# alazarteka/Self-Forcing

Hardware: AMD Instinct MI355X
Metric: decoded frames/sec/node, Wan-1.3B 832x480 4-step AR rollout (higher is better)
Workload: dtype bf16

## Files before the change

include/sf_hip.h:

```cpp
#ifndef SF_HIP_H
#define SF_HIP_H

#include <stddef.h>
#include <stdint.h>

#ifdef __cplusplus
extern "C" {
#endif

#define SF_HIP_ABI_VERSION 10

int sf_abi_version(void);
const char* sf_last_error(void);

enum sf_epilogue {
  SF_EPI_BIAS = 0,
  SF_EPI_BIAS_GELU = 1,
  SF_EPI_BIAS_RESID = 2,
  SF_EPI_BIAS_GATE_RESID = 3,
  SF_EPI_F32 = 4
};

typedef struct sf_gemm_args {
  const void* a;
  const void* w;
  const void* bias;
  void* out;
  const void* resid;
  const void* gate_mod;
  const void* gate_e0;
  int64_t gate_group_stride;
  int32_t rows_per_group;
  int32_t M, N, K;
  int32_t lda, ldw, ldo, ldr;
  int32_t epilogue;
  int32_t batch;
  int64_t a_bstride, w_bstride, o_bstride, r_bstride;
  int32_t structure;
} sf_gemm_args;

enum sf_gemm_structure { SF_GEMM_AUTO = 0, SF_GEMM_T128 = 1 ,
                         SF_GEMM_PP256 = 2 ,
                         SF_GEMM_PP128 = 3 ,
                         SF_GEMM_PP224 = 4, SF_GEMM_PP192 = 5  };

int sf_gemm_bf16(const sf_gemm_args* args, void* stream);

#define SF_FP8_AMAX_PARTS 1024
int sf_quantize_fp8(const void* x, int ldx, int M, int K, int rows_per_segment, void* q_out, float* scale_out, void* stream);

int sf_gemm_fp8(const sf_gemm_args* args, const float* a_scale, int rows_per_segment, const float* w_scale, void* stream);

int sf_small_linear_fp8(const void* x, const void* w_q, const float* w_scale, const void* bias, void* out, int M, int N, int K,
                        int rows_per_segment, int act_in, int act_out, void* stream);

int sf_small_linear(const void* x, const void* w, const void* bias, void* out, int M, int N, int K,
                    int act_in, int act_out, void* stream);

int sf_sinusoid_embedding(const void* t, int t_is_int64, void* out, int n, int dim, void* stream);

int sf_layernorm_modulate(const void* x, void* out, int M, int C, float eps, const void* mod_shift,
                          const void* mod_scale, const void* e0_shift, const void* e0_scale,
                          int64_t e0_group_stride, int rows_per_group, void* stream);

int sf_layernorm_affine(const void* x, const void* weight, const void* bias, void* out, int M, int C,
                        float eps, void* stream);

int sf_rmsnorm(const void* x, int ldx, const void* weight, void* out, int ldo, int M, int C, float eps,
               void* stream);

int sf_qkv_norm_rope_cache(const void* qkv, const void* norm_q_w, const void* norm_k_w, void* q_out,
                           void* k_cache, void* v_cache, const float* rope_cos, const float* rope_sin,
                           int B, int f, int h, int w, int C, int num_heads, int64_t cache_tokens,
                           int write_start, int start_frame, float eps, void* stream);

int sf_kv_evict(void* cache, int B, int64_t cache_tokens, int row_elems, int sink, int evict, int keep,
                void* scratch, size_t scratch_bytes, void* stream);

int sf_attention(const void* q, const void* k, const void* v, void* out, int B, int H, int Lq, int Lk,
                 int64_t q_stride, int64_t q_bstride, int64_t kv_stride, int64_t kv_bstride,
                 int64_t o_stride, int64_t o_bstride, void* stream);

enum sf_attn_structure { SF_ATTN_AUTO = 0, SF_ATTN_R64 = 1, SF_ATTN_W8 = 2, SF_ATTN_W4 = 3 };
int sf_attention_ex(const void* q, const void* k, const void* v, void* out, int B, int H, int Lq, int Lk,
                    int64_t q_stride, int64_t q_bstride, int64_t kv_stride, int64_t kv_bstride,
                    int64_t o_stride, int64_t o_bstride, int structure, void* stream);

int sf_patchify(const void* x, void* cols, int B, int F, int Cin, int H, int W, void* stream);

int sf_unpatchify_x0(const void* head_out, const void* xt, const void* timestep, int t_is_int64,
                     const float* sigmas, const float* timesteps, int n_table, void* flow, void* x0,
                     int B, int F, int groups, int Cout, int H, int W, void* stream);

int sf_add_noise(const void* x0, const void* eps, const void* timestep, int t_is_int64,
                 const float* sigmas, const float* timesteps, int n_table, void* out, int n_outer,
                 int64_t inner, void* stream);

#define SF_LINCOMB_MAX 6
int sf_lincomb_bf16(void* out, const void* const* xs, const float* coefs, int n_terms, int64_t n, void* stream);

typedef struct sf_layer_weights {
  const void* modulation;
  const void *norm3_w, *norm3_b;
  const void *qkv_w, *qkv_b;
  const void *norm_q_w, *norm_k_w;
  const void *o_w, *o_b;
  const void *cq_w, *cq_b;
  const void *ckv_w, *ckv_b;
  const void *cnorm_q_w, *cnorm_k_w;
  const void *co_w, *co_b;
  const void *ffn0_w, *ffn0_b;
  const void *ffn2_w, *ffn2_b;
} sf_layer_weights;

typedef struct sf_model {
  int32_t dim, ffn_dim, num_heads, num_layers, in_dim, out_dim, freq_dim, text_dim, text_len;
  float eps;
  const void *patch_w, *patch_b;
  const void *text0_w, *text0_b, *text2_w, *text2_b;
  const void *time0_w, *time0_b, *time2_w, *time2_b;
  const void *tproj_w, *tproj_b;
  const void *head_w, *head_b;
  const void* head_mod;
  const void *pose_w, *pose_b;
  int32_t pose_dim;
  const sf_layer_weights* layers_host;
  const float *rope_cos, *rope_sin;
  const float *sched_sigmas, *sched_timesteps;
  int32_t n_table;
  int32_t fp8;
  const void *text0_q, *text2_q, *time0_q, *time2_q, *tproj_q, *head_q, *pose_q;
  const float *text0_s, *text2_s, *time0_s, *time2_s, *tproj_s, *head_s, *pose_s;
  const struct sf_layer_fp8* layers_fp8_host;
} sf_model;

typedef struct sf_layer_fp8 {
  const void *qkv_q, *o_q, *cq_q, *ckv_q, *co_q, *ffn0_q, *ffn2_q;
  const float *qkv_s, *o_s, *cq_s, *ckv_s, *co_s, *ffn0_s, *ffn2_s;
} sf_layer_fp8;

typedef struct sf_forward_args {
  int32_t batch, frames, lat_h, lat_w;
  int32_t groups;
  const void* noisy;
  const void* timestep;
  int32_t t_is_int64;
  const void* prompt_embeds;
  int32_t init_cross;
  const void* add_condition;
  void* const* k_cache_host;
  void* const* v_cache_host;
  void* const* ck_cache_host;
  void* const* cv_cache_host;
  int64_t cache_tokens;
  int32_t sink_tokens, evict, keep;
  int32_t write_start;
  int32_t attn_start, attn_end;
  int32_t start_frame;
  void* evict_scratch;
  size_t evict_scratch_bytes;
  int32_t cache_only;
  void* flow_out;
  void* x0_out;
  void* workspace;
  size_t workspace_bytes;
  void* kv_index_out;
  int64_t global_end;
} sf_forward_args;

size_t sf_dit_workspace_bytes(const sf_model* model, int batch, int frames, int lat_h, int lat_w,
                              int groups);
int sf_dit_forward(const sf_model* model, const sf_forward_args* args, void* stream);
int sf_dit_forward_pair(const sf_model* model, const sf_forward_args* context_pass, const sf_forward_args* next_pass,
                        void* stream);


enum sf_conv_epilogue {
  SF_CONV_BIAS = 0,
  SF_CONV_BIAS_RESID = 1,
  SF_CONV_BIAS_CLAMP_F32 = 2
};

typedef struct sf_conv_args {
  const void* x;
  const void* w;
  const void* bias;
  void* out;
  const void* resid;
  float* out_f32;
  int32_t Tout, H, W;
  int32_t Hin, Win;
  int32_t Cin, Cout;
  int32_t kt, kh, kw;
  int32_t upsample;
  int32_t t_in_offset;
  int32_t ldw, ldo, ldr;
  int32_t out_frame_offset;
  int32_t interleave_c;
  int32_t epilogue;
  int32_t structure;
  void* norm_out;
  const void* norm_gamma;
  int32_t norm_ld, norm_frame_offset;
  int32_t stride_hw, stride_t;
} sf_conv_args;

enum sf_conv_structure { SF_CONV_AUTO = 0, SF_CONV_IGEMM = 1 ,
                         SF_CONV_HALO = 2  };

int sf_conv_igemm(const sf_conv_args* args, void* stream);
int sf_conv_pick_nt(int cout);

int sf_rmsnorm_silu_cl(const void* x, const void* gamma, void* out, int64_t rows, int C, int silu,
                       void* stream);

int sf_softmax_rows(const float* s, int64_t lds, void* p, int64_t ldp, int rows, int cols,
                    int cols_padded, float scale, void* stream);

int sf_vae_prepare_latent(const void* latent, const float* mean, const float* std, const void* conv2_w,
                          const void* conv2_b, void* out, int z, int h, int w, int c_pad, void* stream);

typedef struct sf_vae_conv {
  const void* w;
  const void* bias;
  int32_t cin, cout, kt, kh, kw, ldw;
} sf_vae_conv;

typedef struct sf_vae_resblock {
  const void* gamma1;
  const void* gamma2;
  sf_vae_conv conv1;
  sf_vae_conv conv2;
  sf_vae_conv shortcut;
} sf_vae_resblock;

#define SF_VAE_MAX_STAGES 4

typedef struct sf_vae_model {
  int32_t z_dim;
  int32_t n_stages;
  int32_t res_per_stage;
  int32_t temporal_up[SF_VAE_MAX_STAGES];
  const float* latent_mean;
  const float* latent_std;
  const void *conv2_w, *conv2_b;
  sf_vae_conv conv1;
  sf_vae_resblock mid0, mid2;
  const void* attn_gamma;
  const void *attn_qk_w, *attn_qk_b;
  const void *attn_v_w, *attn_v_b;
  const void *attn_proj_w, *attn_proj_b;
  const sf_vae_resblock* res_host;
  sf_vae_conv time_conv[SF_VAE_MAX_STAGES];
  sf_vae_conv up_conv[SF_VAE_MAX_STAGES];
  const void* head_gamma;
  sf_vae_conv head_conv;
} sf_vae_model;

size_t sf_vae_state_bytes(const sf_vae_model* model, int lat_h, int lat_w, int window_frames);
size_t sf_vae_scratch_bytes(const sf_vae_model* model, int lat_h, int lat_w, int window_frames);
int sf_vae_reset(const sf_vae_model* model, void* state, size_t state_bytes, int lat_h, int lat_w,
                 int window_frames, void* stream);
int sf_vae_decode_frames(const sf_vae_model* model, void* state, size_t state_bytes, void* scratch,
                         size_t scratch_bytes, const void* latent_frames, int lat_h, int lat_w, int window_frames,
                         int frame_index, int n_frames, int window, int history_at, float* pixels_out, void* stream);


int sf_vae_prepare_pixels(const void* pixels, int is_f32, int64_t c_stride, void* out, int T, int H, int W, int c_pad,
                          void* stream);

int sf_vae_finish_latent(const void* head_out, int ld_in, int cin, const void* conv1_w, int ld_w, const void* conv1_b,
                         const float* mean, const float* std, float* out, int T, int z, int h, int w, void* stream);

typedef struct sf_vae_encoder {
  int32_t z_dim;
  int32_t n_stages;
  int32_t res_per_stage;
  int32_t temporal_down[SF_VAE_MAX_STAGES];
  const float* latent_mean;
  const float* latent_std;
  const void *conv1_w, *conv1_b;
  sf_vae_conv in_conv;
  const sf_vae_resblock* res_host;
  sf_vae_conv down_conv[SF_VAE_MAX_STAGES];
  sf_vae_conv time_conv[SF_VAE_MAX_STAGES];
  sf_vae_resblock mid0, mid2;
  const void* attn_gamma;
  const void *attn_qk_w, *attn_qk_b;
  const void *attn_v_w, *attn_v_b;
  const void *attn_proj_w, *attn_proj_b;
  const void* head_gamma;
  sf_vae_conv head_conv;
} sf_vae_encoder;

size_t sf_vae_encode_state_bytes(const sf_vae_encoder* enc, int H, int W, int window_frames);
size_t sf_vae_encode_scratch_bytes(const sf_vae_encoder* enc, int H, int W, int window_frames);
int sf_vae_encode_reset(const sf_vae_encoder* enc, void* state, size_t state_bytes, int H, int W, int window_frames,
                        void* stream);
int sf_vae_encode_frames(const sf_vae_encoder* enc, void* state, size_t state_bytes, void* scratch, size_t scratch_bytes,
                         const void* pixels, int is_f32, int64_t c_stride, int H, int W, int window_frames,
                         int chunk_index, int n_chunks, int window, int history_at, float* latents_out, void* stream);


enum sf_taehv_epilogue {
  SF_TAEHV_BIAS_RELU = 0,
  SF_TAEHV_BIAS_RESID_RELU = 1,
  SF_TAEHV_PLAIN = 2,
  SF_TAEHV_RELU = 3,
  SF_TAEHV_HEAD_F32 = 4
};

typedef struct sf_taehv_conv_args {
  const void* x;
  const void* w;
  const void* bias;
  void* out;
  const void* resid;
  float* out_f32;
  int32_t Tout, H, W;
  int32_t Cin, Cout;
  int32_t kt;
  int32_t upsample;
  int32_t ldw, ldo, ldr;
  int32_t tgrow;
  int32_t epilogue;
  int32_t clamp;
} sf_taehv_conv_args;

// ... 145 lines not shown
```

self-forcing_amd/_lib.py:

```python
from __future__ import annotations

import ctypes as C
import os
import subprocess
from typing import Optional

os.environ.setdefault("ROC_SIGNAL_POOL_SIZE", "1024")

_HERE = os.path.dirname(os.path.abspath(__file__))
CSRC = os.path.join(_HERE, "csrc")
LIB_PATH = os.environ.get("SF_HIP_LIB") or os.path.join(CSRC, "libsf_hip.so")

ABI_VERSION = 10
FP8_AMAX_PARTS = 1024

EPI_BIAS, EPI_BIAS_GELU, EPI_BIAS_RESID, EPI_BIAS_GATE_RESID, EPI_F32 = 0, 1, 2, 3, 4
CONV_BIAS, CONV_BIAS_RESID, CONV_BIAS_CLAMP_F32 = 0, 1, 2
VAE_MAX_STAGES = 4
TAEHV_EPILOGUES = {"bias_relu": 0, "bias_resid_relu": 1, "plain": 2, "relu": 3, "head_f32": 4}
TAEHV_STAGES, TAEHV_BLOCKS = 3, 3
POSE_DTYPES = {"uint8": 0, "float32": 1, "bfloat16": 2}
POSE_CONVS = 6
JPEG_SUBSAMPLINGS = {"420": 0, "444": 1}
JPEG_DTYPES = {"uint8": 0, "float32": 1, "bfloat16": 2}
JPEG_RANGES = {(-1, 1): 0, (0, 1): 1}
JPEG_STATUS = {1: "an interval outgrew its worst-case slot", 2: "a coefficient is outside the baseline range",
               4: "the files do not fit the output buffer"}
ACT_NONE, ACT_SILU, ACT_GELU = 0, 1, 2
ATTN_STRUCTURES = {"auto": 0, "r64": 1, "w8": 2, "w4": 3}
CONV_STRUCTURES = {"auto": 0, "igemm": 1, "halo": 2}
GEMM_STRUCTURES = {"auto": 0, "t128": 1, "pp256": 2, "pp128": 3, "pp224": 4, "pp192": 5}


class GemmArgs(C.Structure):
    _fields_ = [
        ("a", C.c_void_p), ("w", C.c_void_p), ("bias", C.c_void_p), ("out", C.c_void_p),
        ("resid", C.c_void_p), ("gate_mod", C.c_void_p), ("gate_e0", C.c_void_p),
        ("gate_group_stride", C.c_int64), ("rows_per_group", C.c_int32),
        ("M", C.c_int32), ("N", C.c_int32), ("K", C.c_int32),
        ("lda", C.c_int32), ("ldw", C.c_int32), ("ldo", C.c_int32), ("ldr", C.c_int32),
        ("epilogue", C.c_int32), ("batch", C.c_int32),
        ("a_bstride", C.c_int64), ("w_bstride", C.c_int64), ("o_bstride", C.c_int64), ("r_bstride", C.c_int64),
        ("structure", C.c_int32),
    ]


class LayerWeights(C.Structure):
    _fields_ = [(n, C.c_void_p) for n in (
        "modulation", "norm3_w", "norm3_b", "qkv_w", "qkv_b", "norm_q_w", "norm_k_w", "o_w", "o_b",
        "cq_w", "cq_b", "ckv_w", "ckv_b", "cnorm_q_w", "cnorm_k_w", "co_w", "co_b",
        "ffn0_w", "ffn0_b", "ffn2_w", "ffn2_b")]


class LayerFp8(C.Structure):
    _fields_ = [(n, C.c_void_p) for n in (
        "qkv_q", "o_q", "cq_q", "ckv_q", "co_q", "ffn0_q", "ffn2_q",
        "qkv_s", "o_s", "cq_s", "ckv_s", "co_s", "ffn0_s", "ffn2_s")]


FP8_MODEL_LINEARS = (("text0", ("text_embedding.0",)), ("text2", ("text_embedding.2",)), ("time0", ("time_embedding.0",)),
                     ("time2", ("time_embedding.2",)), ("tproj", ("time_projection.1",)), ("head", ("head.head",)),
                     ("pose", ("pose_proj",)))
FP8_LAYER_LINEARS = (("qkv", ("self_attn.q", "self_attn.k", "self_attn.v")), ("o", ("self_attn.o",)), ("cq", ("cross_attn.q",)),
                     ("ckv", ("cross_attn.k", "cross_attn.v")), ("co", ("cross_attn.o",)), ("ffn0", ("ffn.0",)), ("ffn2", ("ffn.2",)))


class Model(C.Structure):
    _fields_ = (
        [(n, C.c_int32) for n in ("dim", "ffn_dim", "num_heads", "num_layers", "in_dim", "out_dim",
                                  "freq_dim", "text_dim", "text_len")]
        + [("eps", C.c_float)]
        + [(n, C.c_void_p) for n in ("patch_w", "patch_b", "text0_w", "text0_b", "text2_w", "text2_b",
                                     "time0_w", "time0_b", "time2_w", "time2_b", "tproj_w", "tproj_b",
                                     "head_w", "head_b", "head_mod", "pose_w", "pose_b")]
        + [("pose_dim", C.c_int32)]
        + [("layers_host", C.POINTER(LayerWeights)),
           ("rope_cos", C.c_void_p), ("rope_sin", C.c_void_p),
           ("sched_sigmas", C.c_void_p), ("sched_timesteps", C.c_void_p),
           ("n_table", C.c_int32)]
        + [("fp8", C.c_int32)]
        + [(n + "_q", C.c_void_p) for n, _ in FP8_MODEL_LINEARS]
        + [(n + "_s", C.c_void_p) for n, _ in FP8_MODEL_LINEARS]
        + [("layers_fp8_host", C.POINTER(LayerFp8))]
    )


class ForwardArgs(C.Structure):
    _fields_ = [
        ("batch", C.c_int32), ("frames", C.c_int32), ("lat_h", C.c_int32), ("lat_w", C.c_int32),
        ("groups", C.c_int32),
        ("noisy", C.c_void_p), ("timestep", C.c_void_p), ("t_is_int64", C.c_int32),
        ("prompt_embeds", C.c_void_p), ("init_cross", C.c_int32), ("add_condition", C.c_void_p),
        ("k_cache_host", C.POINTER(C.c_void_p)), ("v_cache_host", C.POINTER(C.c_void_p)),
        ("ck_cache_host", C.POINTER(C.c_void_p)), ("cv_cache_host", C.POINTER(C.c_void_p)),
        ("cache_tokens", C.c_int64),
        ("sink_tokens", C.c_int32), ("evict", C.c_int32), ("keep", C.c_int32),
        ("write_start", C.c_int32), ("attn_start", C.c_int32), ("attn_end", C.c_int32),
        ("start_frame", C.c_int32),
        ("evict_scratch", C.c_void_p), ("evict_scratch_bytes", C.c_size_t),
        ("cache_only", C.c_int32),
        ("flow_out", C.c_void_p), ("x0_out", C.c_void_p),
        ("workspace", C.c_void_p), ("workspace_bytes", C.c_size_t),
        ("kv_index_out", C.c_void_p), ("global_end", C.c_int64),
    ]


class ConvArgs(C.Structure):
    _fields_ = (
        [(n, C.c_void_p) for n in ("x", "w", "bias", "out", "resid", "out_f32")]
        + [(n, C.c_int32) for n in ("Tout", "H", "W", "Hin", "Win", "Cin", "Cout", "kt", "kh", "kw", "upsample",
                                    "t_in_offset", "ldw", "ldo", "ldr", "out_frame_offset", "interleave_c", "epilogue", "structure")]
        + [("norm_out", C.c_void_p), ("norm_gamma", C.c_void_p), ("norm_ld", C.c_int32), ("norm_frame_offset", C.c_int32)]
        + [("stride_hw", C.c_int32), ("stride_t", C.c_int32)]
    )


class VaeConv(C.Structure):
    _fields_ = [("w", C.c_void_p), ("bias", C.c_void_p)] + [(n, C.c_int32) for n in ("cin", "cout", "kt", "kh", "kw", "ldw")]


class VaeResBlock(C.Structure):
    _fields_ = [("gamma1", C.c_void_p), ("gamma2", C.c_void_p), ("conv1", VaeConv), ("conv2", VaeConv), ("shortcut", VaeConv)]


class VaeModel(C.Structure):
    _fields_ = [
        ("z_dim", C.c_int32), ("n_stages", C.c_int32), ("res_per_stage", C.c_int32),
        ("temporal_up", C.c_int32 * VAE_MAX_STAGES),
        ("latent_mean", C.c_void_p), ("latent_std", C.c_void_p), ("conv2_w", C.c_void_p), ("conv2_b", C.c_void_p),
        ("conv1", VaeConv), ("mid0", VaeResBlock), ("mid2", VaeResBlock),
        ("attn_gamma", C.c_void_p), ("attn_qk_w", C.c_void_p), ("attn_qk_b", C.c_void_p),
        ("attn_v_w", C.c_void_p), ("attn_v_b", C.c_void_p), ("attn_proj_w", C.c_void_p), ("attn_proj_b", C.c_void_p),
        ("res_host", C.POINTER(VaeResBlock)),
        ("time_conv", VaeConv * VAE_MAX_STAGES), ("up_conv", VaeConv * VAE_MAX_STAGES),
        ("head_gamma", C.c_void_p), ("head_conv", VaeConv),
    ]


class VaeEncoder(C.Structure):
    _fields_ = [
        ("z_dim", C.c_int32), ("n_stages", C.c_int32), ("res_per_stage", C.c_int32),
        ("temporal_down", C.c_int32 * VAE_MAX_STAGES),
        ("latent_mean", C.c_void_p), ("latent_std", C.c_void_p), ("conv1_w", C.c_void_p), ("conv1_b", C.c_void_p),
        ("in_conv", VaeConv), ("res_host", C.POINTER(VaeResBlock)),
        ("down_conv", VaeConv * VAE_MAX_STAGES), ("time_conv", VaeConv * VAE_MAX_STAGES),
        ("mid0", VaeResBlock), ("mid2", VaeResBlock),
        ("attn_gamma", C.c_void_p), ("attn_qk_w", C.c_void_p), ("attn_qk_b", C.c_void_p),
        ("attn_v_w", C.c_void_p), ("attn_v_b", C.c_void_p), ("attn_proj_w", C.c_void_p), ("attn_proj_b", C.c_void_p),
        ("head_gamma", C.c_void_p), ("head_conv", VaeConv),
    ]


class TaehvConvArgs(C.Structure):
    _fields_ = ([(n, C.c_void_p) for n in ("x", "w", "bias", "out", "resid", "out_f32")]
                + [(n, C.c_int32) for n in ("Tout", "H", "W", "Cin", "Cout", "kt", "upsample", "ldw", "ldo", "ldr", "tgrow", "epilogue", "clamp")])


class TaehvLayer(C.Structure):
    _fields_ = [("w", C.c_void_p), ("bias", C.c_void_p)] + [(n, C.c_int32) for n in ("cin", "cout", "kt", "ldw")]


class TaehvModel(C.Structure):
    _fields_ = [("z_dim", C.c_int32), ("in_conv", TaehvLayer), ("block", ((TaehvLayer * 3) * TAEHV_BLOCKS) * TAEHV_STAGES),
                ("exit_conv", TaehvLayer * TAEHV_STAGES), ("tgrow", C.c_int32 * TAEHV_STAGES), ("head", TaehvLayer)]


class PoseConvArgs(C.Structure):
    _fields_ = ([(n, C.c_void_p) for n in ("x", "w", "bias", "out")]
                + [(n, C.c_int32) for n in ("T", "H", "W", "Cin", "Cout", "kt", "stride_t", "stride_s", "ldw", "ldo", "silu")])


class PoseLayer(C.Structure):
    _fields_ = [("w", C.c_void_p), ("bias", C.c_void_p)] + [(n, C.c_int32) for n in ("cin", "cout", "kt", "stride_t", "stride_s", "ldw", "silu")]


class PoseModel(C.Structure):
    _fields_ = [("conv", PoseLayer * POSE_CONVS), ("embed_w", C.c_void_p), ("embed_b", C.c_void_p), ("pose_dim", C.c_int32),
                ("ref_conv", PoseLayer * POSE_CONVS)]


class T5Layer(C.Structure):
    _fields_ = [(n, C.c_void_p) for n in ("norm1_w", "qk_w", "v_w", "o_w", "norm2_w", "gate_w", "fc1_w", "fc2_w", "pos_emb")]


class T5Model(C.Structure):
    _fields_ = ([(n, C.c_int32) for n in ("vocab", "dim", "dim_attn", "dim_ffn", "num_heads", "num_layers", "num_buckets")]
                + [("eps", C.c_float), ("token_embedding", C.c_void_p), ("layers_host", C.POINTER(T5Layer)),
                   ("final_norm_w", C.c_void_p)])


_vp, _i, _i64, _f, _sz = C.c_void_p, C.c_int, C.c_int64, C.c_float, C.c_size_t
SIGNATURES = {
    "sf_abi_version": (C.c_int, []),
    "sf_last_error": (C.c_char_p, []),
    "sf_gemm_bf16": (C.c_int, [C.POINTER(GemmArgs), _vp]),
    "sf_small_linear": (C.c_int, [_vp, _vp, _vp, _vp, _i, _i, _i, _i, _i, _vp]),
    "sf_quantize_fp8": (C.c_int, [_vp, _i, _i, _i, _i, _vp, _vp, _vp]),
    "sf_gemm_fp8": (C.c_int, [C.POINTER(GemmArgs), _vp, _i, _vp, _vp]),
    "sf_small_linear_fp8": (C.c_int, [_vp, _vp, _vp, _vp, _vp, _i, _i, _i, _i, _i, _i, _vp]),
    "sf_sinusoid_embedding": (C.c_int, [_vp, _i, _vp, _i, _i, _vp]),
    "sf_layernorm_modulate": (C.c_int, [_vp, _vp, _i, _i, _f, _vp, _vp, _vp, _vp, _i64, _i, _vp]),
    "sf_layernorm_affine": (C.c_int, [_vp, _vp, _vp, _vp, _i, _i, _f, _vp]),
    "sf_rmsnorm": (C.c_int, [_vp, _i, _vp, _vp, _i, _i, _i, _f, _vp]),
    "sf_qkv_norm_rope_cache": (C.c_int, [_vp, _vp, _vp, _vp, _vp, _vp, _vp, _vp, _i, _i, _i, _i, _i, _i, _i64,
                                         _i, _i, _f, _vp]),
    "sf_kv_evict": (C.c_int, [_vp, _i, _i64, _i, _i, _i, _i, _vp, _sz, _vp]),
    "sf_attention": (C.c_int, [_vp, _vp, _vp, _vp, _i, _i, _i, _i, _i64, _i64, _i64, _i64, _i64, _i64, _vp]),
    "sf_attention_ex": (C.c_int, [_vp, _vp, _vp, _vp, _i, _i, _i, _i, _i64, _i64, _i64, _i64, _i64, _i64, _i, _vp]),
    "sf_patchify": (C.c_int, [_vp, _vp, _i, _i, _i, _i, _i, _vp]),
    "sf_unpatchify_x0": (C.c_int, [_vp, _vp, _vp, _i, _vp, _vp, _i, _vp, _vp, _i, _i, _i, _i, _i, _i, _vp]),
    "sf_add_noise": (C.c_int, [_vp, _vp, _vp, _i, _vp, _vp, _i, _vp, _i, _i64, _vp]),
    "sf_lincomb_bf16": (C.c_int, [_vp, C.POINTER(C.c_void_p), C.POINTER(C.c_float), _i, _i64, _vp]),
    "sf_dit_workspace_bytes": (C.c_size_t, [C.POINTER(Model), _i, _i, _i, _i, _i]),
    "sf_dit_forward": (C.c_int, [C.POINTER(Model), C.POINTER(ForwardArgs), _vp]),
    "sf_dit_forward_pair": (C.c_int, [C.POINTER(Model), C.POINTER(ForwardArgs), C.POINTER(ForwardArgs), _vp]),
    "sf_conv_igemm": (C.c_int, [C.POINTER(ConvArgs), _vp]),
    "sf_conv_pick_nt": (C.c_int, [_i]),
    "sf_rmsnorm_silu_cl": (C.c_int, [_vp, _vp, _vp, _i64, _i, _i, _vp]),
    "sf_softmax_rows": (C.c_int, [_vp, _i64, _vp, _i64, _i, _i, _i, _f, _vp]),
    "sf_vae_prepare_latent": (C.c_int, [_vp, _vp, _vp, _vp, _vp, _vp, _i, _i, _i, _i, _vp]),
    "sf_vae_state_bytes": (C.c_size_t, [C.POINTER(VaeModel), _i, _i, _i]),
    "sf_vae_scratch_bytes": (C.c_size_t, [C.POINTER(VaeModel), _i, _i, _i]),
    "sf_vae_reset": (C.c_int, [C.POINTER(VaeModel), _vp, _sz, _i, _i, _i, _vp]),
    "sf_vae_decode_frames": (C.c_int, [C.POINTER(VaeModel), _vp, _sz, _vp, _sz, _vp, _i, _i, _i, _i, _i, _i, _i, _vp, _vp]),
    "sf_vae_prepare_pixels": (C.c_int, [_vp, _i, _i64, _vp, _i, _i, _i, _i, _vp]),
    "sf_vae_finish_latent": (C.c_int, [_vp, _i, _i, _vp, _i, _vp, _vp, _vp, _vp, _i, _i, _i, _i, _vp]),
    "sf_vae_encode_state_bytes": (C.c_size_t, [C.POINTER(VaeEncoder), _i, _i, _i]),
    "sf_vae_encode_scratch_bytes": (C.c_size_t, [C.POINTER(VaeEncoder), _i, _i, _i]),
    "sf_vae_encode_reset": (C.c_int, [C.POINTER(VaeEncoder), _vp, _sz, _i, _i, _i, _vp]),
    "sf_vae_encode_frames": (C.c_int, [C.POINTER(VaeEncoder), _vp, _sz, _vp, _sz, _vp, _i, _i64, _i, _i, _i, _i, _i, _i, _i, _vp,
                                       _vp]),
    "sf_taehv_conv": (C.c_int, [C.POINTER(TaehvConvArgs), _vp]),
    "sf_taehv_pick_nt": (C.c_int, [_i]),
    "sf_taehv_prepare_latent": (C.c_int, [_vp, _vp, _i, _i, _i, _i, _i, _vp]),
    "sf_taehv_state_bytes": (C.c_size_t, [C.POINTER(TaehvModel), _i, _i]),
    "sf_taehv_scratch_bytes": (C.c_size_t, [C.POINTER(TaehvModel), _i, _i, _i]),
    "sf_taehv_reset": (C.c_int, [C.POINTER(TaehvModel), _vp, _sz, _i, _i, _vp]),
    "sf_taehv_decode_frames": (C.c_int, [C.POINTER(TaehvModel), _vp, _sz, _vp, _sz, _vp, _i, _i, _i, _i, _vp, _vp]),
    "sf_pose_out_size": (C.c_int, [_i, _i, _i]),
    "sf_pose_conv": (C.c_int, [C.POINTER(PoseConvArgs), _vp]),
    "sf_pose_prepare": (C.c_int, [_vp, _i, _i, _i, _i, _i, _i, _vp, _vp]),
    "sf_pose_patch_embed": (C.c_int, [_vp, _i, _i, _i, _vp, _vp, _i, _vp, _vp, _vp]),
    "sf_pose_scratch_bytes": (C.c_size_t, [C.POINTER(PoseModel), _i, _i, _i]),
    "sf_pose_embed": (C.c_int, [C.POINTER(PoseModel), _vp, _i, _i, _i, _i, _vp, _sz, _vp, _i64, _vp]),
    "sf_pose_embed_ref": (C.c_int, [C.POINTER(PoseModel), _vp, _i, _i, _i, _vp, _sz, _vp, _vp]),
    "sf_jpeg_workspace_bytes": (C.c_size_t, [_i, _i, _i, _i, _i]),
    "sf_jpeg_transform": (C.c_int, [_vp, _i, _i, _i, _i, _i, _i, _i, _vp, _vp]),
    "sf_jpeg_entropy": (C.c_int, [_vp, _i, _i, _i, _i, _i, _i, _vp, _sz, _vp, _sz, _vp, _vp, _vp]),
    "sf_jpeg_encode_frames": (C.c_int, [_vp, _i, _i, _i, _i, _i, _i, _i, _i, _vp, _sz, _vp, _sz, _vp, _vp, _vp]),
    "sf_embedding_gather": (C.c_int, [_vp, _vp, _vp, _i, _i, _i, _vp]),
    "sf_t5_softmax_bias": (C.c_int, [_vp, _vp, _vp, _vp, _vp, _i, _i, _i, _vp]),
    "sf_mul_bf16": (C.c_int, [_vp, _vp, _vp, _i64, _vp]),
    "sf_zero_masked_rows": (C.c_int, [_vp, _vp, _i, _i, _vp]),
    "sf_t5_workspace_bytes": (C.c_size_t, [C.POINTER(T5Model), _i, _i]),
    "sf_t5_encode": (C.c_int, [C.POINTER(T5Model), _vp, _vp, _vp, _i, _i, _vp, _vp, _sz, _vp]),
    "sf_probe_mfma": (C.c_int, [_i, _i, _i, _vp, _vp, C.POINTER(C.c_double), _vp]),
    "sf_probe_copy": (C.c_int, [_vp, _vp, _sz, _vp]),
}

_lib: Optional[C.CDLL] = None


class SfHipError(RuntimeError):
    pass


def build(verbose: bool = False) -> str:
    cmd = ["make", "-C", CSRC, "-j8"]
    res = subprocess.run(cmd, capture_output=True, text=True)
    if verbose or res.returncode != 0:
        print(res.stdout)
        print(res.stderr)
    if res.returncode != 0:
        raise SfHipError(f"building {LIB_PATH} failed (exit {res.returncode})")
    return LIB_PATH


def lib() -> C.CDLL:
    global _lib
    if _lib is not None:
        return _lib
    if not os.path.exists(LIB_PATH):
        raise SfHipError(
            f"{LIB_PATH} not found: the HIP extension is not built. Run "
            f"`python -c 'import __graft_entry__ as g; g.build()'` (or `make -C {CSRC}`). "
            "There is no CPU/eager fallback for this path.")
    handle = C.CDLL(LIB_PATH)
    for name, (res, args) in SIGNATURES.items():
        fn = getattr(handle, name)
        fn.restype = res
        fn.argtypes = args
    ver = handle.sf_abi_version()
    if ver != ABI_VERSION:
        raise SfHipError(f"{LIB_PATH}: ABI version {ver}, expected {ABI_VERSION}; rebuild")
    _lib = handle
    return handle


def check(rc: int, what: str = "") -> None:
    if rc != 0:
        msg = lib().sf_last_error()
        raise SfHipError(f"{what or 'sf_hip'} failed (rc={rc}): {msg.decode() if msg else '?'}")
```

self-forcing_amd/csrc/dit_forward.hip:

```cpp
#include <algorithm>
#include "sf_host.h"

int sf_internal_write_kv_indices(void* buf, int layers, int64_t global_end, int64_t local_end, void* stream);

namespace {

struct Work {
  void *x, *xn, *qkv, *q, *att, *hbuf, *cols, *headout, *sin, *etmp, *e, *e0, *ctx1, *ctx;
  void* xq;
  float* xs;
  size_t total;
};

constexpr int FP8_MAX_SEGMENTS = 8;

Work carve(const sf_model* m, void* ws, int B, int F, int lat_h, int lat_w, int groups) {
  const size_t M = (size_t)B * F * (lat_h / 2) * (lat_w / 2);
  const size_t C = m->dim, BG = (size_t)B * groups, T = (size_t)B * m->text_len;
  Carve c(ws);
  Work w;
  w.x = c.take(M * C * 2);
  w.xn = c.take(M * C * 2);
  w.qkv = c.take(M * 3 * C * 2);
  w.q = c.take(M * C * 2);
  w.att = c.take(M * C * 2);
  w.hbuf = c.take(M * (size_t)m->ffn_dim * 2);
  w.cols = c.take(M * (size_t)m->in_dim * 4 * 2);
  w.headout = c.take(M * (size_t)m->out_dim * 4 * 2);
  w.sin = c.take(BG * m->freq_dim * 2);
  w.etmp = c.take(BG * C * 2);
  w.e = c.take(BG * C * 2);
  w.e0 = c.take(BG * 6 * C * 2);
  w.ctx1 = c.take(T * C * 2);
  w.ctx = c.take(T * C * 2);
  w.xq = nullptr;
  w.xs = nullptr;
  if (m->fp8) {
    const size_t pose = m->pose_dim > 0 ? (size_t)m->pose_dim : C;
    const size_t widest_tok = std::max({(size_t)m->ffn_dim, C, pose}), widest_txt = std::max((size_t)m->text_dim, C);
    w.xq = c.take(std::max(M * widest_tok, T * widest_txt));
    w.xs = (float*)c.take(FP8_MAX_SEGMENTS * (1 + SF_FP8_AMAX_PARTS) * sizeof(float));
  }
  w.total = c.off;
  return w;
}

inline const char* bptr(const void* p, size_t elems) { return (const char*)p + elems * 2; }

}

extern "C" size_t sf_dit_workspace_bytes(const sf_model* model, int batch, int frames, int lat_h, int lat_w, int groups) {
  if (!model || batch <= 0 || frames <= 0 || lat_h <= 0 || lat_w <= 0 || groups <= 0) return 0;
  return carve(model, nullptr, batch, frames, lat_h, lat_w, groups).total;
}

static int forward_passes(const sf_model* m, const sf_forward_args* const* ps, int np, void* stream) {
  const sf_forward_args* a = ps[0];
  SF_CHECK(m && a, "sf_dit_forward: null argument");
  SF_CHECK(m->layers_host && m->num_layers > 0, "sf_dit_forward: model has no layers");
  SF_CHECK(m->dim == m->num_heads * 128, "sf_dit_forward: head_dim must be 128 (dim=%d heads=%d)", m->dim, m->num_heads);
  SF_CHECK(a->batch > 0 && a->frames > 0 && a->groups > 0, "sf_dit_forward: empty input");
  SF_CHECK(a->lat_h % 2 == 0 && a->lat_w % 2 == 0, "sf_dit_forward: latent size must be even");
  const int B = a->batch, F = a->frames, h = a->lat_h / 2, w = a->lat_w / 2;
  const int L = F * h * w, M = B * L, C = m->dim, G = a->groups, BG = B * G;
  const int Mt = np * M, BGt = np * BG;
  SF_CHECK(F % G == 0, "sf_dit_forward: frames=%d not divisible by timestep groups=%d", F, G);
  const int rpg = L / G;
  SF_CHECK(BGt <= 32, "sf_dit_forward: passes*batch*groups=%d exceeds the small-linear limit of 32", BGt);
  int first_full = np;
  for (int p = 0; p < np; ++p) {
    const sf_forward_args* q = ps[p];
    SF_CHECK(q, "sf_dit_forward: null pass");
    SF_CHECK(q->batch == B && q->frames == F && q->lat_h == a->lat_h && q->lat_w == a->lat_w && q->groups == G,
             "sf_dit_forward: the passes of one call must share batch, frames, latent size and timestep groups");
    SF_CHECK(q->k_cache_host == a->k_cache_host && q->v_cache_host == a->v_cache_host && q->ck_cache_host == a->ck_cache_host &&
             q->cv_cache_host == a->cv_cache_host && q->cache_tokens == a->cache_tokens, "sf_dit_forward: the passes of one call must share their caches");
    SF_CHECK(q->noisy && q->timestep, "sf_dit_forward: null tensor");
    SF_CHECK(q->cache_only || (q->flow_out && q->x0_out), "sf_dit_forward: null output tensor");
    SF_CHECK(q->attn_start >= 0 && q->attn_end > q->attn_start && q->attn_end <= q->cache_tokens, "sf_dit_forward: bad attention window [%d, %d) of %lld",
             q->attn_start, q->attn_end, (long long)q->cache_tokens);
    SF_CHECK(q->write_start >= 0 && (int64_t)q->write_start + L <= q->cache_tokens,
             "sf_dit_forward: KV cache overflow: write_start=%d + %d new tokens > capacity %lld", q->write_start, L, (long long)q->cache_tokens);
    SF_CHECK(q->write_start + L == q->attn_end, "sf_dit_forward: the new tokens must end the attention window");
    if (q->evict > 0) SF_CHECK(q->evict_scratch && q->keep >= 0, "sf_dit_forward: eviction needs evict_scratch");
    SF_CHECK(np == 1 || !q->init_cross, "sf_dit_forward_pair: the cross-attention cache must be initialised by an earlier single pass");
    if (!q->cache_only && first_full == np) first_full = p;
    SF_CHECK(!(q->cache_only && first_full != np), "sf_dit_forward_pair: cache_only passes must come first");
  }
  SF_CHECK(a->k_cache_host && a->v_cache_host && a->ck_cache_host && a->cv_cache_host, "sf_dit_forward: null cache table");
  const Work ws = carve(m, a->workspace, np * B, F, a->lat_h, a->lat_w, G);
  SF_CHECK(a->workspace && a->workspace_bytes >= ws.total, "sf_dit_forward: workspace too small (%zu < %zu)", a->workspace_bytes, ws.total);
  SF_CHECK(!a->init_cross || a->prompt_embeds, "sf_dit_forward: init_cross needs prompt_embeds");

  const bool f8 = m->fp8 != 0;
  static const sf_layer_fp8 no_fp8 = {};
  SF_CHECK(!f8 || m->layers_fp8_host, "sf_dit_forward: fp8 model without per-layer fp8 weights");
  auto run = [&](const Gemm& g) -> int { return f8 ? g.fp8(ws.xq, ws.xs, stream) : g.bf16(stream); };
  auto lin = [&](const Gemm& g) -> int {
    if (f8) SF_TRY(sf_quantize_fp8(g.g.a, g.g.lda, g.g.M, g.g.K, g.rows_per_segment, ws.xq, ws.xs, stream));
    return run(g);
  };
  auto small = [&](const void* x, const void* w16, const void* w8, const float* s8, const void* bias, void* out, int N, int K, int act_in,
                   int act_out) -> int {
    if (!f8) return sf_small_linear(x, w16, bias, out, BGt, N, K, act_in, act_out, stream);
    return sf_small_linear_fp8(x, w8, s8, bias, out, BGt, N, K, BG, act_in, act_out, stream);
  };

  const int Kp = m->in_dim * 4, Nh = m->out_dim * 4;
  const long cache_b = (long)a->cache_tokens * C;
  const long ctx_b = (long)m->text_len * C;
  const sf_forward_args* last = ps[np - 1];
  auto finish_indices = [&]() -> int {
    if (last->kv_index_out) return sf_internal_write_kv_indices(last->kv_index_out, m->num_layers, last->global_end, last->attn_end, stream);
    return 0;
  };

  for (int p = 0; p < np; ++p)
    SF_TRY(sf_patchify(ps[p]->noisy, (void*)bptr(ws.cols, (size_t)p * M * Kp), B, F, m->in_dim, a->lat_h, a->lat_w, stream));
  SF_TRY(Gemm(ws.cols, Kp, m->patch_w, Kp, ws.x, C, Mt, C, Kp).bias(m->patch_b).bf16(stream));

  for (int p = 0; p < np; ++p) {
    if (!ps[p]->add_condition) continue;
    void* xp = (void*)bptr(ws.x, (size_t)p * M * C);
    if (m->pose_w || (f8 && m->pose_q)) {
      SF_CHECK(m->pose_dim > 0, "sf_dit_forward: pose_proj weights without pose_dim");
      SF_TRY(lin(Gemm(ps[p]->add_condition, m->pose_dim, m->pose_w, m->pose_dim, xp, C, M, C, m->pose_dim).bias(m->pose_b)
                     .epi(SF_EPI_BIAS_RESID).resid(xp, C).fp8w(m->pose_q, m->pose_s, M)));
    } else {
      SF_CHECK(m->pose_dim == C, "sf_dit_forward: add_condition without pose_proj weights needs pose_dim == dim (%d != %d)", m->pose_dim, C);
      const void* terms[2] = {xp, ps[p]->add_condition};
      const float ones[2] = {1.0f, 1.0f};
      SF_TRY(sf_lincomb_bf16(xp, terms, ones, 2, (int64_t)M * C, stream));
    }
  }

  for (int p = 0; p < np; ++p)
    SF_TRY(sf_sinusoid_embedding(ps[p]->timestep, ps[p]->t_is_int64, (void*)bptr(ws.sin, (size_t)p * BG * m->freq_dim), BG, m->freq_dim, stream));
  SF_TRY(small(ws.sin, m->time0_w, m->time0_q, m->time0_s, m->time0_b, ws.etmp, C, m->freq_dim, 0, 1));
  SF_TRY(small(ws.etmp, m->time2_w, m->time2_q, m->time2_s, m->time2_b, ws.e, C, C, 0, 0));
  SF_TRY(small(ws.e, m->tproj_w, m->tproj_q, m->tproj_s, m->tproj_b, ws.e0, 6 * C, C, 1, 0));

  if (a->init_cross) {
    const int T = B * m->text_len;
    SF_TRY(lin(Gemm(a->prompt_embeds, m->text_dim, m->text0_w, m->text_dim, ws.ctx1, C, T, C, m->text_dim).bias(m->text0_b).epi(SF_EPI_BIAS_GELU)
                   .fp8w(m->text0_q, m->text0_s, T)));
    SF_TRY(lin(Gemm(ws.ctx1, C, m->text2_w, C, ws.ctx, C, T, C, C).bias(m->text2_b).fp8w(m->text2_q, m->text2_s, T)));
    if (f8) SF_TRY(sf_quantize_fp8(ws.ctx, C, T, C, T, ws.xq, ws.xs, stream));
    for (int l = 0; l < m->num_layers; ++l) {
      const sf_layer_weights& lw = m->layers_host[l];
      const sf_layer_fp8& lq = f8 ? m->layers_fp8_host[l] : no_fp8;
      SF_TRY(run(Gemm(ws.ctx, C, lw.ckv_w, C, a->ck_cache_host[l], C, T, C, C).bias(lw.ckv_b).fp8w(lq.ckv_q, lq.ckv_s, T)));
      SF_TRY(sf_rmsnorm(a->ck_cache_host[l], C, lw.cnorm_k_w, a->ck_cache_host[l], C, T, C, m->eps, stream));
      SF_TRY(run(Gemm(ws.ctx, C, bptr(lw.ckv_w, (size_t)C * C), C, a->cv_cache_host[l], C, T, C, C).bias(bptr(lw.ckv_b, C))
                     .fp8w(f8 ? (const char*)lq.ckv_q + (size_t)C * C : nullptr, f8 ? lq.ckv_s + C : nullptr, T)));
    }
  }

  for (int l = 0; l < m->num_layers; ++l) {
    const sf_layer_weights& lw = m->layers_host[l];
    const sf_layer_fp8& lq = f8 ? m->layers_fp8_host[l] : no_fp8;
    const void* mod = lw.modulation;
    const bool last_layer = l == m->num_layers - 1;
    SF_TRY(sf_layernorm_modulate(ws.x, ws.xn, Mt, C, m->eps, bptr(mod, 0), bptr(mod, C), bptr(ws.e0, 0), bptr(ws.e0, C), 6L * C, rpg, stream));
    SF_TRY(lin(Gemm(ws.xn, C, lw.qkv_w, C, ws.qkv, 3 * C, Mt, 3 * C, C).bias(lw.qkv_b).fp8w(lq.qkv_q, lq.qkv_s, M)));
    for (int p = 0; p < np; ++p) {
      const sf_forward_args* q = ps[p];
      const size_t roff = (size_t)p * M;
      if (q->evict > 0) {
        SF_TRY(sf_kv_evict(q->k_cache_host[l], B, q->cache_tokens, C, q->sink_tokens, q->evict, q->keep, q->evict_scratch, q->evict_scratch_bytes, stream));
        SF_TRY(sf_kv_evict(q->v_cache_host[l], B, q->cache_tokens, C, q->sink_tokens, q->evict, q->keep, q->evict_scratch, q->evict_scratch_bytes, stream));
      }
      SF_TRY(sf_qkv_norm_rope_cache(bptr(ws.qkv, roff * 3 * C), lw.norm_q_w, lw.norm_k_w, (void*)bptr(ws.q, roff * C), q->k_cache_host[l], q->v_cache_host[l],
                                    m->rope_cos, m->rope_sin, B, F, h, w, C, m->num_heads, q->cache_tokens, q->write_start, q->start_frame, m->eps, stream));
      if (q->cache_only && last_layer) continue;
      SF_TRY(sf_attention(bptr(ws.q, roff * C), bptr(q->k_cache_host[l], (size_t)q->attn_start * C), bptr(q->v_cache_host[l], (size_t)q->attn_start * C),
                          (void*)bptr(ws.att, roff * C), B, m->num_heads, L, q->attn_end - q->attn_start, C, (long)L * C, C, cache_b, C, (long)L * C, stream));
    }
    const int p0 = last_layer ? first_full : 0;
    if (p0 == np) return finish_indices();
    const size_t r0 = (size_t)p0 * M;
    const int Mr = (np - p0) * M;
    void* x = (void*)bptr(ws.x, r0 * C);
    void* xn = (void*)bptr(ws.xn, r0 * C);
    void* qb = (void*)bptr(ws.q, r0 * C);
    void* att = (void*)bptr(ws.att, r0 * C);
    void* hb = (void*)bptr(ws.hbuf, r0 * m->ffn_dim);
    const void* e0r = bptr(ws.e0, (size_t)p0 * BG * 6 * C);
    SF_TRY(lin(Gemm(att, C, lw.o_w, C, x, C, Mr, C, C).bias(lw.o_b).epi(SF_EPI_BIAS_GATE_RESID).resid(x, C)
                   .gate(bptr(mod, 2 * (size_t)C), bptr(e0r, 2 * (size_t)C), 6L * C, rpg).fp8w(lq.o_q, lq.o_s, M)));
    SF_TRY(sf_layernorm_affine(x, lw.norm3_w, lw.norm3_b, xn, Mr, C, m->eps, stream));
    SF_TRY(lin(Gemm(xn, C, lw.cq_w, C, qb, C, Mr, C, C).bias(lw.cq_b).fp8w(lq.cq_q, lq.cq_s, M)));
    SF_TRY(sf_rmsnorm(qb, C, lw.cnorm_q_w, qb, C, Mr, C, m->eps, stream));
    for (int p = p0; p < np; ++p)
      SF_TRY(sf_attention(bptr(ws.q, (size_t)p * M * C), a->ck_cache_host[l], a->cv_cache_host[l], (void*)bptr(ws.att, (size_t)p * M * C), B, m->num_heads, L,
                          m->text_len, C, (long)L * C, C, ctx_b, C, (long)L * C, stream));
    SF_TRY(lin(Gemm(att, C, lw.co_w, C, x, C, Mr, C, C).bias(lw.co_b).epi(SF_EPI_BIAS_RESID).resid(x, C).fp8w(lq.co_q, lq.co_s, M)));
    SF_TRY(sf_layernorm_modulate(x, xn, Mr, C, m->eps, bptr(mod, 3 * (size_t)C), bptr(mod, 4 * (size_t)C), bptr(e0r, 3 * (size_t)C),
                                 bptr(e0r, 4 * (size_t)C), 6L * C, rpg, stream));
    SF_TRY(lin(Gemm(xn, C, lw.ffn0_w, C, hb, m->ffn_dim, Mr, m->ffn_dim, C).bias(lw.ffn0_b).epi(SF_EPI_BIAS_GELU).fp8w(lq.ffn0_q, lq.ffn0_s, M)));
    SF_TRY(lin(Gemm(hb, m->ffn_dim, lw.ffn2_w, m->ffn_dim, x, C, Mr, C, m->ffn_dim).bias(lw.ffn2_b).epi(SF_EPI_BIAS_GATE_RESID).resid(x, C)
                   .gate(bptr(mod, 5 * (size_t)C), bptr(e0r, 5 * (size_t)C), 6L * C, rpg).fp8w(lq.ffn2_q, lq.ffn2_s, M)));
  }

  {
    const size_t r0 = (size_t)first_full * M;
    const int Mr = (np - first_full) * M;
    const void* er = bptr(ws.e, (size_t)first_full * BG * C);
    SF_TRY(sf_layernorm_modulate(bptr(ws.x, r0 * C), (void*)bptr(ws.xn, r0 * C), Mr, C, m->eps, bptr(m->head_mod, 0), bptr(m->head_mod, C), er, er, (long)C, rpg, stream));
    SF_TRY(lin(Gemm(bptr(ws.xn, r0 * C), C, m->head_w, C, (void*)bptr(ws.headout, r0 * Nh), Nh, Mr, Nh, C).bias(m->head_b)
                   .fp8w(m->head_q, m->head_s, M)));
    for (int p = first_full; p < np; ++p)
      SF_TRY(sf_unpatchify_x0(bptr(ws.headout, (size_t)p * M * Nh), ps[p]->noisy, ps[p]->timestep, ps[p]->t_is_int64, m->sched_sigmas, m->sched_timesteps, m->n_table,
                              ps[p]->flow_out, ps[p]->x0_out, B, F, G, m->out_dim, a->lat_h, a->lat_w, stream));
  }
  return finish_indices();
}

extern "C" int sf_dit_forward(const sf_model* m, const sf_forward_args* a, void* stream) {
  SF_CHECK(m && a, "sf_dit_forward: null argument");
  const sf_forward_args* one[1] = {a};
  return forward_passes(m, one, 1, stream);
}

extern "C" int sf_dit_forward_pair(const sf_model* m, const sf_forward_args* context_pass, const sf_forward_args* next_pass, void* stream) {
  SF_CHECK(m && context_pass && next_pass, "sf_dit_forward_pair: null argument");
  SF_CHECK(context_pass->workspace == next_pass->workspace && context_pass->workspace_bytes == next_pass->workspace_bytes,
           "sf_dit_forward_pair: both passes name the same workspace (sized for 2 x batch)");
  const sf_forward_args* two[2] = {context_pass, next_pass};
  return forward_passes(m, two, 2, stream);
}
```

self-forcing_amd/csrc/elementwise.hip:

```cpp
#include "sf_common.h"
#include "../../include/sf_hip.h"

namespace {

constexpr int ROWS_PER_BLOCK = 4;

template <int NCH>
__device__ __forceinline__ void load_row(const bf16_t* row, int lane, float (&v)[NCH][8]) {
#pragma unroll
  for (int i = 0; i < NCH; ++i) {
    const bf16x8 t = *reinterpret_cast<const bf16x8*>(row + (i * 64 + lane) * 8);
#pragma unroll
    for (int j = 0; j < 8; ++j) v[i][j] = (float)t[j];
  }
}

template <int NCH>
__device__ __forceinline__ void ln_stats(const float (&v)[NCH][8], int C, float eps, float& mean, float& rstd) {
  float s = 0.f;
#pragma unroll
  for (int i = 0; i < NCH; ++i)
#pragma unroll
    for (int j = 0; j < 8; ++j) s += v[i][j];
  mean = wave_sum(s) / (float)C;
  float q = 0.f;
#pragma unroll
  for (int i = 0; i < NCH; ++i)
#pragma unroll
    for (int j = 0; j < 8; ++j) {
      const float d = v[i][j] - mean;
      q += d * d;
    }
  rstd = rsqrtf(wave_sum(q) / (float)C + eps);
}

#ifndef SF_LN_RPW
#define SF_LN_RPW 2
#endif
template <int NCH> struct LnRows { static constexpr int value = NCH <= 4 ? SF_LN_RPW : (NCH <= 6 ? 2 : 1); };
template <int NCH, int MODE>
__global__ __launch_bounds__(64) void layernorm_kernel(const bf16_t* __restrict__ x, bf16_t* __restrict__ out,
                                                       int M, int C, float eps, const bf16_t* __restrict__ p0,
                                                       const bf16_t* __restrict__ p1, const bf16_t* __restrict__ e0_shift,
                                                       const bf16_t* __restrict__ e0_scale, long e0_group_stride,
                                                       int rows_per_group) {
  constexpr int LN_RPW = LnRows<NCH>::value;
  const int lane = threadIdx.x;
  const int row0 = blockIdx.x * LN_RPW;
  bf16x8 raw[LN_RPW][NCH];
#pragma unroll
  for (int r = 0; r < LN_RPW; ++r) {
    const long row = min(row0 + r, M - 1);
#pragma unroll
    for (int i = 0; i < NCH; ++i) raw[r][i] = *reinterpret_cast<const bf16x8*>(x + row * C + (i * 64 + lane) * 8);
  }
  bf16x8 scl[NCH], add[NCH];
  int cur_group = -1;
#pragma unroll
  for (int r = 0; r < LN_RPW; ++r) {
    const int row = row0 + r;
    if (row >= M) break;
    const int grp = MODE == 0 ? row / rows_per_group : 0;
    if (grp != cur_group) {
      cur_group = grp;
      const long goff = (long)grp * e0_group_stride;
#pragma unroll
      for (int i = 0; i < NCH; ++i) {
        const int e = (i * 64 + lane) * 8;
        if (MODE == 0) {
          const bf16x8 ms = *reinterpret_cast<const bf16x8*>(p0 + e);
          const bf16x8 mc = *reinterpret_cast<const bf16x8*>(p1 + e);
          const bf16x8 es = *reinterpret_cast<const bf16x8*>(e0_shift + goff + e);
          const bf16x8 ec = *reinterpret_cast<const bf16x8*>(e0_scale + goff + e);
#pragma unroll
          for (int j = 0; j < 8; ++j) {
            add[i][j] = (bf16_t)((float)ms[j] + (float)es[j]);
            scl[i][j] = (bf16_t)((float)mc[j] + (float)ec[j]);
          }
        } else {
          scl[i] = *reinterpret_cast<const bf16x8*>(p0 + e);
          add[i] = *reinterpret_cast<const bf16x8*>(p1 + e);
        }
      }
    }
    float v[NCH][8];
#pragma unroll
    for (int i = 0; i < NCH; ++i)
#pragma unroll
      for (int j = 0; j < 8; ++j) v[i][j] = (float)raw[r][i][j];
    float mean, rstd;
    ln_stats<NCH>(v, C, eps, mean, rstd);
#pragma unroll
    for (int i = 0; i < NCH; ++i) {
      bf16x8 o;
#pragma unroll
      for (int j = 0; j < 8; ++j)
        o[j] = (bf16_t)((v[i][j] - mean) * rstd * (MODE == 0 ? 1.0f + (float)scl[i][j] : (float)scl[i][j]) + (float)add[i][j]);
      *reinterpret_cast<bf16x8*>(out + (long)row * C + (i * 64 + lane) * 8) = o;
    }
  }
}

template <int NCH>
__global__ __launch_bounds__(256) void rmsnorm_kernel(const bf16_t* __restrict__ x, int ldx, const bf16_t* __restrict__ w,
                                                      bf16_t* __restrict__ out, int ldo, int M, int C, float eps) {
  const int lane = threadIdx.x & 63;
  const int row = blockIdx.x * ROWS_PER_BLOCK + (threadIdx.x >> 6);
  if (row >= M) return;
  float v[NCH][8];
  load_row<NCH>(x + (long)row * ldx, lane, v);
  float q = 0.f;
#pragma unroll
  for (int i = 0; i < NCH; ++i)
#pragma unroll
    for (int j = 0; j < 8; ++j) q += v[i][j] * v[i][j];
  const float r = rsqrtf(wave_sum(q) / (float)C + eps);
#pragma unroll
  for (int i = 0; i < NCH; ++i) {
    const int e = (i * 64 + lane) * 8;
    const bf16x8 wt = *reinterpret_cast<const bf16x8*>(w + e);
    bf16x8 o;
#pragma unroll
    for (int j = 0; j < 8; ++j) o[j] = (bf16_t)((float)(bf16_t)(v[i][j] * r) * (float)wt[j]);
    *reinterpret_cast<bf16x8*>(out + (long)row * ldo + e) = o;
  }
}

template <int NCH>
__global__ __launch_bounds__(256) void qkv_norm_rope_cache_kernel(
    const bf16_t* __restrict__ qkv, const bf16_t* __restrict__ wq, const bf16_t* __restrict__ wk,
    bf16_t* __restrict__ q_out, bf16_t* __restrict__ k_cache, bf16_t* __restrict__ v_cache,
    const float* __restrict__ rope_cos, const float* __restrict__ rope_sin, int rows, int L, int hgt, int wid, int C,
    long cache_tokens, int write_start, int start_frame, float eps, int c0, int c1) {
  const int lane = threadIdx.x & 63;
  const int row = blockIdx.x * ROWS_PER_BLOCK + (threadIdx.x >> 6);
  if (row >= rows) return;
  const int b = row / L, t = row - b * L;
  const int fi = t / (hgt * wid), rem = t - fi * (hgt * wid);
  const int hi = rem / wid, wi = rem - hi * wid;
  const int pos_t = start_frame + fi;
  const bf16_t* src = qkv + (long)row * 3 * C;
  const long crow = ((long)b * cache_tokens + write_start + t) * C;

#pragma unroll
  for (int i = 0; i < NCH; ++i) {
    const int e = (i * 64 + lane) * 8;
    *reinterpret_cast<u32x4*>(v_cache + crow + e) = *reinterpret_cast<const u32x4*>(src + 2 * C + e);
  }

#pragma unroll
  for (int which = 0; which < 2; ++which) {
    float v[NCH][8];
    load_row<NCH>(src + which * C, lane, v);
    float q = 0.f;
#pragma unroll
    for (int i = 0; i < NCH; ++i)
#pragma unroll
      for (int j = 0; j < 8; ++j) q += v[i][j] * v[i][j];
    const float r = rsqrtf(wave_sum(q) / (float)C + eps);
    const bf16_t* wn = which ? wk : wq;
    bf16_t* dst = which ? (k_cache + crow) : (q_out + (long)row * C);
#pragma unroll
    for (int i = 0; i < NCH; ++i) {
      const int e = (i * 64 + lane) * 8;
      const bf16x8 wt = *reinterpret_cast<const bf16x8*>(wn + e);
      const int pair0 = (e & 127) >> 1;
      bf16x8 o;
#pragma unroll
      for (int pp = 0; pp < 4; ++pp) {
        const int pj = pair0 + pp;
        const int pos = pj < c0 ? pos_t : (pj < c0 + c1 ? hi : wi);
        const float cs = rope_cos[pos * 64 + pj];
        const float sn = rope_sin[pos * 64 + pj];
        const float re = (float)(bf16_t)((float)(bf16_t)(v[i][2 * pp] * r) * (float)wt[2 * pp]);
        const float im = (float)(bf16_t)((float)(bf16_t)(v[i][2 * pp + 1] * r) * (float)wt[2 * pp + 1]);
        o[2 * pp] = (bf16_t)(re * cs - im * sn);
        o[2 * pp + 1] = (bf16_t)(re * sn + im * cs);
      }
      *reinterpret_cast<bf16x8*>(dst + e) = o;
    }
  }
}

__global__ __launch_bounds__(256) void copy_rows_kernel(const char* __restrict__ src, long src_bstride,
                                                        char* __restrict__ dst, long dst_bstride, long bytes_per_batch) {
  const long n16 = bytes_per_batch >> 4;
  const char* s = src + (long)blockIdx.y * src_bstride;
  char* d = dst + (long)blockIdx.y * dst_bstride;
  for (long i = (long)blockIdx.x * blockDim.x + threadIdx.x; i < n16; i += (long)gridDim.x * blockDim.x)
    reinterpret_cast<u32x4*>(d)[i] = reinterpret_cast<const u32x4*>(s)[i];
}

__global__ __launch_bounds__(256) void patchify_kernel(const bf16_t* __restrict__ x, bf16_t* __restrict__ cols, long total,
                                                       int Cin, int H, int W) {
  const int h2 = H >> 1, w2 = W >> 1;
  for (long i = (long)blockIdx.x * blockDim.x + threadIdx.x; i < total; i += (long)gridDim.x * blockDim.x) {
    const int cch = (int)(i % Cin);
    long r = i / Cin;
    const int ww = (int)(r % w2); r /= w2;
    const int hh = (int)(r % h2);
    const long bf = r / h2;
    const bf16_t* s = x + ((bf * Cin + cch) * H + 2 * hh) * (long)W + 2 * ww;
    bf16x4 o;
    o[0] = s[0]; o[1] = s[1]; o[2] = s[W]; o[3] = s[W + 1];
    *reinterpret_cast<bf16x4*>(cols + ((bf * h2 + hh) * w2 + ww) * (long)(Cin * 4) + cch * 4) = o;
  }
}

__device__ __forceinline__ double block_sigma_lookup(double t, const float* __restrict__ sigmas,
                                                     const float* __restrict__ timesteps, int n_table) {
  __shared__ double s_val[4];
  __shared__ int s_idx[4];
  double best = 1e300;
  int bi = 0x7fffffff;
  for (int j = threadIdx.x; j < n_table; j += blockDim.x) {
    const double d = fabs((double)timesteps[j] - t);
    if (d < best) { best = d; bi = j; }
  }
#pragma unroll
  for (int o = 32; o > 0; o >>= 1) {
    const double ob = __shfl_xor(best, o, 64);
    const int oi = __shfl_xor(bi, o, 64);
    if (ob < best || (ob == best && oi < bi)) { best = ob; bi = oi; }
  }
  const int wv = threadIdx.x >> 6;
  if ((threadIdx.x & 63) == 0) { s_val[wv] = best; s_idx[wv] = bi; }
  __syncthreads();
  best = s_val[0]; bi = s_idx[0];
  for (int k = 1; k < (int)(blockDim.x >> 6); ++k)
    if (s_val[k] < best || (s_val[k] == best && s_idx[k] < bi)) { best = s_val[k]; bi = s_idx[k]; }
  return (double)sigmas[bi];
}

__device__ __forceinline__ bf16_t double_to_bf16(double d) {
  const float f = (float)d;
  const unsigned u = __float_as_uint(f);
  if ((u & 0xFFFFu) == 0x8000u) {
    const double r = d - (double)f;
    if (r != 0.0) {
      const bool up = (f > 0.f) ? (r > 0.0) : (r < 0.0);
      const unsigned hi = (u >> 16) + (up ? 1u : 0u);
      return __builtin_bit_cast(bf16_t, (unsigned short)hi);
    }
  }
  return (bf16_t)f;
}

__device__ __forceinline__ double read_timestep(const void* t, int is_i64, long idx) {
  return is_i64 ? (double)reinterpret_cast<const long long*>(t)[idx] : (double)reinterpret_cast<const float*>(t)[idx];
}

__global__ __launch_bounds__(256) void unpatchify_x0_kernel(const bf16_t* __restrict__ head_out, const bf16_t* __restrict__ xt,
                                                            const void* __restrict__ timestep, int t_is_i64,
                                                            const float* __restrict__ sigmas, const float* __restrict__ timesteps,
                                                            int n_table, bf16_t* __restrict__ flow, bf16_t* __restrict__ x0,
                                                            int F, int groups, int Cout, int H, int W) {
#pragma clang fp contract(off)
  const int bf = blockIdx.y;
  const int b = bf / F, f = bf - b * F;
  const int grp = f / (F / groups);
  const double sigma = block_sigma_lookup(read_timestep(timestep, t_is_i64, (long)b * groups + grp), sigmas, timesteps, n_table);
  const int h2 = H >> 1, w2 = W >> 1;
  const int total = Cout * H * w2;
  for (int i = blockIdx.x * blockDim.x + threadIdx.x; i < total; i += gridDim.x * blockDim.x) {
    const int ww = i % w2;
    int r = i / w2;
    const int y = r % H;
    const int cch = r / H;
    const int hh = y >> 1, pq = y & 1;
    const long tok = ((long)bf * h2 + hh) * w2 + ww;
    const bf16_t* hs = head_out + tok * (4 * Cout) + (pq * 2) * Cout + cch;
    const long o = (((long)bf * Cout + cch) * H + y) * W + 2 * ww;
    const bf16_t f0 = hs[0], f1 = hs[Cout];
    bf16x2 fo; fo[0] = f0; fo[1] = f1;
    *reinterpret_cast<bf16x2*>(flow + o) = fo;
    const bf16x2 xv = *reinterpret_cast<const bf16x2*>(xt + o);
    bf16x2 xo;
    xo[0] = double_to_bf16((double)(float)xv[0] - sigma * (double)(float)f0);
    xo[1] = double_to_bf16((double)(float)xv[1] - sigma * (double)(float)f1);
    *reinterpret_cast<bf16x2*>(x0 + o) = xo;
  }
}

__global__ __launch_bounds__(256) void add_noise_kernel(const bf16_t* __restrict__ x0, const bf16_t* __restrict__ eps,
                                                        const void* __restrict__ timestep, int t_is_i64,
                                                        const float* __restrict__ sigmas, const float* __restrict__ timesteps,
                                                        int n_table, bf16_t* __restrict__ out, long inner) {
#pragma clang fp contract(off)
  const long base = (long)blockIdx.y * inner;
  const float sigma = (float)block_sigma_lookup(read_timestep(timestep, t_is_i64, blockIdx.y), sigmas, timesteps, n_table);
  const float om = 1.0f - sigma;
  const long n8 = inner >> 3;
  for (long i = (long)blockIdx.x * blockDim.x + threadIdx.x; i < n8; i += (long)gridDim.x * blockDim.x) {
    const bf16x8 a = *reinterpret_cast<const bf16x8*>(x0 + base + i * 8);
    const bf16x8 e = *reinterpret_cast<const bf16x8*>(eps + base + i * 8);
    bf16x8 o;
#pragma unroll
    for (int j = 0; j < 8; ++j) o[j] = (bf16_t)(om * (float)a[j] + sigma * (float)e[j]);
    *reinterpret_cast<bf16x8*>(out + base + i * 8) = o;
  }
}

struct LinCombP {
  const bf16_t* x[SF_LINCOMB_MAX];
  float c[SF_LINCOMB_MAX];
  bf16_t* out;
  long n8;
  int n_terms;
};
template <int NT>
__global__ __launch_bounds__(256) void lincomb_kernel(const LinCombP p) {
#pragma clang fp contract(off)
  for (long i = (long)blockIdx.x * blockDim.x + threadIdx.x; i < p.n8; i += (long)gridDim.x * blockDim.x) {
    float acc[8];
#pragma unroll
    for (int k = 0; k < NT; ++k) {
      const bf16x8 v = *reinterpret_cast<const bf16x8*>(p.x[k] + i * 8);
#pragma unroll
      for (int j = 0; j < 8; ++j) acc[j] = k == 0 ? p.c[0] * (float)v[j] : acc[j] + p.c[k] * (float)v[j];
    }
    bf16x8 o;
#pragma unroll
    for (int j = 0; j < 8; ++j) o[j] = (bf16_t)acc[j];
    *reinterpret_cast<bf16x8*>(p.out + i * 8) = o;
  }
}

__global__ __launch_bounds__(256) void sinusoid_kernel(const void* __restrict__ t, int t_is_i64, bf16_t* __restrict__ out,
                                                       int n, int dim) {
  const int half = dim >> 1;
  const int i = blockIdx.x * blockDim.x + threadIdx.x;
  if (i >= n * half) return;
  const int r = i / half, k = i - r * half;
  const double pos = read_timestep(t, t_is_i64, r);
  const double ang = pos * pow(10000.0, -(double)k / (double)half);
  out[(long)r * dim + k] = double_to_bf16(cos(ang));
  out[(long)r * dim + half + k] = double_to_bf16(sin(ang));
}

template <int MODE>
int launch_layernorm(const bf16_t* x, bf16_t* out, int M, int C, float eps, const bf16_t* p0, const bf16_t* p1,
                     const bf16_t* e0s, const bf16_t* e0c, long gs, int rpg, hipStream_t s) {
  const dim3 block(64);
  switch (C / 512) {
#define SF_LN_CASE(N) \
  case N: hipLaunchKernelGGL((layernorm_kernel<N, MODE>), dim3((M + LnRows<N>::value - 1) / LnRows<N>::value), block, 0, s, x, out, M, C, eps, p0, p1, e0s, e0c, gs, rpg); break;
    SF_LN_CASE(1) SF_LN_CASE(2) SF_LN_CASE(3) SF_LN_CASE(4) SF_LN_CASE(5) SF_LN_CASE(6) SF_LN_CASE(8) SF_LN_CASE(10)
#undef SF_LN_CASE
    default: sf_set_error("layernorm: unsupported channel count %d", C); return -1;
  }
  return 0;
}

bool channels_ok(int C) {
  if (C % 512 != 0) return false;
  const int n = C / 512;
  return n == 1 || n == 2 || n == 3 || n == 4 || n == 5 || n == 6 || n == 8 || n == 10;
}

}

extern "C" int sf_layernorm_modulate(const void* x, void* out, int M, int C, float eps, const void* mod_shift,
                                     const void* mod_scale, const void* e0_shift, const void* e0_scale,
                                     int64_t e0_group_stride, int rows_per_group, void* stream) {
  SF_CHECK(x && out && mod_shift && mod_scale && e0_shift && e0_scale, "sf_layernorm_modulate: null tensor");
  SF_CHECK(M > 0 && channels_ok(C), "sf_layernorm_modulate: unsupported shape M=%d C=%d (C must be 512*{1,2,3,4,5,6,8,10})", M, C);
  SF_CHECK(rows_per_group > 0 && e0_group_stride % 8 == 0, "sf_layernorm_modulate: bad group layout");
  if (launch_layernorm<0>((const bf16_t*)x, (bf16_t*)out, M, C, eps, (const bf16_t*)mod_shift, (const bf16_t*)mod_scale,
                          (const bf16_t*)e0_shift, (const bf16_t*)e0_scale, e0_group_stride, rows_per_group,
                          (hipStream_t)stream) != 0)
    return -1;
  SF_HIP_LAUNCH_CHECK("sf_layernorm_modulate");
  return 0;
}

extern "C" int sf_layernorm_affine(const void* x, const void* weight, const void* bias, void* out, int M, int C,
                                   float eps, void* stream) {
  SF_CHECK(x && out && weight && bias, "sf_layernorm_affine: null tensor");
  SF_CHECK(M > 0 && channels_ok(C), "sf_layernorm_affine: unsupported shape M=%d C=%d", M, C);
  if (launch_layernorm<1>((const bf16_t*)x, (bf16_t*)out, M, C, eps, (const bf16_t*)weight, (const bf16_t*)bias, nullptr,
                          nullptr, 0, 1, (hipStream_t)stream) != 0)
    return -1;
  SF_HIP_LAUNCH_CHECK("sf_layernorm_affine");
  return 0;
}

extern "C" int sf_rmsnorm(const void* x, int ldx, const void* weight, void* out, int ldo, int M, int C, float eps,
                          void* stream) {
  SF_CHECK(x && out && weight, "sf_rmsnorm: null tensor");
  SF_CHECK(M > 0 && channels_ok(C) && ldx >= C && ldo >= C && ldx % 8 == 0 && ldo % 8 == 0, "sf_rmsnorm: unsupported shape M=%d C=%d", M, C);
  const dim3 grid((M + ROWS_PER_BLOCK - 1) / ROWS_PER_BLOCK), block(256);
  hipStream_t s = (hipStream_t)stream;
  switch (C / 512) {
#define SF_RMS_CASE(N) \
  case N: hipLaunchKernelGGL((rmsnorm_kernel<N>), grid, block, 0, s, (const bf16_t*)x, ldx, (const bf16_t*)weight, (bf16_t*)out, ldo, M, C, eps); break;
    SF_RMS_CASE(1) SF_RMS_CASE(2) SF_RMS_CASE(3) SF_RMS_CASE(4) SF_RMS_CASE(5) SF_RMS_CASE(6) SF_RMS_CASE(8) SF_RMS_CASE(10)
#undef SF_RMS_CASE
  }
  SF_HIP_LAUNCH_CHECK("sf_rmsnorm");
  return 0;
}

extern "C" int sf_qkv_norm_rope_cache(const void* qkv, const void* norm_q_w, const void* norm_k_w, void* q_out,
                                      void* k_cache, void* v_cache, const float* rope_cos, const float* rope_sin,
                                      int B, int f, int h, int w, int C, int num_heads, int64_t cache_tokens,
                                      int write_start, int start_frame, float eps, void* stream) {
  SF_CHECK(qkv && norm_q_w && norm_k_w && q_out && k_cache && v_cache && rope_cos && rope_sin, "sf_qkv_norm_rope_cache: null tensor");
  SF_CHECK(B > 0 && f > 0 && h > 0 && w > 0 && channels_ok(C), "sf_qkv_norm_rope_cache: unsupported shape");
  SF_CHECK(num_heads > 0 && C == num_heads * 128, "sf_qkv_norm_rope_cache: head_dim must be 128 (C=%d heads=%d)", C, num_heads);
  const int L = f * h * w;
  SF_CHECK(write_start >= 0 && (int64_t)write_start + L <= cache_tokens, "sf_qkv_norm_rope_cache: cache overflow: write_start=%d + L=%d > capacity=%lld",
           write_start, L, (long long)cache_tokens);
  SF_CHECK(start_frame >= 0 && start_frame + f <= 1024 && h <= 1024 && w <= 1024, "sf_qkv_norm_rope_cache: RoPE position out of the 1024-entry table");
  const int rows = B * L;
  const dim3 grid((rows + ROWS_PER_BLOCK - 1) / ROWS_PER_BLOCK), block(256);
  hipStream_t s = (hipStream_t)stream;
  const int c = 64, c1 = c / 3, c0 = c - 2 * c1;
  switch (C / 512) {
#define SF_QKV_CASE(N)                                                                                                   \
  case N: hipLaunchKernelGGL((qkv_norm_rope_cache_kernel<N>), grid, block, 0, s, (const bf16_t*)qkv, (const bf16_t*)norm_q_w, \
                             (const bf16_t*)norm_k_w, (bf16_t*)q_out, (bf16_t*)k_cache, (bf16_t*)v_cache, rope_cos, rope_sin,  \
                             rows, L, h, w, C, (long)cache_tokens, write_start, start_frame, eps, c0, c1); break;
    SF_QKV_CASE(1) SF_QKV_CASE(2) SF_QKV_CASE(3) SF_QKV_CASE(4) SF_QKV_CASE(5) SF_QKV_CASE(6) SF_QKV_CASE(8) SF_QKV_CASE(10)
#undef SF_QKV_CASE
  }
  SF_HIP_LAUNCH_CHECK("sf_qkv_norm_rope_cache");
  return 0;
}

extern "C" int sf_kv_evict(void* cache, int B, int64_t cache_tokens, int row_elems, int sink, int evict, int keep,
                           void* scratch, size_t scratch_bytes, void* stream) {
  SF_CHECK(cache && B > 0 && row_elems > 0 && (row_elems % 8) == 0, "sf_kv_evict: bad arguments");
  SF_CHECK(sink >= 0 && evict >= 0 && keep >= 0 && (int64_t)sink + evict + keep <= cache_tokens, "sf_kv_evict: window out of range");
  if (evict == 0 || keep == 0) return 0;
  const long row_b = (long)row_elems * 2;
  const long bytes = (long)keep * row_b;
  SF_CHECK(scratch && scratch_bytes >= (size_t)(bytes * B), "sf_kv_evict: scratch too small (%zu < %ld)", scratch_bytes, bytes * B);
  char* base = (char*)cache;
  const long bstride = (long)cache_tokens * row_b;
  const int gx = (int)min((long)2048, (bytes / 16 + 255) / 256);
  const dim3 grid(gx, B), block(256);
  hipStream_t s = (hipStream_t)stream;
  hipLaunchKernelGGL(copy_rows_kernel, grid, block, 0, s, base + (long)(sink + evict) * row_b, bstride, (char*)scratch, bytes, bytes);
  hipLaunchKernelGGL(copy_rows_kernel, grid, block, 0, s, (const char*)scratch, bytes, base + (long)sink * row_b, bstride, bytes);
  SF_HIP_LAUNCH_CHECK("sf_kv_evict");
  return 0;
}

extern "C" int sf_patchify(const void* x, void* cols, int B, int F, int Cin, int H, int W, void* stream) {
  SF_CHECK(x && cols && B > 0 && F > 0 && Cin > 0, "sf_patchify: bad arguments");
  SF_CHECK(H % 2 == 0 && W % 2 == 0, "sf_patchify: latent H=%d W=%d must be even (patch 2x2)", H, W);
  const long total = (long)B * F * (H / 2) * (W / 2) * Cin;
  const int gx = (int)min((long)4096, (total + 255) / 256);
  hipLaunchKernelGGL(patchify_kernel, dim3(gx), dim3(256), 0, (hipStream_t)stream, (const bf16_t*)x, (bf16_t*)cols, total, Cin, H, W);
  SF_HIP_LAUNCH_CHECK("sf_patchify");
  return 0;
}

extern "C" int sf_unpatchify_x0(const void* head_out, const void* xt, const void* timestep, int t_is_int64,
                                const float* sigmas, const float* timesteps, int n_table, void* flow, void* x0,
                                int B, int F, int groups, int Cout, int H, int W, void* stream) {
  SF_CHECK(head_out && xt && timestep && sigmas && timesteps && flow && x0, "sf_unpatchify_x0: null tensor");
  SF_CHECK(B > 0 && F > 0 && groups > 0 && F % groups == 0, "sf_unpatchify_x0: frames=%d not divisible by groups=%d", F, groups);
  SF_CHECK(H % 2 == 0 && W % 2 == 0 && n_table > 0, "sf_unpatchify_x0: bad shape");
  const int total = Cout * H * (W / 2);
  const dim3 grid(min(64, (total + 255) / 256), B * F), block(256);
  hipLaunchKernelGGL(unpatchify_x0_kernel, grid, block, 0, (hipStream_t)stream, (const bf16_t*)head_out, (const bf16_t*)xt, timestep,
                     t_is_int64, sigmas, timesteps, n_table, (bf16_t*)flow, (bf16_t*)x0, F, groups, Cout, H, W);
  SF_HIP_LAUNCH_CHECK("sf_unpatchify_x0");
  return 0;
}

extern "C" int sf_add_noise(const void* x0, const void* eps, const void* timestep, int t_is_int64, const float* sigmas,
                            const float* timesteps, int n_table, void* out, int n_outer, int64_t inner, void* stream) {
  SF_CHECK(x0 && eps && timestep && sigmas && timesteps && out, "sf_add_noise: null tensor");
  SF_CHECK(n_outer > 0 && inner > 0 && inner % 8 == 0 && n_table > 0, "sf_add_noise: bad shape (inner must be a multiple of 8)");
  const dim3 grid((unsigned)min((long)64, (long)((inner / 8 + 255) / 256)), n_outer), block(256);
  hipLaunchKernelGGL(add_noise_kernel, grid, block, 0, (hipStream_t)stream, (const bf16_t*)x0, (const bf16_t*)eps, timestep, t_is_int64,
                     sigmas, timesteps, n_table, (bf16_t*)out, (long)inner);
  SF_HIP_LAUNCH_CHECK("sf_add_noise");
  return 0;
}

extern "C" int sf_lincomb_bf16(void* out, const void* const* xs, const float* coefs, int n_terms, int64_t n, void* stream) {
  SF_CHECK(out && xs && coefs, "sf_lincomb_bf16: null argument");
  SF_CHECK(n_terms >= 1 && n_terms <= SF_LINCOMB_MAX, "sf_lincomb_bf16: n_terms must be 1..%d, got %d", SF_LINCOMB_MAX, n_terms);
  SF_CHECK(n > 0 && n % 8 == 0, "sf_lincomb_bf16: element count must be a positive multiple of 8");
  LinCombP p;
  for (int k = 0; k < SF_LINCOMB_MAX; ++k) {
    p.x[k] = k < n_terms ? (const bf16_t*)xs[k] : nullptr;
    p.c[k] = k < n_terms ? coefs[k] : 0.0f;
    SF_CHECK(k >= n_terms || xs[k], "sf_lincomb_bf16: null input %d", k);
  }
  p.out = (bf16_t*)out;
  p.n8 = n / 8;
  p.n_terms = n_terms;
  const dim3 grid((unsigned)min((long)2048, (p.n8 + 255) / 256)), block(256);
  switch (n_terms) {
    case 1: hipLaunchKernelGGL(lincomb_kernel<1>, grid, block, 0, (hipStream_t)stream, p); break;
    case 2: hipLaunchKernelGGL(lincomb_kernel<2>, grid, block, 0, (hipStream_t)stream, p); break;
    case 3: hipLaunchKernelGGL(lincomb_kernel<3>, grid, block, 0, (hipStream_t)stream, p); break;
    case 4: hipLaunchKernelGGL(lincomb_kernel<4>, grid, block, 0, (hipStream_t)stream, p); break;
    case 5: hipLaunchKernelGGL(lincomb_kernel<5>, grid, block, 0, (hipStream_t)stream, p); break;
    default: hipLaunchKernelGGL(lincomb_kernel<6>, grid, block, 0, (hipStream_t)stream, p); break;
  }
  SF_HIP_LAUNCH_CHECK("sf_lincomb_bf16");
  return 0;
}

__global__ void kv_index_kernel(long long* __restrict__ buf, int layers, long long global_end, long long local_end) {
  const int i = blockIdx.x * blockDim.x + threadIdx.x;
  if (i < 2 * layers) buf[i] = (i & 1) ? local_end : global_end;
}
__attribute__((visibility("hidden"))) int sf_internal_write_kv_indices(void* buf, int layers, int64_t global_end, int64_t local_end, void* stream) {
  hipLaunchKernelGGL(kv_index_kernel, dim3((2 * layers + 63) / 64), dim3(64), 0, (hipStream_t)stream, (long long*)buf, layers,
                     (long long)global_end, (long long)local_end);
  SF_HIP_LAUNCH_CHECK("kv_index_kernel");
  return 0;
}

extern "C" int sf_sinusoid_embedding(const void* t, int t_is_int64, void* out, int n, int dim, void* stream) {
  SF_CHECK(t && out && n > 0 && dim > 0 && dim % 2 == 0, "sf_sinusoid_embedding: bad arguments");
  const int total = n * (dim / 2);
  hipLaunchKernelGGL(sinusoid_kernel, dim3((total + 255) / 256), dim3(256), 0, (hipStream_t)stream, t, t_is_int64, (bf16_t*)out, n, dim);
  SF_HIP_LAUNCH_CHECK("sf_sinusoid_embedding");
  return 0;
}
```

self-forcing_amd/csrc/gemm_bf16.hip:

```cpp
#include <type_traits>
#include "sf_common.h"
#include "../../include/sf_hip.h"

namespace {

constexpr int BM = 128, BN = 128, BK = 64;
constexpr int GEMM_THREADS = 256;
constexpr int TILE_BYTES = BM * BK * 2;
constexpr int STAGE_BYTES = 2 * TILE_BYTES;
constexpr int GEMM_LDS = 2 * STAGE_BYTES;

struct GemmP {
  const bf16_t* a;
  const bf16_t* w;
  const bf16_t* bias;
  bf16_t* out;
  const bf16_t* resid;
  const bf16_t* gate_mod;
  const bf16_t* gate_e0;
  long gate_group_stride;
  int rows_per_group;
  int M, N, K, lda, ldw, ldo, ldr;
  int tiles_m, tiles_n;
  long a_bs, w_bs, o_bs, r_bs;
  const float* a_scale;
  const float* w_scale;
  int rows_per_seg;
};

typedef const __attribute__((address_space(1))) void* gptr_t;
typedef __attribute__((address_space(3))) void* lptr_t;

__device__ __forceinline__ void glds16(const bf16_t* src, char* lds_wave_base) {
  __builtin_amdgcn_global_load_lds((gptr_t)src, (lptr_t)lds_wave_base, 16, 0, 0);
}

typedef int i32x4 __attribute__((ext_vector_type(4)));
typedef int i32x8 __attribute__((ext_vector_type(8)));

__device__ __forceinline__ f32x4 mfma_f8(const bf16x8& w0, const bf16x8& w1, const bf16x8& x0, const bf16x8& x1, const f32x4& acc) {
  const i32x8 wv = __builtin_shufflevector(__builtin_bit_cast(i32x4, w0), __builtin_bit_cast(i32x4, w1), 0, 1, 2, 3, 4, 5, 6, 7);
  const i32x8 xv = __builtin_shufflevector(__builtin_bit_cast(i32x4, x0), __builtin_bit_cast(i32x4, x1), 0, 1, 2, 3, 4, 5, 6, 7);
  return __builtin_amdgcn_mfma_scale_f32_16x16x128_f8f6f4(wv, xv, acc, 0, 0, 0, 127, 0, 127);
}

template <int MT>
__device__ __forceinline__ void fp8_scale_acc(const GemmP& p, f32x4 (&acc)[MT][4], int m_base, int n_base, int lane) {
  f32x4 ws[4];
#pragma unroll
  for (int nt = 0; nt < 4; ++nt) ws[nt] = *reinterpret_cast<const f32x4*>(p.w_scale + min(n_base + nt * 16 + (lane >> 4) * 4, p.N - 4));
#pragma unroll
  for (int mt = 0; mt < MT; ++mt) {
    const float sa = p.a_scale[min(m_base + mt * 16 + (lane & 15), p.M - 1) / p.rows_per_seg];
#pragma unroll
    for (int nt = 0; nt < 4; ++nt)
#pragma unroll
      for (int j = 0; j < 4; ++j) acc[mt][nt][j] = acc[mt][nt][j] * (sa * ws[nt][j]);
  }
}

template <int EPI>
__device__ __forceinline__ bf16x4 epi_apply(const GemmP& p, const f32x4& a4, int m, int n, const bf16_t* e0row) {
  float y[4];
#pragma unroll
  for (int j = 0; j < 4; ++j) y[j] = a4[j];
  if (p.bias) {
    const bf16x4 b = *reinterpret_cast<const bf16x4*>(p.bias + n);
#pragma unroll
    for (int j = 0; j < 4; ++j) y[j] += (float)b[j];
  }
  if (EPI == SF_EPI_BIAS_GELU) {
#pragma unroll
    for (int j = 0; j < 4; ++j) y[j] = gelu_tanh_f(y[j]);
  }
  if (EPI == SF_EPI_BIAS_GATE_RESID) {
    const bf16x4 gm = *reinterpret_cast<const bf16x4*>(p.gate_mod + n);
    const bf16x4 ge = *reinterpret_cast<const bf16x4*>(e0row + n);
#pragma unroll
    for (int j = 0; j < 4; ++j) y[j] *= (float)(bf16_t)((float)gm[j] + (float)ge[j]);
  }
  if (EPI == SF_EPI_BIAS_RESID || EPI == SF_EPI_BIAS_GATE_RESID) {
    const bf16x4 rv = *reinterpret_cast<const bf16x4*>(p.resid + (long)m * p.ldr + n);
#pragma unroll
    for (int j = 0; j < 4; ++j) y[j] += (float)rv[j];
  }
  bf16x4 o;
#pragma unroll
  for (int j = 0; j < 4; ++j) o[j] = (bf16_t)y[j];
  return o;
}

template <int EPI, int MT>
__device__ __forceinline__ void gemm_epilogue(const GemmP& p, f32x4 (&acc)[MT][4], int mrow, int ncol) {
#pragma unroll
  for (int mt = 0; mt < MT; ++mt) {
    const int m = mrow + mt * 16;
    if (m >= p.M) continue;
    const bf16_t* e0row = nullptr;
    if (EPI == SF_EPI_BIAS_GATE_RESID) e0row = p.gate_e0 + (long)(m / p.rows_per_group) * p.gate_group_stride;
#pragma unroll
    for (int nt = 0; nt < 4; ++nt) {
      const int n = ncol + nt * 16;
      if (n >= p.N) continue;
      if (EPI == SF_EPI_F32) {
        *reinterpret_cast<f32x4*>(reinterpret_cast<float*>(p.out) + (long)m * p.ldo + n) = acc[mt][nt];
        continue;
      }
      *reinterpret_cast<bf16x4*>(p.out + (long)m * p.ldo + n) = epi_apply<EPI>(p, acc[mt][nt], m, n, e0row);
    }
  }
}

template <int EPI>
__device__ __forceinline__ bf16x4 epi_math(const f32x4& a4, const bf16x4& b, const bf16x4& gm, const bf16x4& ge, const bf16x4& rv) {
  float y[4];
#pragma unroll
  for (int j = 0; j < 4; ++j) y[j] = a4[j] + (float)b[j];
  if (EPI == SF_EPI_BIAS_GELU) {
#pragma unroll
    for (int j = 0; j < 4; ++j) y[j] = gelu_tanh_f(y[j]);
  }
  if (EPI == SF_EPI_BIAS_GATE_RESID) {
#pragma unroll
    for (int j = 0; j < 4; ++j) y[j] *= (float)(bf16_t)((float)gm[j] + (float)ge[j]);
  }
  if (EPI == SF_EPI_BIAS_RESID || EPI == SF_EPI_BIAS_GATE_RESID) {
#pragma unroll
    for (int j = 0; j < 4; ++j) y[j] += (float)rv[j];
  }
  bf16x4 o;
#pragma unroll
  for (int j = 0; j < 4; ++j) o[j] = (bf16_t)y[j];
  return o;
}

template <int EPI, int MT>
__device__ __forceinline__ void gemm_epilogue_lds(const GemmP& p, f32x4 (&acc)[MT][4], int m_base, int n_base, char* wbuf, int lane) {
  const int r16 = lane & 15, cg = lane >> 4;
  constexpr bool GATE = EPI == SF_EPI_BIAS_GATE_RESID;
  constexpr bool RESID = EPI == SF_EPI_BIAS_RESID || EPI == SF_EPI_BIAS_GATE_RESID;
  const bf16x4 zero4 = {(bf16_t)0.f, (bf16_t)0.f, (bf16_t)0.f, (bf16_t)0.f};
  int ncol[4];
  bf16x4 bias_v[4], gm_v[4];
#pragma unroll
  for (int nt = 0; nt < 4; ++nt) {
    ncol[nt] = min(n_base + nt * 16 + cg * 4, p.N - 4);
    bias_v[nt] = zero4;
    gm_v[nt] = zero4;
  }
  if (p.bias) {
#pragma unroll
    for (int nt = 0; nt < 4; ++nt) bias_v[nt] = *reinterpret_cast<const bf16x4*>(p.bias + ncol[nt]);
  }
  if (GATE) {
#pragma unroll
    for (int nt = 0; nt < 4; ++nt) gm_v[nt] = *reinterpret_cast<const bf16x4*>(p.gate_mod + ncol[nt]);
  }
  constexpr int MB = 4;
#pragma unroll
  for (int m0 = 0; m0 < MT; m0 += MB) {
    bf16x4 rv[MB][4], ge[MB][4];
#pragma unroll
    for (int i = 0; i < MB; ++i) {
      if (m0 + i >= MT) break;
      const int m = min(m_base + (m0 + i) * 16 + r16, p.M - 1);
      const bf16_t* e0row = GATE ? p.gate_e0 + (long)(m / p.rows_per_group) * p.gate_group_stride : nullptr;
#pragma unroll
      for (int nt = 0; nt < 4; ++nt) {
        rv[i][nt] = RESID ? *reinterpret_cast<const bf16x4*>(p.resid + (long)m * p.ldr + ncol[nt]) : zero4;
        ge[i][nt] = GATE ? *reinterpret_cast<const bf16x4*>(e0row + ncol[nt]) : zero4;
      }
    }
#pragma unroll
    for (int i = 0; i < MB; ++i) {
      if (m0 + i >= MT) break;
      const int row = (m0 + i) * 16 + r16;
#pragma unroll
      for (int nt = 0; nt < 4; ++nt) {
        const int col = nt * 16 + cg * 4;
        const bf16x4 o = epi_math<EPI>(acc[m0 + i][nt], bias_v[nt], gm_v[nt], ge[i][nt], rv[i][nt]);
        const int chunk = (col >> 3) ^ (row & 7);
        *reinterpret_cast<bf16x4*>(wbuf + row * 128 + (chunk << 4) + (col & 4) * 2) = o;
      }
    }
  }
  __builtin_amdgcn_s_waitcnt(0xc07f);
  const int rr = lane >> 3, ch = lane & 7;
#pragma unroll
  for (int i = 0; i < 2 * MT; ++i) {
    const int row = i * 8 + rr;
    const int m = m_base + row, n = n_base + ch * 8;
    const bf16x8 v = *reinterpret_cast<const bf16x8*>(wbuf + row * 128 + ((ch ^ (row & 7)) << 4));
    if (m < p.M && n < p.N) *reinterpret_cast<bf16x8*>(p.out + (long)m * p.ldo + n) = v;
  }
}

template <int EPI, bool F8>
__global__ __launch_bounds__(GEMM_THREADS, 2) void gemm_bf16_kernel(GemmP p) {
  extern __shared__ __attribute__((aligned(16))) char smem[];
  const int tid = threadIdx.x;
  const int lane = tid & 63;
  const int wave = __builtin_amdgcn_readfirstlane(tid >> 6);

  if (blockIdx.y) {
    const long bz = blockIdx.y;
    p.a += bz * p.a_bs; p.w += bz * p.w_bs;
    if (EPI == SF_EPI_F32) p.out = reinterpret_cast<bf16_t*>(reinterpret_cast<float*>(p.out) + bz * p.o_bs); else p.out += bz * p.o_bs;
    if (p.resid) p.resid += bz * p.r_bs;
  }
  const int nwg = gridDim.x, bid = blockIdx.x;
  const int wg = sf_xcd_remap(bid, nwg);
  constexpr int GROUP_M = 8;
  const int width = GROUP_M * p.tiles_n;
  const int group = wg / width, first_m = group * GROUP_M;
  const int gsz = min(p.tiles_m - first_m, GROUP_M);
  const int in_group = wg - group * width;
  const int tm = first_m + in_group % gsz, tn = in_group / gsz;
  const int m0 = tm * BM, n0 = tn * BN;

  const bf16_t* a_src[4];
  const bf16_t* w_src[4];
#pragma unroll
  for (int i = 0; i < 4; ++i) {
    const int r = (wave * 4 + i) * 8 + (lane >> 3);
    const int c = (lane & 7) ^ ((r >> 1) & 7);
    const int am = min(m0 + r, p.M - 1);
    const int wn = min(n0 + r, p.N - 1);
    a_src[i] = p.a + (long)am * p.lda + c * 8;
    w_src[i] = p.w + (long)wn * p.ldw + c * 8;
  }
  auto stage = [&](int buf, int kt) {
    char* base = smem + buf * STAGE_BYTES + wave * 4096;
    const int k0 = kt * BK;
#pragma unroll
    for (int i = 0; i < 4; ++i) glds16(a_src[i] + k0, base + i * 1024);
#pragma unroll
    for (int i = 0; i < 4; ++i) glds16(w_src[i] + k0, base + TILE_BYTES + i * 1024);
  };

  const int wr = wave >> 1, wc = wave & 1;
  const int i16 = lane & 15, kq = lane >> 4;
  const int swz = (i16 >> 1) & 7;
  const int x_row_off = (wr * 64 + i16) * 128;
  const int w_row_off = TILE_BYTES + (wc * 64 + i16) * 128;
  const int coff0 = ((0 + kq) ^ swz) << 4;
  const int coff1 = ((4 + kq) ^ swz) << 4;

  f32x4 acc[4][4];
#pragma unroll
  for (int i = 0; i < 4; ++i)
#pragma unroll
    for (int j = 0; j < 4; ++j) acc[i][j] = f32x4{0.f, 0.f, 0.f, 0.f};

  const int nk = p.K / BK;
  stage(0, 0);
  __builtin_amdgcn_s_waitcnt(0);
  __syncthreads();

  for (int kt = 0; kt < nk; ++kt) {
    const int cur = kt & 1;
    const char* buf = smem + cur * STAGE_BYTES;
    const int kn = min(kt + 1, nk - 1) * BK;
    char* sbase = smem + (cur ^ 1) * STAGE_BYTES + wave * 4096;
    bf16x8 xf0[4], wf0[4], xf1[4], wf1[4];
    if constexpr (F8) {
#pragma unroll
      for (int t = 0; t < 4; ++t) {
        xf0[t] = *reinterpret_cast<const bf16x8*>(buf + x_row_off + t * 2048 + coff0);
        wf0[t] = *reinterpret_cast<const bf16x8*>(buf + w_row_off + t * 2048 + coff0);
        xf1[t] = *reinterpret_cast<const bf16x8*>(buf + x_row_off + t * 2048 + coff1);
        wf1[t] = *reinterpret_cast<const bf16x8*>(buf + w_row_off + t * 2048 + coff1);
      }
      __builtin_amdgcn_sched_barrier(0);
#pragma unroll
      for (int i = 0; i < 8; ++i) {
        const int mt = i >> 1, nt0 = (i & 1) * 2;
        acc[mt][nt0] = mfma_f8(wf0[nt0], wf1[nt0], xf0[mt], xf1[mt], acc[mt][nt0]);
        acc[mt][nt0 + 1] = mfma_f8(wf0[nt0 + 1], wf1[nt0 + 1], xf0[mt], xf1[mt], acc[mt][nt0 + 1]);
        if (i < 4) glds16(a_src[i] + kn, sbase + i * 1024);
        else glds16(w_src[i - 4] + kn, sbase + TILE_BYTES + (i - 4) * 1024);
        __builtin_amdgcn_sched_barrier(0);
      }
      __syncthreads();
      continue;
    }
#pragma unroll
    for (int t = 0; t < 4; ++t) {
      xf0[t] = *reinterpret_cast<const bf16x8*>(buf + x_row_off + t * 2048 + coff0);
      wf0[t] = *reinterpret_cast<const bf16x8*>(buf + w_row_off + t * 2048 + coff0);
    }
    __builtin_amdgcn_sched_barrier(0);
#pragma unroll
    for (int i = 0; i < 8; ++i) {
      const int mt = i >> 1, nt0 = (i & 1) * 2;
      acc[mt][nt0] = __builtin_amdgcn_mfma_f32_16x16x32_bf16(wf0[nt0], xf0[mt], acc[mt][nt0], 0, 0, 0);
      acc[mt][nt0 + 1] = __builtin_amdgcn_mfma_f32_16x16x32_bf16(wf0[nt0 + 1], xf0[mt], acc[mt][nt0 + 1], 0, 0, 0);
      if (i < 4) {
        xf1[i] = *reinterpret_cast<const bf16x8*>(buf + x_row_off + i * 2048 + coff1);
        glds16(a_src[i] + kn, sbase + i * 1024);
      } else {
        wf1[i - 4] = *reinterpret_cast<const bf16x8*>(buf + w_row_off + (i - 4) * 2048 + coff1);
        glds16(w_src[i - 4] + kn, sbase + TILE_BYTES + (i - 4) * 1024);
      }
      __builtin_amdgcn_sched_barrier(0);
    }
#pragma unroll
    for (int mt = 0; mt < 4; ++mt)
#pragma unroll
      for (int nt = 0; nt < 4; ++nt)
        acc[mt][nt] = __builtin_amdgcn_mfma_f32_16x16x32_bf16(wf1[nt], xf1[mt], acc[mt][nt], 0, 0, 0);
    __builtin_amdgcn_sched_barrier(0);
    __syncthreads();
  }

  if constexpr (F8) fp8_scale_acc<4>(p, acc, m0 + wr * 64, n0 + wc * 64, lane);
  const int mrow = m0 + wr * 64 + (lane & 15);
  const int ncol = n0 + wc * 64 + (lane >> 4) * 4;
  if (EPI != SF_EPI_F32 && (p.N & 7) == 0 && (p.ldo & 7) == 0)
    gemm_epilogue_lds<EPI, 4>(p, acc, m0 + wr * 64, n0 + wc * 64, smem + wave * 8192, lane);
  else
    gemm_epilogue<EPI, 4>(p, acc, mrow, ncol);
}


constexpr int PP_THREADS = 512;

template <int MT>
struct PPCfg {
  static constexpr int BM = 32 * MT;
  static constexpr int A_BYTES = BM * 128;
  static constexpr int B_BYTES = 256 * 128;
  static constexpr int STAGE = A_BYTES + B_BYTES;
  static constexpr int LDS = 2 * STAGE;
  static constexpr int PA = (2 * MT + 7) / 8;
};

template <int EPI, int MT, bool F8>
__global__ __launch_bounds__(PP_THREADS) void gemm_pp_kernel(GemmP p) {
  using Cfg = PPCfg<MT>;
  constexpr int BMp = Cfg::BM, PA = Cfg::PA;
  constexpr int HQA = (MT + 1) / 2, HQB = MT / 2;
  extern __shared__ __attribute__((aligned(16))) char smem[];
  const int tid = threadIdx.x;
  const int lane = tid & 63;
  const int wave = __builtin_amdgcn_readfirstlane(tid >> 6);
  const int grp = wave >> 2, wc = wave & 3;

  const int nwg = gridDim.x, bid = blockIdx.x;
  const int wg = sf_xcd_remap(bid, nwg);
  constexpr int GROUP_M = MT >= 6 ? 4 : 8;
  const int width = GROUP_M * p.tiles_n;
  const int group = wg / width, first_m = group * GROUP_M;
  const int gsz = min(p.tiles_m - first_m, GROUP_M);
  const int in_group = wg - group * width;
  const int tm = first_m + in_group % gsz, tn = in_group / gsz;
  const int m0 = tm * BMp, n0 = tn * 256;

  const bf16_t* a_src[2][PA];
  const bf16_t* w_src[2][2];
#pragma unroll
  for (int h = 0; h < 2; ++h) {
#pragma unroll
    for (int i = 0; i < PA; ++i) {
      const int r = h * (BMp / 2) + (wave + 8 * i) * 8 + (lane >> 3);
      const int c = (lane & 7) ^ ((r >> 1) & 7);
      a_src[h][i] = p.a + (long)min(m0 + r, p.M - 1) * p.lda + c * 8;
    }
#pragma unroll
    for (int i = 0; i < 2; ++i) {
      const int r = h * 128 + (wave + 8 * i) * 8 + (lane >> 3);
      const int c = (lane & 7) ^ ((r >> 1) & 7);
      w_src[h][i] = p.w + (long)min(n0 + r, p.N - 1) * p.ldw + c * 8;
    }
  }
  auto dma_a = [&](int h, int kt) {
    char* base = smem + (kt & 1) * Cfg::STAGE + h * (Cfg::A_BYTES / 2) + wave * 1024;
#pragma unroll
    for (int i = 0; i < PA; ++i)
      if (wave + 8 * i < 2 * MT) glds16(a_src[h][i] + kt * BK, base + i * 8192);
  };
  auto dma_b = [&](int h, int kt) {
    char* base = smem + (kt & 1) * Cfg::STAGE + Cfg::A_BYTES + h * (Cfg::B_BYTES / 2) + wave * 1024;
#pragma unroll
    for (int i = 0; i < 2; ++i) glds16(w_src[h][i] + kt * BK, base + i * 8192);
  };

  const int i16 = lane & 15, kq = lane >> 4;
  const int swz = (i16 >> 1) & 7;
  const int x_row_off = (grp * (BMp / 2) + i16) * 128;
  const int w_row_off = Cfg::A_BYTES + (wc * 64 + i16) * 128;
  const int coff[2] = {((0 + kq) ^ swz) << 4, ((4 + kq) ^ swz) << 4};

  f32x4 acc[MT][4];
#pragma unroll
  for (int i = 0; i < MT; ++i)
#pragma unroll
    for (int j = 0; j < 4; ++j) acc[i][j] = f32x4{0.f, 0.f, 0.f, 0.f};
  bf16x8 af[HQA][2], bfr[4][2];

#ifdef SF_STAMP
  unsigned long long* stamp = (EPI == SF_EPI_BIAS && p.gate_e0) ? reinterpret_cast<unsigned long long*>(const_cast<bf16_t*>(p.gate_e0)) + ((long)bid * 2 + grp) * 8 : nullptr;
  if (stamp && (tid & 255) == 0) { stamp[0] = __builtin_amdgcn_s_memtime(); stamp[4] = __builtin_amdgcn_s_memrealtime(); }
#endif
  const int nk = p.K / BK;
  dma_a(0, 0); dma_a(1, 0); dma_b(0, 0); dma_b(1, 0);
  if (nk > 1) { dma_b(0, 1); dma_b(1, 1); asm volatile("s_waitcnt vmcnt(4)" ::: "memory"); }
  else asm volatile("s_waitcnt vmcnt(0)" ::: "memory");
  __builtin_amdgcn_s_barrier();
#ifdef SF_STAMP
  if (stamp && (tid & 255) == 0) stamp[1] = __builtin_amdgcn_s_memtime();
#endif
  if (grp == 1) __builtin_amdgcn_s_barrier();

  auto end_load_segment = [&]() {
    __builtin_amdgcn_s_waitcnt(0xc07f);
    __builtin_amdgcn_sched_barrier(0);
    __builtin_amdgcn_s_barrier();
    __builtin_amdgcn_sched_barrier(0);
  };
  auto cluster = [&](auto qc, int c0) {
    constexpr int q = decltype(qc)::value, NQ = q == 0 ? HQA : HQB;
    __builtin_amdgcn_s_setprio(1);
    if constexpr (F8) {
#pragma unroll
      for (int mt = 0; mt < NQ; ++mt)
#pragma unroll
        for (int nt = 0; nt < 2; ++nt)
          acc[q * HQA + mt][c0 + nt] = mfma_f8(bfr[c0 + nt][0], bfr[c0 + nt][1], af[mt][0], af[mt][1], acc[q * HQA + mt][c0 + nt]);
    } else {
#pragma unroll
      for (int ks = 0; ks < 2; ++ks)
#pragma unroll
        for (int mt = 0; mt < NQ; ++mt)
#pragma unroll
          for (int nt = 0; nt < 2; ++nt)
            acc[q * HQA + mt][c0 + nt] = __builtin_amdgcn_mfma_f32_16x16x32_bf16(bfr[c0 + nt][ks], af[mt][ks], acc[q * HQA + mt][c0 + nt], 0, 0, 0);
    }
    __builtin_amdgcn_s_setprio(0);
    __builtin_amdgcn_sched_barrier(0);
    __builtin_amdgcn_s_barrier();
    __builtin_amdgcn_sched_barrier(0);
  };
  auto read_a = [&](const char* buf, auto qc) {
    constexpr int q = decltype(qc)::value, NQ = q == 0 ? HQA : HQB;
#pragma unroll
    for (int mt = 0; mt < NQ; ++mt)
#pragma unroll
      for (int ks = 0; ks < 2; ++ks)
        af[mt][ks] = *reinterpret_cast<const bf16x8*>(buf + x_row_off + (q * HQA + mt) * 2048 + coff[ks]);
  };
  auto read_b = [&](const char* buf, int c0) {
#pragma unroll
    for (int nt = 0; nt < 2; ++nt)
#pragma unroll
      for (int ks = 0; ks < 2; ++ks)
        bfr[c0 + nt][ks] = *reinterpret_cast<const bf16x8*>(buf + w_row_off + (c0 + nt) * 2048 + coff[ks]);
  };

  constexpr std::integral_constant<int, 0> Q0{};
  constexpr std::integral_constant<int, 1> Q1{};
  for (int kt = 0; kt < nk; ++kt) {
    const char* buf = smem + (kt & 1) * Cfg::STAGE;
    const bool more1 = kt + 1 < nk, more2 = kt + 2 < nk;
    read_a(buf, Q0);
    read_b(buf, 0);
    if (more1) dma_a(0, kt + 1);
    end_load_segment();
    cluster(Q0, 0);
    read_b(buf, 2);
    if (more1) dma_a(1, kt + 1);
    end_load_segment();
    cluster(Q0, 2);
    read_a(buf, Q1);
    if (more2) dma_b(0, kt + 2);
    end_load_segment();
    cluster(Q1, 2);
    if (more2) {
      dma_b(1, kt + 2);
      asm volatile("s_waitcnt vmcnt(4)" ::: "memory");
    } else {
      asm volatile("s_waitcnt vmcnt(0)" ::: "memory");
    }
    end_load_segment();
    cluster(Q1, 0);
  }
  if (grp == 0) __builtin_amdgcn_s_barrier();
#ifdef SF_STAMP
  if (stamp && (tid & 255) == 0) stamp[2] = __builtin_amdgcn_s_memtime();
#endif

  const int m_base = m0 + grp * (BMp / 2), n_base = n0 + wc * 64;
  if constexpr (F8) fp8_scale_acc<MT>(p, acc, m_base, n_base, lane);
  if ((p.N & 7) == 0 && (p.ldo & 7) == 0)
    gemm_epilogue_lds<EPI, MT>(p, acc, m_base, n_base, smem + wave * (MT * 2048), lane);
  else
    gemm_epilogue<EPI, MT>(p, acc, m_base + (lane & 15), n_base + (lane >> 4) * 4);
#ifdef SF_STAMP
  asm volatile("s_waitcnt vmcnt(0)" ::: "memory");
  if (stamp && (tid & 255) == 0) { stamp[3] = __builtin_amdgcn_s_memtime(); stamp[5] = __builtin_amdgcn_s_memrealtime(); }
#endif
}

constexpr int PP2_A = 128 * 128, PP2_B = 256 * 128;
constexpr int PP2_LDS = 3 * (PP2_A + PP2_B);

template <int EPI, bool F8>
__global__ __launch_bounds__(PP_THREADS) void gemm_pp2_kernel(GemmP p) {
  extern __shared__ __attribute__((aligned(16))) char smem[];
  const int tid = threadIdx.x;
  const int lane = tid & 63;
  const int wave = __builtin_amdgcn_readfirstlane(tid >> 6);
  const int grp = wave >> 2, wc = wave & 3;

  const int nwg = gridDim.x, bid = blockIdx.x;
  const int wg = sf_xcd_remap(bid, nwg);
  constexpr int GROUP_M = 8;
  const int width = GROUP_M * p.tiles_n;
  const int group = wg / width, first_m = group * GROUP_M;
  const int gsz = min(p.tiles_m - first_m, GROUP_M);
  const int in_group = wg - group * width;
  const int tm = first_m + in_group % gsz, tn = in_group / gsz;
  const int m0 = tm * 128, n0 = tn * 256;

  const bf16_t* a_src[2];
  const bf16_t* w_src[4];
#pragma unroll
  for (int i = 0; i < 2; ++i) {
    const int r = (wave + 8 * i) * 8 + (lane >> 3);
    a_src[i] = p.a + (long)min(m0 + r, p.M - 1) * p.lda + ((lane & 7) ^ ((r >> 1) & 7)) * 8;
  }
#pragma unroll
  for (int i = 0; i < 4; ++i) {
    const int r = (wave + 8 * i) * 8 + (lane >> 3);
    w_src[i] = p.w + (long)min(n0 + r, p.N - 1) * p.ldw + ((lane & 7) ^ ((r >> 1) & 7)) * 8;
  }
  auto dma_a = [&](int slot, int kt) {
    char* base = smem + slot * PP2_A + wave * 1024;
#pragma unroll
    for (int i = 0; i < 2; ++i) glds16(a_src[i] + kt * BK, base + i * 8192);
  };
  auto dma_b = [&](int slot, int kt) {
    char* base = smem + 3 * PP2_A + slot * PP2_B + wave * 1024;
#pragma unroll
    for (int i = 0; i < 4; ++i) glds16(w_src[i] + kt * BK, base + i * 8192);
  };

  const int i16 = lane & 15, kq = lane >> 4;
  const int swz = (i16 >> 1) & 7;
  const int x_row_off = (grp * 64 + i16) * 128;
  const int w_row_off = 3 * PP2_A + (wc * 64 + i16) * 128;
  const int coff[2] = {((0 + kq) ^ swz) << 4, ((4 + kq) ^ swz) << 4};

  f32x4 acc[4][4];
#pragma unroll
  for (int i = 0; i < 4; ++i)
#pragma unroll
    for (int j = 0; j < 4; ++j) acc[i][j] = f32x4{0.f, 0.f, 0.f, 0.f};
  bf16x8 af[4][2], bfr[4][2];

  const int nk = p.K / BK;
  dma_a(0, 0); dma_b(0, 0);
  if (nk > 1) { dma_a(1, 1); dma_b(1, 1); asm volatile("s_waitcnt vmcnt(6)" ::: "memory"); }
  else asm volatile("s_waitcnt vmcnt(0)" ::: "memory");
  __builtin_amdgcn_s_barrier();
  if (grp == 1) __builtin_amdgcn_s_barrier();

  auto end_load_segment = [&]() {
    __builtin_amdgcn_s_waitcnt(0xc07f);
    __builtin_amdgcn_sched_barrier(0);
    __builtin_amdgcn_s_barrier();
    __builtin_amdgcn_sched_barrier(0);
  };
  auto cluster = [&](int c0) {
    __builtin_amdgcn_s_setprio(1);
    if constexpr (F8) {
#pragma unroll
      for (int mt = 0; mt < 4; ++mt)
#pragma unroll
        for (int nt = 0; nt < 2; ++nt)
          acc[mt][c0 + nt] = mfma_f8(bfr[c0 + nt][0], bfr[c0 + nt][1], af[mt][0], af[mt][1], acc[mt][c0 + nt]);
    } else {
#pragma unroll
      for (int ks = 0; ks < 2; ++ks)
#pragma unroll
        for (int mt = 0; mt < 4; ++mt)
#pragma unroll
          for (int nt = 0; nt < 2; ++nt)
            acc[mt][c0 + nt] = __builtin_amdgcn_mfma_f32_16x16x32_bf16(bfr[c0 + nt][ks], af[mt][ks], acc[mt][c0 + nt], 0, 0, 0);
    }
    __builtin_amdgcn_s_setprio(0);
    __builtin_amdgcn_sched_barrier(0);
    __builtin_amdgcn_s_barrier();
    __builtin_amdgcn_sched_barrier(0);
  };

  int slot = 0;
  for (int kt = 0; kt < nk; ++kt) {
    const char* abuf = smem + slot * PP2_A;
    const char* bbuf = smem + slot * PP2_B;
    const int nslot = slot == 0 ? 2 : slot - 1;
    const bool more2 = kt + 2 < nk;
#pragma unroll
    for (int mt = 0; mt < 4; ++mt)
#pragma unroll
      for (int ks = 0; ks < 2; ++ks) af[mt][ks] = *reinterpret_cast<const bf16x8*>(abuf + x_row_off + mt * 2048 + coff[ks]);
#pragma unroll
    for (int nt = 0; nt < 2; ++nt)
#pragma unroll
      for (int ks = 0; ks < 2; ++ks) bfr[nt][ks] = *reinterpret_cast<const bf16x8*>(bbuf + w_row_off + nt * 2048 + coff[ks]);
    if (more2) dma_a(nslot, kt + 2);
    end_load_segment();
    cluster(0);
#pragma unroll
    for (int nt = 2; nt < 4; ++nt)
#pragma unroll
      for (int ks = 0; ks < 2; ++ks) bfr[nt][ks] = *reinterpret_cast<const bf16x8*>(bbuf + w_row_off + nt * 2048 + coff[ks]);
    if (more2) {
      dma_b(nslot, kt + 2);
      asm volatile("s_waitcnt vmcnt(6)" ::: "memory");
    } else {
      asm volatile("s_waitcnt vmcnt(0)" ::: "memory");
    }
    end_load_segment();
    cluster(2);
    slot = slot == 2 ? 0 : slot + 1;
  }
  if (grp == 0) __builtin_amdgcn_s_barrier();

  const int m_base = m0 + grp * 64, n_base = n0 + wc * 64;
  if constexpr (F8) fp8_scale_acc<4>(p, acc, m_base, n_base, lane);
  if ((p.N & 7) == 0 && (p.ldo & 7) == 0)
    gemm_epilogue_lds<EPI, 4>(p, acc, m_base, n_base, smem + wave * 8192, lane);
  else
    gemm_epilogue<EPI, 4>(p, acc, m_base + (lane & 15), n_base + (lane >> 4) * 4);
}

template <int EPI, bool F8>
int launch_pp2(GemmP& p, hipStream_t s) {
  static bool attr = false;
  if (!attr) {
    (void)hipFuncSetAttribute(reinterpret_cast<const void*>(&gemm_pp2_kernel<EPI, F8>), hipFuncAttributeMaxDynamicSharedMemorySize, PP2_LDS);
    attr = true;
  }
  p.tiles_m = (p.M + 127) / 128;
  p.tiles_n = (p.N + 255) / 256;
  hipLaunchKernelGGL((gemm_pp2_kernel<EPI, F8>), dim3(p.tiles_m * p.tiles_n), dim3(PP_THREADS), PP2_LDS, s, p);
  return 0;
}

template <bool F8>
int launch_pp2_epi(GemmP& p, int epilogue, hipStream_t s) {
  switch (epilogue) {
    case SF_EPI_BIAS: return launch_pp2<SF_EPI_BIAS, F8>(p, s);
    case SF_EPI_BIAS_GELU: return launch_pp2<SF_EPI_BIAS_GELU, F8>(p, s);
    case SF_EPI_BIAS_RESID: return launch_pp2<SF_EPI_BIAS_RESID, F8>(p, s);
    case SF_EPI_BIAS_GATE_RESID: return launch_pp2<SF_EPI_BIAS_GATE_RESID, F8>(p, s);
    default: return -1;
  }
}

template <int EPI, int MT, bool F8>
int launch_pp(GemmP& p, hipStream_t s) {
  using Cfg = PPCfg<MT>;
  static bool attr = false;
  if (!attr) {
    (void)hipFuncSetAttribute(reinterpret_cast<const void*>(&gemm_pp_kernel<EPI, MT, F8>), hipFuncAttributeMaxDynamicSharedMemorySize, Cfg::LDS);
    attr = true;
  }
  p.tiles_m = (p.M + Cfg::BM - 1) / Cfg::BM;
  p.tiles_n = (p.N + 255) / 256;
  hipLaunchKernelGGL((gemm_pp_kernel<EPI, MT, F8>), dim3(p.tiles_m * p.tiles_n), dim3(PP_THREADS), Cfg::LDS, s, p);
  return 0;
}

template <int MT, bool F8>
int launch_pp_epi(GemmP& p, int epilogue, hipStream_t s) {
  switch (epilogue) {
    case SF_EPI_BIAS: return launch_pp<SF_EPI_BIAS, MT, F8>(p, s);
    case SF_EPI_BIAS_GELU: return launch_pp<SF_EPI_BIAS_GELU, MT, F8>(p, s);
    case SF_EPI_BIAS_RESID: return launch_pp<SF_EPI_BIAS_RESID, MT, F8>(p, s);
    case SF_EPI_BIAS_GATE_RESID: return launch_pp<SF_EPI_BIAS_GATE_RESID, MT, F8>(p, s);
    default: return -1;
  }
}

int check_args(const sf_gemm_args* a, const char* name, int bk) {
  SF_CHECK(a != nullptr, "%s: null args", name);
  SF_CHECK(a->M > 0 && a->N > 0 && a->K > 0, "%s: empty problem M=%d N=%d K=%d", name, a->M, a->N, a->K);
  SF_CHECK(a->K % bk == 0, "%s: K=%d must be a multiple of %d", name, a->K, bk);
  SF_CHECK(a->N % 4 == 0, "%s: N=%d must be a multiple of 4", name, a->N);
  SF_CHECK(a->lda % (bk / 8) == 0 && a->ldw % (bk / 8) == 0 && a->ldo % 4 == 0, "%s: lda/ldw must be multiples of %d, ldo of 4", name, bk / 8);
  SF_CHECK(a->lda >= a->K && a->ldw >= a->K && a->ldo >= a->N, "%s: leading dimension too small", name);
  SF_CHECK(a->a && a->w && a->out, "%s: null tensor", name);
  SF_CHECK(((uintptr_t)a->a % 16 == 0) && ((uintptr_t)a->w % 16 == 0) && ((uintptr_t)a->out % 8 == 0), "%s: misaligned tensor", name);
  if (a->epilogue == SF_EPI_BIAS_RESID || a->epilogue == SF_EPI_BIAS_GATE_RESID) {
    SF_CHECK(a->resid != nullptr && a->ldr >= a->N && a->ldr % 4 == 0, "%s: residual epilogue needs resid/ldr", name);
  }
  if (a->epilogue == SF_EPI_BIAS_GATE_RESID) {
    SF_CHECK(a->gate_mod && a->gate_e0 && a->rows_per_group > 0, "%s: gate epilogue needs gate_mod/gate_e0/rows_per_group", name);
  }
  SF_CHECK(a->structure >= SF_GEMM_AUTO && a->structure <= SF_GEMM_PP192, "%s: unknown structure %d", name, a->structure);
  return 0;
}

template <bool F8>
int run_gemm(const sf_gemm_args* a, GemmP& p, const char* name, hipStream_t s) {
  int st = a->structure;
  const int nk = p.K / BK;
  const bool pp_ok = a->batch <= 1 && a->epilogue != SF_EPI_F32 && nk >= 2;
  if (st == SF_GEMM_AUTO) {
    st = SF_GEMM_T128;
    if (pp_ok && a->M >= 1024 && a->N >= 1024 && a->K >= 512) {
      static const struct { int st, rows; double rel; } cand[] = {
          {SF_GEMM_PP256, 256, 1.00}, {SF_GEMM_PP224, 224, 1.02}, {SF_GEMM_PP192, 192, 1.05}, {SF_GEMM_PP128, 128, 1.14}};
      const long tn = (a->N + 255) / 256;
      double best = 1e30;
      for (const auto& c : cand) {
        const long tiles = (long)((a->M + c.rows - 1) / c.rows) * tn;
        const double cost = (double)((tiles + 255) / 256) * (c.rows / 256.0 * c.rel + 0.04);
        if (cost < best - 1e-9) { best = cost; st = c.st; }
      }
    }
  }
  const bool is_pp = st == SF_GEMM_PP256 || st == SF_GEMM_PP224 || st == SF_GEMM_PP192 || st == SF_GEMM_PP128;
  if (is_pp && !pp_ok) st = SF_GEMM_T128;
  else if (is_pp) {
    const int rc = st == SF_GEMM_PP256 ? launch_pp_epi<8, F8>(p, a->epilogue, s)
                 : st == SF_GEMM_PP224 ? launch_pp_epi<7, F8>(p, a->epilogue, s)
                 : st == SF_GEMM_PP192 ? launch_pp_epi<6, F8>(p, a->epilogue, s) : launch_pp2_epi<F8>(p, a->epilogue, s);
    SF_CHECK(rc == 0, "%s: unknown epilogue %d", name, a->epilogue);
    SF_HIP_LAUNCH_CHECK(name);
    return 0;
  }
  const int batch = a->batch > 1 ? a->batch : 1;
  p.a_bs = a->a_bstride; p.w_bs = a->w_bstride; p.o_bs = a->o_bstride; p.r_bs = a->r_bstride;
  SF_CHECK(batch == 1 || (a->a_bstride % 8 == 0 && a->w_bstride % 8 == 0 && a->o_bstride % 4 == 0 && a->r_bstride % 4 == 0),
           "%s: batch strides must keep 16-byte (operands) / 8-byte (output) alignment", name);
  const dim3 grid(p.tiles_m * p.tiles_n, batch), block(GEMM_THREADS);
  switch (a->epilogue) {
    case SF_EPI_BIAS: hipLaunchKernelGGL((gemm_bf16_kernel<SF_EPI_BIAS, F8>), grid, block, GEMM_LDS, s, p); break;
    case SF_EPI_BIAS_GELU: hipLaunchKernelGGL((gemm_bf16_kernel<SF_EPI_BIAS_GELU, F8>), grid, block, GEMM_LDS, s, p); break;
    case SF_EPI_BIAS_RESID: hipLaunchKernelGGL((gemm_bf16_kernel<SF_EPI_BIAS_RESID, F8>), grid, block, GEMM_LDS, s, p); break;
    case SF_EPI_BIAS_GATE_RESID: hipLaunchKernelGGL((gemm_bf16_kernel<SF_EPI_BIAS_GATE_RESID, F8>), grid, block, GEMM_LDS, s, p); break;
    case SF_EPI_F32:
      if constexpr (F8) {
        SF_CHECK(false, "%s: the raw fp32 epilogue is bf16-only", name);
      } else {
        SF_CHECK((uintptr_t)a->out % 16 == 0, "%s: fp32 output must be 16-byte aligned", name);
        hipLaunchKernelGGL((gemm_bf16_kernel<SF_EPI_F32, false>), grid, block, GEMM_LDS, s, p);
      }
      break;
    default: SF_CHECK(false, "%s: unknown epilogue %d", name, a->epilogue);
  }
  SF_HIP_LAUNCH_CHECK(name);
  return 0;
}

void fill_params(const sf_gemm_args* a, GemmP& p, int unit) {
  p.a = (const bf16_t*)a->a; p.w = (const bf16_t*)a->w; p.bias = (const bf16_t*)a->bias;
  p.out = (bf16_t*)a->out; p.resid = (const bf16_t*)a->resid;
  p.gate_mod = (const bf16_t*)a->gate_mod; p.gate_e0 = (const bf16_t*)a->gate_e0;
  p.gate_group_stride = a->gate_group_stride; p.rows_per_group = a->rows_per_group;
  p.M = a->M; p.N = a->N; p.K = a->K / unit; p.lda = a->lda / unit; p.ldw = a->ldw / unit; p.ldo = a->ldo; p.ldr = a->ldr;
  p.tiles_n = (a->N + BN - 1) / BN;
  p.tiles_m = (a->M + BM - 1) / BM;
  p.a_scale = nullptr; p.w_scale = nullptr; p.rows_per_seg = 1;
}

}

extern "C" int sf_gemm_bf16(const sf_gemm_args* a, void* stream) {
  if (const int rc = check_args(a, "sf_gemm_bf16", BK)) return rc;
  GemmP p;
  fill_params(a, p, 1);
  return run_gemm<false>(a, p, "sf_gemm_bf16", (hipStream_t)stream);
}

extern "C" int sf_gemm_fp8(const sf_gemm_args* a, const float* a_scale, int rows_per_segment, const float* w_scale, void* stream) {
  if (const int rc = check_args(a, "sf_gemm_fp8", 2 * BK)) return rc;
  SF_CHECK(a->batch <= 1, "sf_gemm_fp8: batched products are bf16-only");
  SF_CHECK(a_scale && w_scale && rows_per_segment > 0, "sf_gemm_fp8: needs a_scale, w_scale and rows_per_segment > 0");
  SF_CHECK((uintptr_t)w_scale % 16 == 0, "sf_gemm_fp8: w_scale must be 16-byte aligned");
  GemmP p;
  fill_params(a, p, 2);
  p.a_scale = a_scale; p.w_scale = w_scale; p.rows_per_seg = rows_per_segment;
  return run_gemm<true>(a, p, "sf_gemm_fp8", (hipStream_t)stream);
}
```

self-forcing_amd/csrc/sf_host.h:

```cpp
#pragma once
#include <cstring>
#include "sf_common.h"
#include "../../include/sf_hip.h"

#define SF_TRY(expr)            \
  do {                          \
    int rc__ = (expr);          \
    if (rc__ != 0) return rc__; \
  } while (0)

inline int sf_hip_ok(hipError_t e, const char* who, const char* what) {
  SF_CHECK(e == hipSuccess, "%s: %s failed: %s", who, what, hipGetErrorString(e));
  return 0;
}

struct Carve {
  char* base;
  size_t off;
  explicit Carve(void* p) : base((char*)p), off(0) {}
  char* take(size_t bytes) {
    char* r = base ? base + off : nullptr;
    off += (bytes + 255) & ~(size_t)255;
    return r;
  }
};

struct Gemm {
  sf_gemm_args g;
  const void* wq = nullptr;
  const float* w_scale = nullptr;
  int rows_per_segment = 0;
  Gemm(const void* a, int lda, const void* w, int ldw, void* out, int ldo, int M, int N, int K) {
    memset(&g, 0, sizeof(g));
    g.a = a; g.lda = lda; g.w = w; g.ldw = ldw; g.out = out; g.ldo = ldo; g.M = M; g.N = N; g.K = K;
    g.epilogue = SF_EPI_BIAS;
    g.rows_per_group = 1;
  }
  Gemm& bias(const void* b) { g.bias = b; return *this; }
  Gemm& epi(int e) { g.epilogue = e; return *this; }
  Gemm& resid(const void* r, int ldr) { g.resid = r; g.ldr = ldr; return *this; }
  Gemm& gate(const void* gate_mod, const void* gate_e0, long group_stride, int rows_per_group) {
    g.gate_mod = gate_mod; g.gate_e0 = gate_e0; g.gate_group_stride = group_stride; g.rows_per_group = rows_per_group;
    return *this;
  }
  Gemm& batch(int n, long a_bstride, long w_bstride, long o_bstride) {
    g.batch = n; g.a_bstride = a_bstride; g.w_bstride = w_bstride; g.o_bstride = o_bstride;
    return *this;
  }
  Gemm& fp8w(const void* w_e4m3, const float* scale, int rows_per_seg) {
    wq = w_e4m3; w_scale = scale; rows_per_segment = rows_per_seg;
    return *this;
  }
  int bf16(void* stream) const { return sf_gemm_bf16(&g, stream); }
  int fp8(const void* aq, const float* a_scale, void* stream) const {
    sf_gemm_args q = g;
    q.a = aq; q.lda = g.K; q.w = wq;
    return sf_gemm_fp8(&q, a_scale, rows_per_segment, w_scale, stream);
  }
};
```

self-forcing_amd/model.py:

```python
from __future__ import annotations

import ctypes as C
from typing import Dict, List, Optional

import torch

from . import _lib, fp8 as fp8_recipe, torch_ops
from .device_model import DeviceModel
from .kvcache import CachePlan
from .weights import WanShape, param_shapes

Tensor = torch.Tensor


def rope_tables(head_dim: int, max_pos: int = 1024, theta: float = 10000.0):
    d = head_dim
    parts = []
    for dim in (d - 4 * (d // 6), 2 * (d // 6), 2 * (d // 6)):
        inv = 1.0 / torch.pow(torch.tensor(theta, dtype=torch.float64),
                              torch.arange(0, dim, 2, dtype=torch.float64) / dim)
        parts.append(torch.arange(max_pos, dtype=torch.float64)[:, None] * inv[None, :])
    ang = torch.cat(parts, dim=1)
    return ang.cos().float().contiguous(), ang.sin().float().contiguous()


class CausalWanModel(DeviceModel):

    def __init__(self, shape: WanShape, state_dict: Dict[str, Tensor], device, sched_sigmas: Tensor,
                 sched_timesteps: Tensor, fp8: bool = False):
        if shape.head_dim != 128:
            raise ValueError(f"head_dim must be 128 (dim={shape.dim}, heads={shape.num_heads})")
        if tuple(shape.patch_size) != (1, 2, 2):
            raise ValueError("only patch_size (1, 2, 2) is supported")
        super().__init__(device)
        self.shape = shape
        self.dim, self.num_heads, self.num_layers = shape.dim, shape.num_heads, shape.num_layers
        self.local_attn_size = shape.local_attn_size
        self.sink_size = shape.sink_size
        self.num_frame_per_block = 1
        self.independent_first_frame = False
        self.fp8 = bool(fp8)
        self.fp8_weights: Dict[str, tuple] = {}
        self._load(state_dict, sched_sigmas, sched_timesteps)
        self._handle = torch_ops.register_model(self)

    def _dev8(self, name: str, parts: List[Tensor]):
        q, s = fp8_recipe.quantize_weight([p.detach().to(device=self.device, dtype=torch.bfloat16) for p in parts])
        self._keep += [q, s]
        self.fp8_weights[name] = (q, s)
        return C.c_void_p(q.data_ptr()), C.c_void_p(s.data_ptr())

    def _load(self, sd: Dict[str, Tensor], sigmas: Tensor, timesteps: Tensor) -> None:
        self._check_state_dict(sd, param_shapes(self.shape), "state dict")
        s = self.shape
        if self.fp8:
            for name, k in (("text_embedding.0", s.text_dim), ("the dim-wide Linears", s.dim), ("ffn.2", s.ffn_dim)):
                fp8_recipe.check_k(name, k)
            if "pose_proj.weight" in sd:
                fp8_recipe.check_k("pose_proj", sd["pose_proj.weight"].shape[1])
        m = _lib.Model()
        m.fp8 = int(self.fp8)
        m.dim, m.ffn_dim, m.num_heads, m.num_layers = s.dim, s.ffn_dim, s.num_heads, s.num_layers
        m.in_dim, m.out_dim, m.freq_dim, m.text_dim, m.text_len = s.in_dim, s.out_dim, s.freq_dim, s.text_dim, s.text_len
        m.eps = s.eps
        P = lambda t: C.c_void_p(t.data_ptr())
        m.patch_w = P(self._dev(sd["patch_embedding.weight"].flatten(1)))
        m.patch_b = P(self._dev(sd["patch_embedding.bias"]))
        for dst, src in (("text0", "text_embedding.0"), ("text2", "text_embedding.2"), ("time0", "time_embedding.0"),
                         ("time2", "time_embedding.2"), ("tproj", "time_projection.1"), ("head", "head.head")):
            if self.fp8:
                q8, s8 = self._dev8(src, [sd[src + ".weight"]])
                setattr(m, dst + "_q", q8)
                setattr(m, dst + "_s", s8)
            else:
                setattr(m, dst + "_w", P(self._dev(sd[src + ".weight"])))
            setattr(m, dst + "_b", P(self._dev(sd[src + ".bias"])))
        m.head_mod = P(self._dev(sd["head.modulation"].reshape(2, s.dim)))
        from .weights import POSE_DIM
        self.has_pose_proj = "pose_proj.weight" in sd
        if self.has_pose_proj:
            if self.fp8:
                m.pose_q, m.pose_s = self._dev8("pose_proj", [sd["pose_proj.weight"]])
            else:
                m.pose_w = P(self._dev(sd["pose_proj.weight"]))
            m.pose_b = P(self._dev(sd["pose_proj.bias"]))
            m.pose_dim = sd["pose_proj.weight"].shape[1]
        elif s.dim == POSE_DIM:
            m.pose_dim = s.dim
        self.accepts_pose = self.has_pose_proj or s.dim == POSE_DIM
        layers = (_lib.LayerWeights * s.num_layers)()
        layers8 = (_lib.LayerFp8 * s.num_layers)()
        for i in range(s.num_layers):
            p = f"blocks.{i}."
            lw = layers[i]
            if self.fp8:
                for dst, srcs in _lib.FP8_LAYER_LINEARS:
                    q8, s8 = self._dev8(p + dst, [sd[p + src + ".weight"] for src in srcs])
                    setattr(layers8[i], dst + "_q", q8)
                    setattr(layers8[i], dst + "_s", s8)
            lw.modulation = P(self._dev(sd[p + "modulation"].reshape(6, s.dim)))
            lw.norm3_w, lw.norm3_b = P(self._dev(sd[p + "norm3.weight"])), P(self._dev(sd[p + "norm3.bias"]))
            sa, ca = p + "self_attn.", p + "cross_attn."
            W = (lambda t: None) if self.fp8 else (lambda t: P(self._dev(t)))
            lw.qkv_w = W(torch.cat([sd[sa + "q.weight"], sd[sa + "k.weight"], sd[sa + "v.weight"]], 0))
            lw.qkv_b = P(self._dev(torch.cat([sd[sa + "q.bias"], sd[sa + "k.bias"], sd[sa + "v.bias"]], 0)))
            lw.norm_q_w, lw.norm_k_w = P(self._dev(sd[sa + "norm_q.weight"])), P(self._dev(sd[sa + "norm_k.weight"]))
            lw.o_w, lw.o_b = W(sd[sa + "o.weight"]), P(self._dev(sd[sa + "o.bias"]))
            lw.cq_w, lw.cq_b = W(sd[ca + "q.weight"]), P(self._dev(sd[ca + "q.bias"]))
            lw.ckv_w = W(torch.cat([sd[ca + "k.weight"], sd[ca + "v.weight"]], 0))
            lw.ckv_b = P(self._dev(torch.cat([sd[ca + "k.bias"], sd[ca + "v.bias"]], 0)))
            lw.cnorm_q_w, lw.cnorm_k_w = P(self._dev(sd[ca + "norm_q.weight"])), P(self._dev(sd[ca + "norm_k.weight"]))
            lw.co_w, lw.co_b = W(sd[ca + "o.weight"]), P(self._dev(sd[ca + "o.bias"]))
            lw.ffn0_w, lw.ffn0_b = W(sd[p + "ffn.0.weight"]), P(self._dev(sd[p + "ffn.0.bias"]))
            lw.ffn2_w, lw.ffn2_b = W(sd[p + "ffn.2.weight"]), P(self._dev(sd[p + "ffn.2.bias"]))
        self._layers = layers
        m.layers_host = C.cast(layers, C.POINTER(_lib.LayerWeights))
        if self.fp8:
            self._layers8 = layers8
            m.layers_fp8_host = C.cast(layers8, C.POINTER(_lib.LayerFp8))
        cos, sin = rope_tables(s.head_dim)
        self.rope_cos = cos.to(self.device)
        self.rope_sin = sin.to(self.device)
        self.sched_sigmas = sigmas.to(device=self.device, dtype=torch.float32).contiguous()
        self.sched_timesteps = timesteps.to(device=self.device, dtype=torch.float32).contiguous()
        m.rope_cos, m.rope_sin = self.rope_cos.data_ptr(), self.rope_sin.data_ptr()
        m.sched_sigmas, m.sched_timesteps = self.sched_sigmas.data_ptr(), self.sched_timesteps.data_ptr()
        m.n_table = self.sched_sigmas.numel()
        self.cmodel = m

    def workspace(self, B: int, F: int, H: int, W: int, G: int) -> Tensor:
        return self._stream_bytes((B, F, H, W, G), lambda: _lib.lib().sf_dit_workspace_bytes(C.byref(self.cmodel), B, F, H, W, G))

    def forward(self, noisy: Tensor, timestep: Tensor, prompt_embeds: Optional[Tensor], init_cross: bool,
                k_cache: List[Tensor], v_cache: List[Tensor], ck_cache: List[Tensor], cv_cache: List[Tensor], plan: CachePlan,
                start_frame: int, evict_scratch: Optional[Tensor] = None, cache_only: bool = False,
                add_condition: Optional[Tensor] = None, kv_index: Optional[Tensor] = None):
        B, F, Cin, H, W = noisy.shape
        ws = self.workspace(B, F, H, W, timestep.shape[1])
        flow, x0 = torch.ops.sf_hip.dit_forward(
            self._handle, noisy, timestep, prompt_embeds, add_condition, k_cache, v_cache, ck_cache, cv_cache, ws, evict_scratch,
            bool(init_cross), bool(cache_only), plan.sink, plan.evict, plan.keep, plan.write_start, plan.attn_start, plan.local_end,
            start_frame, kv_index, plan.global_end)
        return (None, None) if cache_only else (flow, x0)

    def forward_pair(self, ctx_noisy: Tensor, ctx_timestep: Tensor, noisy: Tensor, timestep: Tensor, k_cache: List[Tensor],
                     v_cache: List[Tensor], ck_cache: List[Tensor], cv_cache: List[Tensor], ctx_plan: CachePlan, plan: CachePlan,
                     ctx_start_frame: int, start_frame: int, evict_scratch: Optional[Tensor] = None, kv_index: Optional[Tensor] = None):
        B, F, Cin, H, W = noisy.shape
        ws = self.workspace(2 * B, F, H, W, timestep.shape[1])
        as_list = lambda pl, sf: [pl.sink, pl.evict, pl.keep, pl.write_start, pl.attn_start, pl.local_end, sf]
        return torch.ops.sf_hip.dit_forward_pair(self._handle, ctx_noisy, ctx_timestep, noisy, timestep, k_cache, v_cache, ck_cache, cv_cache,
                                                 ws, evict_scratch, as_list(ctx_plan, ctx_start_frame), as_list(plan, start_frame), kv_index,
                                                 plan.global_end)
```

self-forcing_amd/ops.py:

```python
from __future__ import annotations

import ctypes as C
from typing import Optional

import torch

from . import _lib
from . import torch_ops
from ._lib import (ACT_GELU, ACT_NONE, ACT_SILU, CONV_BIAS, CONV_BIAS_CLAMP_F32, CONV_BIAS_RESID, EPI_BIAS,
                   EPI_BIAS_GATE_RESID, EPI_BIAS_GELU, EPI_BIAS_RESID, EPI_F32, ConvArgs, GemmArgs, check, lib)

Tensor = torch.Tensor
_EPI = {"bias": EPI_BIAS, "gelu": EPI_BIAS_GELU, "resid": EPI_BIAS_RESID, "gate_resid": EPI_BIAS_GATE_RESID,
        "f32": EPI_F32}
_ACT = {None: ACT_NONE, "none": ACT_NONE, "silu": ACT_SILU, "gelu": ACT_GELU}


def stream_handle() -> int:
    return torch.cuda.current_stream().cuda_stream


def _bf16(t: Tensor, name: str) -> Tensor:
    if not t.is_cuda:
        raise ValueError(f"{name}: expected a CUDA/ROCm tensor (the HIP path has no CPU fallback)")
    if t.dtype != torch.bfloat16:
        raise ValueError(f"{name}: expected bfloat16, got {t.dtype}")
    return t


def _rows(t: Tensor, name: str, dtype=torch.bfloat16) -> Tensor:
    if not t.is_cuda:
        raise ValueError(f"{name}: expected a CUDA/ROCm tensor (the HIP path has no CPU fallback)")
    if t.dtype != dtype:
        raise ValueError(f"{name}: expected {dtype}, got {t.dtype}")
    if t.dim() != 2 or t.stride(1) != 1:
        raise ValueError(f"{name}: expected a 2-D tensor with contiguous rows, got shape {tuple(t.shape)} strides {t.stride()}")
    return t


def _ptr(t: Optional[Tensor]) -> Optional[int]:
    return None if t is None else t.data_ptr()


def _timestep(t: Tensor):
    if t.dtype == torch.int64:
        return t.contiguous(), 1
    return t.to(torch.float32).contiguous(), 0


def gemm(a: Tensor, w: Tensor, bias: Optional[Tensor] = None, epilogue: str = "bias",
         resid: Optional[Tensor] = None, gate_mod: Optional[Tensor] = None, gate_e0: Optional[Tensor] = None,
         rows_per_group: int = 1, out: Optional[Tensor] = None, structure: str = "auto") -> Tensor:
    a, w = _rows(a, "a"), _rows(w, "w")
    epi, st = _EPI[epilogue], _lib.GEMM_STRUCTURES[structure]
    if out is None:
        return torch.ops.sf_hip.gemm(a, w, bias, epi, resid, gate_mod, gate_e0, rows_per_group, st)
    torch.ops.sf_hip.gemm_out(out, a, w, bias, epi, resid, gate_mod, gate_e0, rows_per_group, st)
    return out


def small_linear(x: Tensor, w: Tensor, bias: Optional[Tensor], act_in=None, act_out=None) -> Tensor:
    x, w = _rows(x, "x").contiguous(), _rows(w, "w").contiguous()
    M, K = x.shape
    N = w.shape[0]
    out = torch.empty(M, N, dtype=torch.bfloat16, device=x.device)
    check(lib().sf_small_linear(x.data_ptr(), w.data_ptr(), _ptr(bias), out.data_ptr(), M, N, K,
                                _ACT[act_in], _ACT[act_out], stream_handle()), "sf_small_linear")
    return out


def quantize_fp8(x: Tensor, rows_per_segment: Optional[int] = None):
    x = _rows(x, "x")
    return torch.ops.sf_hip.quantize_fp8(x, rows_per_segment or x.shape[0])


def gemm_fp8(a: Tensor, a_scale: Tensor, w: Tensor, w_scale: Tensor, bias: Optional[Tensor] = None, epilogue: str = "bias",
             resid: Optional[Tensor] = None, gate_mod: Optional[Tensor] = None, gate_e0: Optional[Tensor] = None,
             rows_per_group: int = 1, rows_per_segment: Optional[int] = None, structure: str = "auto") -> Tensor:
    a, w = _rows(a, "a", torch.float8_e4m3fn), _rows(w, "w", torch.float8_e4m3fn)
    if w_scale.numel() == 1:
        w_scale = w_scale.reshape(1).expand(w.shape[0])
    return torch.ops.sf_hip.gemm_fp8(a, a_scale.float().contiguous(), rows_per_segment or a.shape[0], w, w_scale.float().contiguous(), bias,
                                     _EPI[epilogue], resid, gate_mod, gate_e0, rows_per_group, _lib.GEMM_STRUCTURES[structure])


def small_linear_fp8(x: Tensor, w_q: Tensor, w_scale: Tensor, bias: Optional[Tensor], act_in=None, act_out=None,
                     rows_per_segment: Optional[int] = None) -> Tensor:
    x, w_q = _rows(x, "x").contiguous(), _rows(w_q, "w_q", torch.float8_e4m3fn).contiguous()
    M, K = x.shape
    N = w_q.shape[0]
    w_scale = (w_scale.reshape(1).expand(N) if w_scale.numel() == 1 else w_scale).float().contiguous()
    out = torch.empty(M, N, dtype=torch.bfloat16, device=x.device)
    check(lib().sf_small_linear_fp8(x.data_ptr(), w_q.data_ptr(), w_scale.data_ptr(), _ptr(bias), out.data_ptr(), M, N, K,
                                    rows_per_segment or M, _ACT[act_in], _ACT[act_out], stream_handle()), "sf_small_linear_fp8")
    return out


def sinusoid_embedding(t: Tensor, dim: int) -> Tensor:
    tt, is64 = _timestep(t.flatten())
    out = torch.empty(tt.numel(), dim, dtype=torch.bfloat16, device=t.device)
    check(lib().sf_sinusoid_embedding(tt.data_ptr(), is64, out.data_ptr(), tt.numel(), dim, stream_handle()),
          "sf_sinusoid_embedding")
    return out


def layernorm_modulate(x: Tensor, mod_shift: Tensor, mod_scale: Tensor, e0_shift: Tensor, e0_scale: Tensor,
                       rows_per_group: int, eps: float = 1e-6) -> Tensor:
    x = _rows(x, "x").contiguous()
    M, Cc = x.shape
    _rows(e0_shift, "e0_shift"), _rows(e0_scale, "e0_scale")
    if e0_shift.stride(0) != e0_scale.stride(0):
        raise ValueError("layernorm_modulate: e0_shift / e0_scale must share a row stride")
    out = torch.empty_like(x)
    check(lib().sf_layernorm_modulate(x.data_ptr(), out.data_ptr(), M, Cc, eps, mod_shift.data_ptr(), mod_scale.data_ptr(),
                                      e0_shift.data_ptr(), e0_scale.data_ptr(), e0_shift.stride(0), rows_per_group,
                                      stream_handle()), "sf_layernorm_modulate")
    return out


def layernorm_affine(x: Tensor, weight: Tensor, bias: Tensor, eps: float = 1e-6) -> Tensor:
    x = _rows(x, "x").contiguous()
    out = torch.empty_like(x)
    check(lib().sf_layernorm_affine(x.data_ptr(), weight.data_ptr(), bias.data_ptr(), out.data_ptr(), x.shape[0], x.shape[1],
                                    eps, stream_handle()), "sf_layernorm_affine")
    return out


def rmsnorm(x: Tensor, weight: Tensor, eps: float = 1e-6, out: Optional[Tensor] = None) -> Tensor:
    x = _rows(x, "x")
    if out is None:
        out = torch.empty(x.shape, dtype=torch.bfloat16, device=x.device)
    check(lib().sf_rmsnorm(x.data_ptr(), x.stride(0), weight.data_ptr(), out.data_ptr(), out.stride(0), x.shape[0], x.shape[1],
                           eps, stream_handle()), "sf_rmsnorm")
    return out


def qkv_norm_rope_cache(qkv: Tensor, norm_q_w: Tensor, norm_k_w: Tensor, k_cache: Tensor, v_cache: Tensor,
                        rope_cos: Tensor, rope_sin: Tensor, grid, write_start: int, start_frame: int,
                        eps: float = 1e-6) -> Tensor:
    qkv = _rows(qkv, "qkv").contiguous()
    B, S, H, D = k_cache.shape
    f, h, w = grid
    Cc = H * D
    if not (k_cache.is_contiguous() and v_cache.is_contiguous()):
        raise ValueError("qkv_norm_rope_cache: caches must be contiguous [B, S, H, D]")
    q = torch.empty(qkv.shape[0], Cc, dtype=torch.bfloat16, device=qkv.device)
    check(lib().sf_qkv_norm_rope_cache(qkv.data_ptr(), norm_q_w.data_ptr(), norm_k_w.data_ptr(), q.data_ptr(), k_cache.data_ptr(),
                                       v_cache.data_ptr(), rope_cos.data_ptr(), rope_sin.data_ptr(), B, f, h, w, Cc, H, S,
                                       write_start, start_frame, eps, stream_handle()), "sf_qkv_norm_rope_cache")
    return q


def kv_evict(cache: Tensor, sink: int, evict: int, keep: int, scratch: Tensor) -> None:
    B, S, H, D = cache.shape
    check(lib().sf_kv_evict(cache.data_ptr(), B, S, H * D, sink, evict, keep, scratch.data_ptr(),
                            scratch.numel() * scratch.element_size(), stream_handle()), "sf_kv_evict")


def attention(q: Tensor, k: Tensor, v: Tensor, structure: str = "auto") -> Tensor:
    return torch.ops.sf_hip.attention(q, k, v, _lib.ATTN_STRUCTURES[structure])


def patchify(x: Tensor) -> Tensor:
    x = _bf16(x, "x").contiguous()
    B, F, Cin, H, W = x.shape
    out = torch.empty(B * F * (H // 2) * (W // 2), Cin * 4, dtype=torch.bfloat16, device=x.device)
    check(lib().sf_patchify(x.data_ptr(), out.data_ptr(), B, F, Cin, H, W, stream_handle()), "sf_patchify")
    return out


def unpatchify_x0(head_out: Tensor, xt: Tensor, timestep: Tensor, sigmas: Tensor, timesteps: Tensor):
    xt = _bf16(xt, "xt").contiguous()
    B, F, Cout, H, W = xt.shape
    tt, is64 = _timestep(timestep)
    G = tt.shape[1]
    flow = torch.empty_like(xt)
    x0 = torch.empty_like(xt)
    check(lib().sf_unpatchify_x0(_rows(head_out, "head_out").contiguous().data_ptr(), xt.data_ptr(), tt.data_ptr(), is64,
                                 sigmas.data_ptr(), timesteps.data_ptr(), sigmas.numel(), flow.data_ptr(), x0.data_ptr(),
                                 B, F, G, Cout, H, W, stream_handle()), "sf_unpatchify_x0")
    return flow, x0


def add_noise(x0: Tensor, eps: Tensor, timestep: Tensor, sigmas: Tensor, timesteps: Tensor) -> Tensor:
    x0 = _bf16(x0, "x0").contiguous()
    eps = _bf16(eps, "eps").contiguous()
    tt, _ = _timestep(timestep.flatten())
    if tt.numel() != x0.shape[0]:
        raise ValueError(f"add_noise: {x0.shape[0]} samples but {tt.numel()} timesteps")
    return torch.ops.sf_hip.add_noise(x0, eps, tt, sigmas, timesteps)


LINCOMB_MAX = 6


def lincomb(tensors, coefs, out: Optional[Tensor] = None) -> Tensor:
    if not 1 <= len(tensors) <= LINCOMB_MAX or len(tensors) != len(coefs):
        raise ValueError(f"lincomb: 1..{LINCOMB_MAX} tensors with one coefficient each, got {len(tensors)} / {len(coefs)}")
    xs = [_bf16(t, f"tensors[{i}]").contiguous() for i, t in enumerate(tensors)]
    cf = [float(c) for c in coefs]
    if out is None:
        return torch.ops.sf_hip.lincomb(xs, cf)
    torch.ops.sf_hip.lincomb_out(out, xs, cf)
    return out


def conv_igemm(x: Tensor, w_packed: Tensor, bias: Tensor, kernel, t_out: int, upsample: bool = False,
               t_in_offset: int = 0, resid: Optional[Tensor] = None, interleave: bool = False,
               clamp_f32: bool = False, cin: Optional[int] = None, structure: str = "auto", stride=(1, 1)) -> Tensor:
    _bf16(x, "x"), _bf16(w_packed, "w_packed"), _bf16(bias, "bias")
    if x.dim() != 4 or not x.is_contiguous():
        raise ValueError("conv_igemm: x must be a contiguous [T, H, W, C] volume")
    tin, hin, win, c = x.shape
    kt, kh, kw = kernel
    cout = w_packed.shape[0]
    st, sh = stride
    H, W = (2 * hin, 2 * win) if upsample else (hin // 2, win // 2) if sh == 2 else (hin, win)
    if st * (t_out - 1) + kt + t_in_offset > tin:
        raise ValueError(f"conv_igemm: {tin} input frames do not cover {t_out} output frames (kt={kt}, offset={t_in_offset})")
    a = ConvArgs()
    a.x, a.w, a.bias = x.data_ptr(), w_packed.data_ptr(), bias.data_ptr()
    a.Tout, a.H, a.W, a.Hin, a.Win = t_out, H, W, hin, win
    a.Cin, a.Cout, a.kt, a.kh, a.kw = cin or c, cout, kt, kh, kw
    a.upsample, a.t_in_offset, a.ldw = int(upsample), t_in_offset, w_packed.stride(0)
    a.structure = _lib.CONV_STRUCTURES[structure]
    a.stride_t, a.stride_hw = st, sh
    if clamp_f32:
        out = torch.empty(t_out, cout, H, W, dtype=torch.float32, device=x.device)
        a.out_f32, a.epilogue = out.data_ptr(), CONV_BIAS_CLAMP_F32
    else:
        co = cout // 2 if interleave else cout
        out = torch.empty(2 * t_out if interleave else t_out, H, W, co, dtype=torch.bfloat16, device=x.device)
        a.out, a.ldo, a.epilogue = out.data_ptr(), co, CONV_BIAS
        a.interleave_c = co if interleave else 0
        if resid is not None:
            _bf16(resid, "resid")
            if tuple(resid.shape) != tuple(out.shape) or not resid.is_contiguous():
                raise ValueError("conv_igemm: resid must match the output volume")
            a.resid, a.ldr, a.epilogue = resid.data_ptr(), cout, CONV_BIAS_RESID
    check(lib().sf_conv_igemm(a, stream_handle()), "sf_conv_igemm")
    return out


def taehv_conv(x: Tensor, w_packed: Tensor, bias: Optional[Tensor], kt: int, t_out: int, epilogue: str = "bias_relu", upsample: bool = False,
               resid: Optional[Tensor] = None, tgrow: int = 1, clamp: bool = False, cin: Optional[int] = None) -> Tensor:
    _bf16(x, "x"), _bf16(w_packed, "w_packed")
    if bias is not None:
        _bf16(bias, "bias")
    if x.dim() != 4 or not x.is_contiguous():
        raise ValueError("taehv_conv: x must be a contiguous [T, H, W, C] volume")
    if epilogue not in _lib.TAEHV_EPILOGUES:
        raise ValueError(f"taehv_conv: unknown epilogue {epilogue!r}")
    tin, hin, win, c = x.shape
    if t_out - 1 + kt > tin:
        raise ValueError(f"taehv_conv: {tin} input frames do not cover {t_out} output frames (kt={kt})")
    cout = w_packed.shape[0]
    H, W = (2 * hin, 2 * win) if upsample else (hin, win)
    a = _lib.TaehvConvArgs()
    a.x, a.w, a.bias = x.data_ptr(), w_packed.data_ptr(), None if bias is None else bias.data_ptr()
    a.Tout, a.H, a.W, a.Cin, a.Cout, a.kt = t_out, H, W, cin or c, cout, kt
    a.upsample, a.ldw, a.tgrow, a.epilogue, a.clamp = int(upsample), w_packed.stride(0), tgrow, _lib.TAEHV_EPILOGUES[epilogue], int(clamp)
    if epilogue == "head_f32":
        out = torch.empty(t_out, cout, H, W, dtype=torch.float32, device=x.device)
        a.out_f32 = out.data_ptr()
    else:
        if tgrow < 1 or cout % tgrow:
            raise ValueError(f"taehv_conv: tgrow={tgrow} does not divide Cout={cout}")
        co = cout // tgrow
        out = torch.empty(tgrow * t_out, H, W, co, dtype=torch.bfloat16, device=x.device)
        a.out, a.ldo = out.data_ptr(), co
        if resid is not None:
            _bf16(resid, "resid")
            if tuple(resid.shape) != tuple(out.shape) or not resid.is_contiguous():
                raise ValueError("taehv_conv: resid must match the output volume")
            a.resid, a.ldr = resid.data_ptr(), cout
    check(lib().sf_taehv_conv(a, stream_handle()), "sf_taehv_conv")
    return out


def pose_prepare(src: Tensor, lead: int = 3, hwc: bool = False) -> Tensor:
    if not src.is_cuda:
        raise ValueError("pose_prepare: expected a CUDA/ROCm tensor (the HIP path has no CPU fallback)")
    name = str(src.dtype).replace("torch.", "")
    if name not in _lib.POSE_DTYPES:
        raise ValueError(f"pose_prepare: pose data must be uint8, float32 or bfloat16, got {src.dtype}")
    if hwc:
        if src.dim() != 3 or src.shape[2] != 3:
            raise ValueError(f"pose_prepare: expected an image [H, W, 3], got {tuple(src.shape)}")
        F, (H, W) = 1, src.shape[:2]
    else:
        if src.dim() != 4 or src.shape[0] != 3:
            raise ValueError(f"pose_prepare: expected pose frames [3, F, H, W], got {tuple(src.shape)}")
        F, H, W = src.shape[1:]
    src = src.contiguous()
    out = torch.empty(lead + F, H, W, 8, dtype=torch.bfloat16, device=src.device)
    check(lib().sf_pose_prepare(src.data_ptr(), _lib.POSE_DTYPES[name], int(hwc), F, H, W, lead, out.data_ptr(), stream_handle()), "sf_pose_prepare")
    return out


def pose_conv(x: Tensor, w_packed: Tensor, bias: Tensor, cout: int, kt: int = 3, stride_t: int = 1, stride_s: int = 1, silu: bool = True) -> Tensor:
    _bf16(x, "x"), _bf16(w_packed, "w_packed")
# ... 99 lines not shown
```

self-forcing_amd/torch_ops.py:

```python
from __future__ import annotations

import ctypes as C
import threading
import time
import weakref
from typing import Dict, List, Optional, Sequence, Tuple

import torch
from torch.library import custom_op

from . import _lib

Tensor = torch.Tensor
NAMESPACE = "sf_hip"

_MODELS: "weakref.WeakValueDictionary[int, object]" = weakref.WeakValueDictionary()


def register_model(obj) -> int:
    h = id(obj)
    _MODELS[h] = obj
    return h


# ... 163 lines not shown
    for i, t in enumerate(tensors):
        _need_gpu(t, f"tensors[{i}]")
        if not t.is_contiguous() or t.shape != tensors[0].shape or t.device != tensors[0].device:
            raise ValueError("lincomb: tensors must be contiguous and share shape and device")
    if out.shape != tensors[0].shape or out.dtype != torch.bfloat16 or not out.is_contiguous():
        raise ValueError("lincomb: out must be a contiguous bf16 tensor of the inputs' shape")
    ptrs = (C.c_void_p * n)(*[t.data_ptr() for t in tensors])
    cf = (C.c_float * n)(*[float(c) for c in coefs])
    _lib.check(_lib.lib().sf_lincomb_bf16(out.data_ptr(), ptrs, cf, n, tensors[0].numel(), _stream(out)), "sf_lincomb_bf16")


@custom_op(f"{NAMESPACE}::lincomb", mutates_args=())
def lincomb(tensors: List[Tensor], coefs: List[float]) -> Tensor:
    if not tensors:
        raise ValueError("lincomb: 1..6 tensors with one coefficient each, got 0")
    out = torch.empty_like(tensors[0], memory_format=torch.contiguous_format)
    _lincomb_launch(out, tensors, coefs)
    return out


@lincomb.register_fake
def _(tensors, coefs):
    return torch.empty_like(tensors[0])


@custom_op(f"{NAMESPACE}::lincomb_out", mutates_args=("out",))
def lincomb_out(out: Tensor, tensors: List[Tensor], coefs: List[float]) -> None:
    _lincomb_launch(out, tensors, coefs)


@custom_op(f"{NAMESPACE}::add_noise", mutates_args=())
def add_noise(x0: Tensor, eps: Tensor, timestep: Tensor, sigmas: Tensor, timesteps: Tensor) -> Tensor:
    _need_gpu(x0, "x0"), _need_gpu(eps, "eps"), _need_gpu(sigmas, "sigmas", torch.float32), _need_gpu(timesteps, "timesteps", torch.float32)
    if not (x0.is_contiguous() and eps.is_contiguous() and timestep.is_contiguous()):
        raise ValueError("add_noise: contiguous tensors expected")
    n = x0.shape[0]
    if timestep.numel() != n or timestep.dtype not in (torch.float32, torch.int64):
        raise ValueError(f"add_noise: {n} samples need {n} float32 / int64 timesteps, got {timestep.numel()} of {timestep.dtype}")
    out = torch.empty_like(eps)
    _lib.check(_lib.lib().sf_add_noise(x0.data_ptr(), eps.data_ptr(), timestep.data_ptr(), int(timestep.dtype == torch.int64),
                                       sigmas.data_ptr(), timesteps.data_ptr(), sigmas.numel(), out.data_ptr(), n, x0.numel() // n,
                                       _stream(x0)), "sf_add_noise")
    return out


@add_noise.register_fake
def _(x0, eps, timestep, sigmas, timesteps):
    return torch.empty_like(eps)


_TABLES: Dict[int, tuple] = {}

HOST_ENQUEUE: Dict[int, list] = {}


def host_enqueue_stats(reset: bool = False):
    calls = sum(v[0] for v in HOST_ENQUEUE.values())
    wall = sum(v[1] for v in HOST_ENQUEUE.values())
    cpu = sum(v[2] for v in HOST_ENQUEUE.values())
    n = sum(1 for v in HOST_ENQUEUE.values() if v[0])
    if reset:
        HOST_ENQUEUE.clear()
    return calls, wall, cpu, n


def _pointer_tables(handle: int, k: Sequence[Tensor], v: Sequence[Tensor], ck: Sequence[Tensor], cv: Sequence[Tensor],
                    want_kv: tuple, want_cross: tuple, device):
    key = (want_kv, want_cross) + tuple(t.data_ptr() for t in k) + tuple(t.data_ptr() for t in v) + tuple(t.data_ptr() for t in ck) \
        + tuple(t.data_ptr() for t in cv)
    slot = (handle, torch.cuda.current_stream(device).cuda_stream)
    hit = _TABLES.get(slot)
    if hit is not None and hit[0] == key:
        return hit[1]
    for name, tensors, want in (("k_cache", k, want_kv), ("v_cache", v, want_kv), ("ck_cache", ck, want_cross), ("cv_cache", cv, want_cross)):
        for i, t in enumerate(tensors):
            if not t.is_cuda or t.dtype != torch.bfloat16 or tuple(t.shape) != want or not t.is_contiguous() or t.device != device:
                raise ValueError(f"dit_forward: {name}[{i}] must be a contiguous bf16 tensor {want} on {device}, got "
                                 f"{tuple(t.shape)} {t.dtype} {t.device}")
    arr = lambda ts: (C.c_void_p * len(ts))(*[t.data_ptr() for t in ts])
    tabs = (arr(k), arr(v), arr(ck), arr(cv))
    if len(_TABLES) > 64:
        _TABLES.clear()
    _TABLES[slot] = (key, tabs)
    return tabs


def _forward_args(m, model: int, noisy: Tensor, timestep: Tensor, prompt_embeds: Optional[Tensor], add_condition: Optional[Tensor],
                  k_cache, v_cache, ck_cache, cv_cache, workspace: Tensor, evict_scratch: Optional[Tensor], init_cross: bool,
                  cache_only: bool, sink: int, evict: int, keep: int, write_start: int, attn_start: int, attn_end: int,
                  start_frame: int, kv_index: Optional[Tensor], global_end: int):
    _need_gpu(noisy, "noisy")
    _need_gpu(timestep, "timestep", None)
    if noisy.dim() != 5 or not noisy.is_contiguous() or timestep.dim() != 2 or not timestep.is_contiguous():
        raise ValueError("dit_forward: noisy must be contiguous [B, F, C, H, W], timestep contiguous [B, groups]")
    if timestep.dtype not in (torch.float32, torch.int64):
        raise ValueError(f"dit_forward: timestep must be float32 or int64, got {timestep.dtype}")
    L = m.num_layers
    if not (len(k_cache) == len(v_cache) == len(ck_cache) == len(cv_cache) == L):
        raise ValueError(f"dit_forward: cache lists must have {L} entries")
    B, F, _, H, W = noisy.shape
    sh = m.shape
    if noisy.shape[2] != sh.in_dim or timestep.shape[0] != B:
        raise ValueError(f"dit_forward: noisy must carry {sh.in_dim} channels and timestep one row per sample")
    cap = k_cache[0].shape[1] if k_cache[0].dim() == 4 else -1
    want_kv, want_cross = (B, cap, sh.num_heads, sh.head_dim), (B, sh.text_len, sh.num_heads, sh.head_dim)
    n_new = F * (H // 2) * (W // 2)
    if not (0 <= attn_start < attn_end <= cap and 0 <= write_start and write_start + n_new == attn_end):
        raise ValueError(f"dit_forward: cache plan does not fit the cache (write_start {write_start} + {n_new} new tokens, "
                         f"window [{attn_start}, {attn_end}), capacity {cap})")
    if init_cross:
        if prompt_embeds is None:
            raise ValueError("dit_forward: init_cross needs prompt_embeds")
        _need_gpu(prompt_embeds, "prompt_embeds")
        if tuple(prompt_embeds.shape) != (B, sh.text_len, sh.text_dim) or not prompt_embeds.is_contiguous():
            raise ValueError(f"dit_forward: prompt_embeds must be contiguous [{B}, {sh.text_len}, {sh.text_dim}], got {tuple(prompt_embeds.shape)}")
    if add_condition is not None:
        _need_gpu(add_condition, "add_condition")
        if add_condition.dim() != 3 or add_condition.shape[:2] != (B, n_new) or not add_condition.is_contiguous():
            raise ValueError(f"dit_forward: add_condition must be contiguous [{B}, {n_new}, pose_dim], got {tuple(add_condition.shape)}")
    if not workspace.is_cuda or workspace.dtype != torch.uint8 or not workspace.is_contiguous():
        raise ValueError("dit_forward: workspace must be a contiguous CUDA uint8 tensor")
    if evict_scratch is not None and (not evict_scratch.is_cuda or evict_scratch.dtype != torch.uint8 or not evict_scratch.is_contiguous()):
        raise ValueError("dit_forward: evict_scratch must be a contiguous CUDA uint8 tensor")
    k_ptrs, v_ptrs, ck_ptrs, cv_ptrs = _pointer_tables(model, k_cache, v_cache, ck_cache, cv_cache, want_kv, want_cross, noisy.device)
    a = _lib.ForwardArgs()
    a.batch, a.frames, a.lat_h, a.lat_w, a.groups = B, F, H, W, timestep.shape[1]
    a.noisy, a.timestep = noisy.data_ptr(), timestep.data_ptr()
    a.t_is_int64 = 1 if timestep.dtype == torch.int64 else 0
    a.prompt_embeds = _ptr(prompt_embeds)
    a.init_cross = 1 if init_cross else 0
    a.add_condition = _ptr(add_condition)
    a.k_cache_host, a.v_cache_host, a.ck_cache_host, a.cv_cache_host = k_ptrs, v_ptrs, ck_ptrs, cv_ptrs
    a.cache_tokens = cap
    a.sink_tokens, a.evict, a.keep = sink, evict, keep
    a.write_start, a.attn_start, a.attn_end, a.start_frame = write_start, attn_start, attn_end, start_frame
    if evict_scratch is not None:
        a.evict_scratch, a.evict_scratch_bytes = evict_scratch.data_ptr(), evict_scratch.numel() * evict_scratch.element_size()
    a.cache_only = 1 if cache_only else 0
    if cache_only:
        flow = torch.empty(0, dtype=torch.bfloat16, device=noisy.device)
        x0 = torch.empty(0, dtype=torch.bfloat16, device=noisy.device)
    else:
        flow = torch.empty(B, F, m.shape.out_dim, H, W, dtype=torch.bfloat16, device=noisy.device)
        x0 = torch.empty_like(flow)
        a.flow_out, a.x0_out = flow.data_ptr(), x0.data_ptr()
    a.workspace, a.workspace_bytes = workspace.data_ptr(), workspace.numel() * workspace.element_size()
    if kv_index is not None:
        if kv_index.dtype != torch.int64 or not kv_index.is_cuda or not kv_index.is_contiguous() or tuple(kv_index.shape) != (L, 2):
            raise ValueError(f"dit_forward: kv_index must be a contiguous CUDA int64 [{L}, 2] tensor")
        a.kv_index_out, a.global_end = kv_index.data_ptr(), global_end
    return a, flow, x0


def _timed_call(fn, *args) -> int:
    t0, c0 = time.perf_counter(), time.thread_time()
    rc = fn(*args)
    dt, dc = time.perf_counter() - t0, time.thread_time() - c0
    rec = HOST_ENQUEUE.setdefault(threading.get_ident(), [0, 0.0, 0.0])
    rec[0] += 1
    rec[1] += dt
    rec[2] += dc
    return rc


@custom_op(f"{NAMESPACE}::dit_forward",
           mutates_args=("k_cache", "v_cache", "ck_cache", "cv_cache", "workspace", "evict_scratch", "kv_index"))
def dit_forward(model: int, noisy: Tensor, timestep: Tensor, prompt_embeds: Optional[Tensor], add_condition: Optional[Tensor],
                k_cache: List[Tensor], v_cache: List[Tensor], ck_cache: List[Tensor], cv_cache: List[Tensor],
                workspace: Tensor, evict_scratch: Optional[Tensor], init_cross: bool, cache_only: bool, sink: int, evict: int,
                keep: int, write_start: int, attn_start: int, attn_end: int, start_frame: int,
                kv_index: Optional[Tensor], global_end: int) -> Tuple[Tensor, Tensor]:
    m = _model(model)
    a, flow, x0 = _forward_args(m, model, noisy, timestep, prompt_embeds, add_condition, k_cache, v_cache, ck_cache, cv_cache, workspace,
                                evict_scratch, init_cross, cache_only, sink, evict, keep, write_start, attn_start, attn_end, start_frame,
                                kv_index, global_end)
    _lib.check(_timed_call(_lib.lib().sf_dit_forward, C.byref(m.cmodel), C.byref(a), _stream(noisy)), "sf_dit_forward")
    return flow, x0


@custom_op(f"{NAMESPACE}::dit_forward_pair",
           mutates_args=("k_cache", "v_cache", "ck_cache", "cv_cache", "workspace", "evict_scratch", "kv_index"))
def dit_forward_pair(model: int, ctx_noisy: Tensor, ctx_timestep: Tensor, noisy: Tensor, timestep: Tensor,
                     k_cache: List[Tensor], v_cache: List[Tensor], ck_cache: List[Tensor], cv_cache: List[Tensor],
                     workspace: Tensor, evict_scratch: Optional[Tensor], ctx_plan: List[int], plan: List[int],
                     kv_index: Optional[Tensor], global_end: int) -> Tuple[Tensor, Tensor]:
    m = _model(model)
    if len(ctx_plan) != 7 or len(plan) != 7 or ctx_noisy.shape != noisy.shape or ctx_timestep.shape != timestep.shape:
        raise ValueError("dit_forward_pair: two passes of one shape with 7 plan integers each expected")
    a0, _, _ = _forward_args(m, model, ctx_noisy, ctx_timestep, None, None, k_cache, v_cache, ck_cache, cv_cache, workspace, evict_scratch,
                             False, True, *ctx_plan, None, 0)
    a1, flow, x0 = _forward_args(m, model, noisy, timestep, None, None, k_cache, v_cache, ck_cache, cv_cache, workspace, evict_scratch,
                                 False, False, *plan, kv_index, global_end)
    _lib.check(_timed_call(_lib.lib().sf_dit_forward_pair, C.byref(m.cmodel), C.byref(a0), C.byref(a1), _stream(noisy)), "sf_dit_forward_pair")
    return flow, x0


@dit_forward_pair.register_fake
def _(model, ctx_noisy, ctx_timestep, noisy, timestep, k_cache, v_cache, ck_cache, cv_cache, workspace, evict_scratch, ctx_plan, plan,
      kv_index, global_end):
    B, F, _, H, W = noisy.shape
    out_dim = _model(model).shape.out_dim
    return noisy.new_empty((B, F, out_dim, H, W)), noisy.new_empty((B, F, out_dim, H, W))


@dit_forward.register_fake
def _(model, noisy, timestep, prompt_embeds, add_condition, k_cache, v_cache, ck_cache, cv_cache, workspace, evict_scratch,
      init_cross, cache_only, sink, evict, keep, write_start, attn_start, attn_end, start_frame, kv_index, global_end):
    if cache_only:
        return noisy.new_empty((0,)), noisy.new_empty((0,))
    B, F, _, H, W = noisy.shape
    out_dim = _model(model).shape.out_dim
    return noisy.new_empty((B, F, out_dim, H, W)), noisy.new_empty((B, F, out_dim, H, W))


@custom_op(f"{NAMESPACE}::vae_decode_frames", mutates_args=("state", "scratch", "out"))
def vae_decode_frames(model: int, state: Tensor, scratch: Tensor, z: Tensor, out: Tensor, h: int, w: int, window_frames: int,
                      frame_index: int, window: int, history_at: int) -> None:
    m = _model(model)
    _need_gpu(z, "z")
    _need_gpu(out, "out", torch.float32)
    if z.dim() != 4 or not z.is_contiguous() or not out.is_contiguous():
        raise ValueError("vae_decode_frames: contiguous z [F, z_dim, h, w] and out expected")
    if tuple(z.shape[1:]) != (m.shape.z_dim, h, w):
        raise ValueError(f"vae_decode_frames: z must be [F, {m.shape.z_dim}, {h}, {w}], got {tuple(z.shape)}")
    for name, t in (("state", state), ("scratch", scratch)):
        if not t.is_cuda or t.dtype != torch.uint8 or not t.is_contiguous():
            raise ValueError(f"vae_decode_frames: {name} must be a contiguous CUDA uint8 tensor")
    sf_, tf_ = m.shape.spatial_factor, m.shape.temporal_factor
    frames = 1 if frame_index == 0 else tf_ * z.shape[0]
    if frame_index == 0 and z.shape[0] != 1:
        raise ValueError("vae_decode_frames: the frame that follows a reset (frame_index 0) is decoded alone")
    if out.numel() < frames * 3 * (sf_ * h) * (sf_ * w):
        raise ValueError(f"vae_decode_frames: out holds {out.numel()} floats, {frames} frames of 3 x {sf_ * h} x {sf_ * w} need "
                         f"{frames * 3 * sf_ * h * sf_ * w}")
    _lib.check(_lib.lib().sf_vae_decode_frames(C.byref(m.cmodel), state.data_ptr(), state.numel(), scratch.data_ptr(), scratch.numel(),
                                               z.data_ptr(), h, w, window_frames, frame_index, z.shape[0], window, history_at,
                                               out.data_ptr(), _stream(z)),
               "sf_vae_decode_frames")


@custom_op(f"{NAMESPACE}::taehv_decode_frames", mutates_args=("state", "scratch", "out"))
def taehv_decode_frames(model: int, state: Tensor, scratch: Tensor, z: Tensor, out: Tensor, h: int, w: int, clamp: bool) -> None:
    m = _model(model)
    _need_gpu(z, "z")
    _need_gpu(out, "out", torch.float32)
    if z.dim() != 4 or not z.is_contiguous() or not out.is_contiguous():
        raise ValueError("taehv_decode_frames: contiguous z [F, z_dim, h, w] and out expected")
    zc = m.cmodel.z_dim
    if tuple(z.shape[1:]) != (zc, h, w):
        raise ValueError(f"taehv_decode_frames: z must be [F, {zc}, {h}, {w}], got {tuple(z.shape)}")
    for name, t in (("state", state), ("scratch", scratch)):
        if not t.is_cuda or t.dtype != torch.uint8 or not t.is_contiguous():
            raise ValueError(f"taehv_decode_frames: {name} must be a contiguous CUDA uint8 tensor")
    need = 4 * z.shape[0] * 3 * (8 * h) * (8 * w)
    if out.numel() < need:
        raise ValueError(f"taehv_decode_frames: out holds {out.numel()} floats, {4 * z.shape[0]} frames of 3 x {8 * h} x {8 * w} need {need}")
    _lib.check(_lib.lib().sf_taehv_decode_frames(C.byref(m.cmodel), state.data_ptr(), state.numel(), scratch.data_ptr(), scratch.numel(),
                                                 z.data_ptr(), h, w, z.shape[0], int(clamp), out.data_ptr(), _stream(z)),
               "sf_taehv_decode_frames")


@custom_op(f"{NAMESPACE}::vae_encode_frames", mutates_args=("state", "scratch", "out"))
def vae_encode_frames(model: int, state: Tensor, scratch: Tensor, pixels: Tensor, out: Tensor, H: int, W: int, window_frames: int,
                      chunk_index: int, window: int, history_at: int) -> None:
    m = _model(model)
    _need_gpu(pixels, "pixels", None)
    _need_gpu(out, "out", torch.float32)
    if pixels.dtype not in (torch.bfloat16, torch.float32):
        raise ValueError(f"vae_encode_frames: pixels must be bf16 or float32, got {pixels.dtype}")
    if pixels.dim() != 4 or pixels.shape[0] != 3 or tuple(pixels.shape[2:]) != (H, W) or not pixels[0].is_contiguous():
        raise ValueError(f"vae_encode_frames: pixels must be [3, T, {H}, {W}] with contiguous frames, got {tuple(pixels.shape)}")
    for name, t in (("state", state), ("scratch", scratch)):
        if not t.is_cuda or t.dtype != torch.uint8 or not t.is_contiguous():
            raise ValueError(f"vae_encode_frames: {name} must be a contiguous CUDA uint8 tensor")
    T = pixels.shape[1]
    if chunk_index == 0:
        if T != 1:
            raise ValueError("vae_encode_frames: the chunk that follows a reset (chunk_index 0) is one pixel frame")
        n = 1
    else:
        if T % 4 or T == 0:
            raise ValueError(f"vae_encode_frames: {T} pixel frames is not a whole number of 4-frame chunks")
        n = T // 4
    sf_ = m.shape.spatial_factor
    if tuple(out.shape) != (n, m.shape.z_dim, H // sf_, W // sf_) or not out.is_contiguous():
        raise ValueError(f"vae_encode_frames: out must be contiguous [{n}, {m.shape.z_dim}, {H // sf_}, {W // sf_}], got {tuple(out.shape)}")
    _lib.check(_lib.lib().sf_vae_encode_frames(C.byref(m.cmodel), state.data_ptr(), state.numel(), scratch.data_ptr(), scratch.numel(),
                                               pixels.data_ptr(), int(pixels.dtype == torch.float32), pixels.stride(0), H, W, window_frames,
                                               chunk_index, n, window, history_at, out.data_ptr(), _stream(pixels)),
               "sf_vae_encode_frames")


@vae_encode_frames.register_fake
def _(model, state, scratch, pixels, out, H, W, window_frames, chunk_index, window, history_at):
    return None


@custom_op(f"{NAMESPACE}::t5_encode", mutates_args=("workspace",))
def t5_encode(model: int, ids: Tensor, mask: Tensor, buckets: Tensor, workspace: Tensor) -> Tensor:
    m = _model(model)
    _need_gpu(ids, "ids", torch.int64), _need_gpu(mask, "mask", torch.int64), _need_gpu(buckets, "buckets", torch.int32)
    if ids.dim() != 2 or ids.shape != mask.shape or not ids.is_contiguous() or not mask.is_contiguous():
        raise ValueError("t5_encode: ids and mask must be contiguous [B, L]")
    B, L = ids.shape
    out = torch.empty(B, L, m.shape.dim, dtype=torch.bfloat16, device=ids.device)
    _lib.check(_lib.lib().sf_t5_encode(C.byref(m.cmodel), ids.data_ptr(), mask.data_ptr(), buckets.data_ptr(), B, L, out.data_ptr(),
                                       workspace.data_ptr(), workspace.numel(), _stream(ids)), "sf_t5_encode")
    return out


@t5_encode.register_fake
def _(model, ids, mask, buckets, workspace):
    return ids.new_empty((ids.shape[0], ids.shape[1], _model(model).shape.dim), dtype=torch.bfloat16)


OPS = ("attention", "gemm", "gemm_out", "lincomb", "lincomb_out", "add_noise", "dit_forward", "dit_forward_pair", "vae_decode_frames", "vae_encode_frames", "taehv_decode_frames",
       "t5_encode")
```

Measured before the change: 90.56.

## Write V directly from QKV GEMM epilogue into the KV cache

Adds a split-output GEMM variant whose epilogue routes columns past n_split (the V third of QKV) straight into per-batch KV cache segments, and skips the V copy in the qkv norm/rope/cache kernel when this path is active. This removes one read and write of V per layer. Direct routing is disabled when eviction runs or when pass write ranges overlap another pass's attention window, and a copy route remains selectable. It adds per-row segment-offset arithmetic in the GEMM epilogue and ABI surface.

```diff
diff --git a/include/sf_hip.h b/include/sf_hip.h
--- a/include/sf_hip.h
+++ b/include/sf_hip.h
@@ -46,10 +46,22 @@
 
 int sf_gemm_bf16(const sf_gemm_args* args, void* stream);
 
+typedef struct sf_gemm_split {
+  void* out2;
+  int32_t n_split;
+  int32_t ldo2;
+  int32_t seg_rows;
+  int32_t n_segs;
+  const int64_t* seg_off;
+} sf_gemm_split;
+int sf_gemm_bf16_split(const sf_gemm_args* args, const sf_gemm_split* split, void* stream);
+
 #define SF_FP8_AMAX_PARTS 1024
 int sf_quantize_fp8(const void* x, int ldx, int M, int K, int rows_per_segment, void* q_out, float* scale_out, void* stream);
 
 int sf_gemm_fp8(const sf_gemm_args* args, const float* a_scale, int rows_per_segment, const float* w_scale, void* stream);
+int sf_gemm_fp8_split(const sf_gemm_args* args, const float* a_scale, int rows_per_segment, const float* w_scale,
+                      const sf_gemm_split* split, void* stream);
 
 int sf_small_linear_fp8(const void* x, const void* w_q, const float* w_scale, const void* bias, void* out, int M, int N, int K,
                         int rows_per_segment, int act_in, int act_out, void* stream);
@@ -174,6 +186,11 @@
 int sf_dit_forward_pair(const sf_model* model, const sf_forward_args* context_pass, const sf_forward_args* next_pass,
                         void* stream);
 
+enum sf_v_route { SF_V_ROUTE_AUTO = 0, SF_V_ROUTE_COPY = 1 };
+int sf_dit_forward_ex(const sf_model* model, const sf_forward_args* args, int v_route, void* stream);
+int sf_dit_forward_pair_ex(const sf_model* model, const sf_forward_args* context_pass, const sf_forward_args* next_pass,
+                           int v_route, void* stream);
+
 
 enum sf_conv_epilogue {
   SF_CONV_BIAS = 0,
diff --git a/self-forcing_amd/_lib.py b/self-forcing_amd/_lib.py
--- a/self-forcing_amd/_lib.py
+++ b/self-forcing_amd/_lib.py
@@ -30,6 +30,8 @@
 ATTN_STRUCTURES = {"auto": 0, "r64": 1, "w8": 2, "w4": 3}
 CONV_STRUCTURES = {"auto": 0, "igemm": 1, "halo": 2}
 GEMM_STRUCTURES = {"auto": 0, "t128": 1, "pp256": 2, "pp128": 3, "pp224": 4, "pp192": 5}
+V_ROUTES = {"auto": 0, "copy": 1}
+GEMM_MAX_SEGS = 32
 
 
 class GemmArgs(C.Structure):
@@ -43,6 +45,11 @@
         ("a_bstride", C.c_int64), ("w_bstride", C.c_int64), ("o_bstride", C.c_int64), ("r_bstride", C.c_int64),
         ("structure", C.c_int32),
     ]
+
+
+class GemmSplit(C.Structure):
+    _fields_ = [("out2", C.c_void_p), ("n_split", C.c_int32), ("ldo2", C.c_int32), ("seg_rows", C.c_int32), ("n_segs", C.c_int32),
+                ("seg_off", C.POINTER(C.c_int64))]
 
 
 class LayerWeights(C.Structure):
@@ -197,6 +204,8 @@
     "sf_small_linear": (C.c_int, [_vp, _vp, _vp, _vp, _i, _i, _i, _i, _i, _vp]),
     "sf_quantize_fp8": (C.c_int, [_vp, _i, _i, _i, _i, _vp, _vp, _vp]),
     "sf_gemm_fp8": (C.c_int, [C.POINTER(GemmArgs), _vp, _i, _vp, _vp]),
+    "sf_gemm_bf16_split": (C.c_int, [C.POINTER(GemmArgs), C.POINTER(GemmSplit), _vp]),
+    "sf_gemm_fp8_split": (C.c_int, [C.POINTER(GemmArgs), _vp, _i, _vp, C.POINTER(GemmSplit), _vp]),
     "sf_small_linear_fp8": (C.c_int, [_vp, _vp, _vp, _vp, _vp, _i, _i, _i, _i, _i, _i, _vp]),
     "sf_sinusoid_embedding": (C.c_int, [_vp, _i, _vp, _i, _i, _vp]),
     "sf_layernorm_modulate": (C.c_int, [_vp, _vp, _i, _i, _f, _vp, _vp, _vp, _vp, _i64, _i, _vp]),
@@ -214,6 +223,8 @@
     "sf_dit_workspace_bytes": (C.c_size_t, [C.POINTER(Model), _i, _i, _i, _i, _i]),
     "sf_dit_forward": (C.c_int, [C.POINTER(Model), C.POINTER(ForwardArgs), _vp]),
     "sf_dit_forward_pair": (C.c_int, [C.POINTER(Model), C.POINTER(ForwardArgs), C.POINTER(ForwardArgs), _vp]),
+    "sf_dit_forward_ex": (C.c_int, [C.POINTER(Model), C.POINTER(ForwardArgs), _i, _vp]),
+    "sf_dit_forward_pair_ex": (C.c_int, [C.POINTER(Model), C.POINTER(ForwardArgs), C.POINTER(ForwardArgs), _i, _vp]),
     "sf_conv_igemm": (C.c_int, [C.POINTER(ConvArgs), _vp]),
     "sf_conv_pick_nt": (C.c_int, [_i]),
     "sf_rmsnorm_silu_cl": (C.c_int, [_vp, _vp, _vp, _i64, _i, _i, _vp]),
diff --git a/self-forcing_amd/csrc/dit_forward.hip b/self-forcing_amd/csrc/dit_forward.hip
--- a/self-forcing_amd/csrc/dit_forward.hip
+++ b/self-forcing_amd/csrc/dit_forward.hip
@@ -54,7 +54,7 @@
   return carve(model, nullptr, batch, frames, lat_h, lat_w, groups).total;
 }
 
-static int forward_passes(const sf_model* m, const sf_forward_args* const* ps, int np, void* stream) {
+static int forward_passes(const sf_model* m, const sf_forward_args* const* ps, int np, int v_route, void* stream) {
   const sf_forward_args* a = ps[0];
   SF_CHECK(m && a, "sf_dit_forward: null argument");
   SF_CHECK(m->layers_host && m->num_layers > 0, "sf_dit_forward: model has no layers");
@@ -88,6 +88,16 @@
     SF_CHECK(!(q->cache_only && first_full != np), "sf_dit_forward_pair: cache_only passes must come first");
   }
   SF_CHECK(a->k_cache_host && a->v_cache_host && a->ck_cache_host && a->cv_cache_host, "sf_dit_forward: null cache table");
+  SF_CHECK(v_route == SF_V_ROUTE_AUTO || v_route == SF_V_ROUTE_COPY, "sf_dit_forward: unknown v_route %d", v_route);
+  bool v_direct = v_route == SF_V_ROUTE_AUTO;
+  for (int p = 0; p < np; ++p) {
+    if (ps[p]->evict > 0) v_direct = false;
+    for (int p2 = p + 1; p2 < np; ++p2)
+      if (ps[p2]->write_start < ps[p]->attn_end && ps[p2]->write_start + L > ps[p]->attn_start) v_direct = false;
+  }
+  int64_t v_off[32];
+  for (int p = 0; p < np; ++p)
+    for (int b = 0; b < B; ++b) v_off[p * B + b] = ((int64_t)b * a->cache_tokens + ps[p]->write_start) * C;
   const Work ws = carve(m, a->workspace, np * B, F, a->lat_h, a->lat_w, G);
   SF_CHECK(a->workspace && a->workspace_bytes >= ws.total, "sf_dit_forward: workspace too small (%zu < %zu)", a->workspace_bytes, ws.total);
   SF_CHECK(!a->init_cross || a->prompt_embeds, "sf_dit_forward: init_cross needs prompt_embeds");
@@ -162,7 +172,10 @@
     const void* mod = lw.modulation;
     const bool last_layer = l == m->num_layers - 1;
     SF_TRY(sf_layernorm_modulate(ws.x, ws.xn, Mt, C, m->eps, bptr(mod, 0), bptr(mod, C), bptr(ws.e0, 0), bptr(ws.e0, C), 6L * C, rpg, stream));
-    SF_TRY(lin(Gemm(ws.xn, C, lw.qkv_w, C, ws.qkv, 3 * C, Mt, 3 * C, C).bias(lw.qkv_b).fp8w(lq.qkv_q, lq.qkv_s, M)));
+    Gemm qkv(ws.xn, C, lw.qkv_w, C, ws.qkv, 3 * C, Mt, 3 * C, C);
+    qkv.bias(lw.qkv_b).fp8w(lq.qkv_q, lq.qkv_s, M);
+    if (v_direct) qkv.split(a->v_cache_host[l], C, 2 * C, L, v_off, np * B);
+    SF_TRY(lin(qkv));
     for (int p = 0; p < np; ++p) {
       const sf_forward_args* q = ps[p];
       const size_t roff = (size_t)p * M;
@@ -170,7 +183,8 @@
         SF_TRY(sf_kv_evict(q->k_cache_host[l], B, q->cache_tokens, C, q->sink_tokens, q->evict, q->keep, q->evict_scratch, q->evict_scratch_bytes, stream));
         SF_TRY(sf_kv_evict(q->v_cache_host[l], B, q->cache_tokens, C, q->sink_tokens, q->evict, q->keep, q->evict_scratch, q->evict_scratch_bytes, stream));
       }
-      SF_TRY(sf_qkv_norm_rope_cache(bptr(ws.qkv, roff * 3 * C), lw.norm_q_w, lw.norm_k_w, (void*)bptr(ws.q, roff * C), q->k_cache_host[l], q->v_cache_host[l],
+      SF_TRY(sf_qkv_norm_rope_cache(bptr(ws.qkv, roff * 3 * C), lw.norm_q_w, lw.norm_k_w, (void*)bptr(ws.q, roff * C), q->k_cache_host[l],
+                                    v_direct ? nullptr : q->v_cache_host[l],
                                     m->rope_cos, m->rope_sin, B, F, h, w, C, m->num_heads, q->cache_tokens, q->write_start, q->start_frame, m->eps, stream));
       if (q->cache_only && last_layer) continue;
       SF_TRY(sf_attention(bptr(ws.q, roff * C), bptr(q->k_cache_host[l], (size_t)q->attn_start * C), bptr(q->v_cache_host[l], (size_t)q->attn_start * C),
@@ -219,13 +233,24 @@
 extern "C" int sf_dit_forward(const sf_model* m, const sf_forward_args* a, void* stream) {
   SF_CHECK(m && a, "sf_dit_forward: null argument");
   const sf_forward_args* one[1] = {a};
-  return forward_passes(m, one, 1, stream);
+  return forward_passes(m, one, 1, SF_V_ROUTE_AUTO, stream);
+}
+
+extern "C" int sf_dit_forward_ex(const sf_model* m, const sf_forward_args* a, int v_route, void* stream) {
+  SF_CHECK(m && a, "sf_dit_forward: null argument");
+  const sf_forward_args* one[1] = {a};
+  return forward_passes(m, one, 1, v_route, stream);
 }
 
 extern "C" int sf_dit_forward_pair(const sf_model* m, const sf_forward_args* context_pass, const sf_forward_args* next_pass, void* stream) {
+  return sf_dit_forward_pair_ex(m, context_pass, next_pass, SF_V_ROUTE_AUTO, stream);
+}
+
+extern "C" int sf_dit_forward_pair_ex(const sf_model* m, const sf_forward_args* context_pass, const sf_forward_args* next_pass, int v_route,
+                                      void* stream) {
   SF_CHECK(m && context_pass && next_pass, "sf_dit_forward_pair: null argument");
   SF_CHECK(context_pass->workspace == next_pass->workspace && context_pass->workspace_bytes == next_pass->workspace_bytes,
            "sf_dit_forward_pair: both passes name the same workspace (sized for 2 x batch)");
   const sf_forward_args* two[2] = {context_pass, next_pass};
-  return forward_passes(m, two, 2, stream);
-}
+  return forward_passes(m, two, 2, v_route, stream);
+}
diff --git a/self-forcing_amd/csrc/elementwise.hip b/self-forcing_amd/csrc/elementwise.hip
--- a/self-forcing_amd/csrc/elementwise.hip
+++ b/self-forcing_amd/csrc/elementwise.hip
@@ -126,7 +126,7 @@
   }
 }
 
-template <int NCH>
+template <int NCH, bool COPY_V>
 __global__ __launch_bounds__(256) void qkv_norm_rope_cache_kernel(
     const bf16_t* __restrict__ qkv, const bf16_t* __restrict__ wq, const bf16_t* __restrict__ wk,
     bf16_t* __restrict__ q_out, bf16_t* __restrict__ k_cache, bf16_t* __restrict__ v_cache,
@@ -142,10 +142,12 @@
   const bf16_t* src = qkv + (long)row * 3 * C;
   const long crow = ((long)b * cache_tokens + write_start + t) * C;
 
-#pragma unroll
-  for (int i = 0; i < NCH; ++i) {
-    const int e = (i * 64 + lane) * 8;
-    *reinterpret_cast<u32x4*>(v_cache + crow + e) = *reinterpret_cast<const u32x4*>(src + 2 * C + e);
+  if constexpr (COPY_V) {
+#pragma unroll
+    for (int i = 0; i < NCH; ++i) {
+      const int e = (i * 64 + lane) * 8;
+      *reinterpret_cast<u32x4*>(v_cache + crow + e) = *reinterpret_cast<const u32x4*>(src + 2 * C + e);
+    }
   }
 
 #pragma unroll
@@ -405,7 +407,7 @@
                                       void* k_cache, void* v_cache, const float* rope_cos, const float* rope_sin,
                                       int B, int f, int h, int w, int C, int num_heads, int64_t cache_tokens,
                                       int write_start, int start_frame, float eps, void* stream) {
-  SF_CHECK(qkv && norm_q_w && norm_k_w && q_out && k_cache && v_cache && rope_cos && rope_sin, "sf_qkv_norm_rope_cache: null tensor");
+  SF_CHECK(qkv && norm_q_w && norm_k_w && q_out && k_cache && rope_cos && rope_sin, "sf_qkv_norm_rope_cache: null tensor");
   SF_CHECK(B > 0 && f > 0 && h > 0 && w > 0 && channels_ok(C), "sf_qkv_norm_rope_cache: unsupported shape");
   SF_CHECK(num_heads > 0 && C == num_heads * 128, "sf_qkv_norm_rope_cache: head_dim must be 128 (C=%d heads=%d)", C, num_heads);
   const int L = f * h * w;
@@ -417,12 +419,17 @@
   hipStream_t s = (hipStream_t)stream;
   const int c = 64, c1 = c / 3, c0 = c - 2 * c1;
   switch (C / 512) {
-#define SF_QKV_CASE(N)                                                                                                   \
-  case N: hipLaunchKernelGGL((qkv_norm_rope_cache_kernel<N>), grid, block, 0, s, (const bf16_t*)qkv, (const bf16_t*)norm_q_w, \
-                             (const bf16_t*)norm_k_w, (bf16_t*)q_out, (bf16_t*)k_cache, (bf16_t*)v_cache, rope_cos, rope_sin,  \
-                             rows, L, h, w, C, (long)cache_tokens, write_start, start_frame, eps, c0, c1); break;
+#define SF_QKV_LAUNCH(N, COPY_V)                                                                                              \
+  hipLaunchKernelGGL((qkv_norm_rope_cache_kernel<N, COPY_V>), grid, block, 0, s, (const bf16_t*)qkv, (const bf16_t*)norm_q_w,     \
+                     (const bf16_t*)norm_k_w, (bf16_t*)q_out, (bf16_t*)k_cache, (bf16_t*)v_cache, rope_cos, rope_sin, rows, L, h, \
+                     w, C, (long)cache_tokens, write_start, start_frame, eps, c0, c1)
+#define SF_QKV_CASE(N)                                                        \
+  case N:                                                                     \
+    if (v_cache) SF_QKV_LAUNCH(N, true); else SF_QKV_LAUNCH(N, false);       \
+    break;
     SF_QKV_CASE(1) SF_QKV_CASE(2) SF_QKV_CASE(3) SF_QKV_CASE(4) SF_QKV_CASE(5) SF_QKV_CASE(6) SF_QKV_CASE(8) SF_QKV_CASE(10)
 #undef SF_QKV_CASE
+#undef SF_QKV_LAUNCH
   }
   SF_HIP_LAUNCH_CHECK("sf_qkv_norm_rope_cache");
   return 0;
diff --git a/self-forcing_amd/csrc/gemm_bf16.hip b/self-forcing_amd/csrc/gemm_bf16.hip
--- a/self-forcing_amd/csrc/gemm_bf16.hip
+++ b/self-forcing_amd/csrc/gemm_bf16.hip
@@ -28,6 +28,14 @@
   int rows_per_seg;
 };
 
+constexpr int GEMM_MAX_SEGS = 32;
+struct GemmSplitP : GemmP {
+  bf16_t* out2;
+  int n_split, ldo2, seg_rows;
+  long seg_off[GEMM_MAX_SEGS];
+};
+template <class P> constexpr bool is_split = std::is_same<P, GemmSplitP>::value;
+
 typedef const __attribute__((address_space(1))) void* gptr_t;
 typedef __attribute__((address_space(3))) void* lptr_t;
 
@@ -90,14 +98,19 @@
   return o;
 }
 
-template <int EPI, int MT>
-__device__ __forceinline__ void gemm_epilogue(const GemmP& p, f32x4 (&acc)[MT][4], int mrow, int ncol) {
+template <int EPI, int MT, class P>
+__device__ __forceinline__ void gemm_epilogue(const P& p, f32x4 (&acc)[MT][4], int mrow, int ncol) {
 #pragma unroll
   for (int mt = 0; mt < MT; ++mt) {
     const int m = mrow + mt * 16;
     if (m >= p.M) continue;
     const bf16_t* e0row = nullptr;
     if (EPI == SF_EPI_BIAS_GATE_RESID) e0row = p.gate_e0 + (long)(m / p.rows_per_group) * p.gate_group_stride;
+    bf16_t* row2 = nullptr;
+    if constexpr (is_split<P>) {
+      const int s = m / p.seg_rows;
+      row2 = p.out2 + p.seg_off[s] + (long)(m - s * p.seg_rows) * p.ldo2 - p.n_split;
+    }
 #pragma unroll
     for (int nt = 0; nt < 4; ++nt) {
       const int n = ncol + nt * 16;
@@ -106,6 +119,12 @@
         *reinterpret_cast<f32x4*>(reinterpret_cast<float*>(p.out) + (long)m * p.ldo + n) = acc[mt][nt];
         continue;
       }
+      if constexpr (is_split<P>) {
+        if (n >= p.n_split) {
+          *reinterpret_cast<bf16x4*>(row2 + n) = epi_apply<EPI>(p, acc[mt][nt], m, n, e0row);
+          continue;
+        }
+      }
       *reinterpret_cast<bf16x4*>(p.out + (long)m * p.ldo + n) = epi_apply<EPI>(p, acc[mt][nt], m, n, e0row);
     }
   }
@@ -134,8 +153,8 @@
   return o;
 }
 
-template <int EPI, int MT>
-__device__ __forceinline__ void gemm_epilogue_lds(const GemmP& p, f32x4 (&acc)[MT][4], int m_base, int n_base, char* wbuf, int lane) {
+template <int EPI, int MT, class P>
+__device__ __forceinline__ void gemm_epilogue_lds(const P& p, f32x4 (&acc)[MT][4], int m_base, int n_base, char* wbuf, int lane) {
   const int r16 = lane & 15, cg = lane >> 4;
   constexpr bool GATE = EPI == SF_EPI_BIAS_GATE_RESID;
   constexpr bool RESID = EPI == SF_EPI_BIAS_RESID || EPI == SF_EPI_BIAS_GATE_RESID;
@@ -186,6 +205,25 @@
   }
   __builtin_amdgcn_s_waitcnt(0xc07f);
   const int rr = lane >> 3, ch = lane & 7;
+  if constexpr (is_split<P>) {
+    if (n_base >= p.n_split) {
+      int s = (m_base + rr) / p.seg_rows, t = m_base + rr - s * p.seg_rows;
+      long off = p.seg_off[min(s, GEMM_MAX_SEGS - 1)];
+#pragma unroll
+      for (int i = 0; i < 2 * MT; ++i) {
+        const int row = i * 8 + rr;
+        const int m = m_base + row, n = n_base + ch * 8;
+        const bf16x8 v = *reinterpret_cast<const bf16x8*>(wbuf + row * 128 + ((ch ^ (row & 7)) << 4));
+        if (m < p.M && n < p.N) *reinterpret_cast<bf16x8*>(p.out2 + off + (long)t * p.ldo2 + (n - p.n_split)) = v;
+        t += 8;
+        while (t >= p.seg_rows) {
+          t -= p.seg_rows;
+          off = p.seg_off[min(++s, GEMM_MAX_SEGS - 1)];
+        }
+      }
+      return;
+    }
+  }
 #pragma unroll
   for (int i = 0; i < 2 * MT; ++i) {
     const int row = i * 8 + rr;
@@ -195,18 +233,26 @@
   }
 }
 
-template <int EPI, bool F8>
-__global__ __launch_bounds__(GEMM_THREADS, 2) void gemm_bf16_kernel(GemmP p) {
+template <class P>
+__device__ __forceinline__ bool ldo2_ok(const P& p) {
+  if constexpr (is_split<P>) return (p.ldo2 & 7) == 0;
+  else return true;
+}
+
+template <int EPI, bool F8, class P = GemmP>
+__global__ __launch_bounds__(GEMM_THREADS, 2) void gemm_bf16_kernel(P p) {
   extern __shared__ __attribute__((aligned(16))) char smem[];
   const int tid = threadIdx.x;
   const int lane = tid & 63;
   const int wave = __builtin_amdgcn_readfirstlane(tid >> 6);
 
+  if constexpr (!is_split<P>) {
   if (blockIdx.y) {
     const long bz = blockIdx.y;
     p.a += bz * p.a_bs; p.w += bz * p.w_bs;
     if (EPI == SF_EPI_F32) p.out = reinterpret_cast<bf16_t*>(reinterpret_cast<float*>(p.out) + bz * p.o_bs); else p.out += bz * p.o_bs;
     if (p.resid) p.resid += bz * p.r_bs;
+  }
   }
   const int nwg = gridDim.x, bid = blockIdx.x;
   const int wg = sf_xcd_remap(bid, nwg);
@@ -316,7 +362,7 @@
   if constexpr (F8) fp8_scale_acc<4>(p, acc, m0 + wr * 64, n0 + wc * 64, lane);
   const int mrow = m0 + wr * 64 + (lane & 15);
   const int ncol = n0 + wc * 64 + (lane >> 4) * 4;
-  if (EPI != SF_EPI_F32 && (p.N & 7) == 0 && (p.ldo & 7) == 0)
+  if (EPI != SF_EPI_F32 && (p.N & 7) == 0 && (p.ldo & 7) == 0 && ldo2_ok(p))
     gemm_epilogue_lds<EPI, 4>(p, acc, m0 + wr * 64, n0 + wc * 64, smem + wave * 8192, lane);
   else
     gemm_epilogue<EPI, 4>(p, acc, mrow, ncol);
@@ -335,8 +381,8 @@
   static constexpr int PA = (2 * MT + 7) / 8;
 };
 
-template <int EPI, int MT, bool F8>
-__global__ __launch_bounds__(PP_THREADS) void gemm_pp_kernel(GemmP p) {
+template <int EPI, int MT, bool F8, class P = GemmP>
+__global__ __launch_bounds__(PP_THREADS) void gemm_pp_kernel(P p) {
   using Cfg = PPCfg<MT>;
   constexpr int BMp = Cfg::BM, PA = Cfg::PA;
   constexpr int HQA = (MT + 1) / 2, HQB = MT / 2;
@@ -491,7 +537,7 @@
 
   const int m_base = m0 + grp * (BMp / 2), n_base = n0 + wc * 64;
   if constexpr (F8) fp8_scale_acc<MT>(p, acc, m_base, n_base, lane);
-  if ((p.N & 7) == 0 && (p.ldo & 7) == 0)
+  if ((p.N & 7) == 0 && (p.ldo & 7) == 0 && ldo2_ok(p))
     gemm_epilogue_lds<EPI, MT>(p, acc, m_base, n_base, smem + wave * (MT * 2048), lane);
   else
     gemm_epilogue<EPI, MT>(p, acc, m_base + (lane & 15), n_base + (lane >> 4) * 4);
@@ -504,8 +550,8 @@
 constexpr int PP2_A = 128 * 128, PP2_B = 256 * 128;
 constexpr int PP2_LDS = 3 * (PP2_A + PP2_B);
 
-template <int EPI, bool F8>
-__global__ __launch_bounds__(PP_THREADS) void gemm_pp2_kernel(GemmP p) {
+template <int EPI, bool F8, class P = GemmP>
+__global__ __launch_bounds__(PP_THREADS) void gemm_pp2_kernel(P p) {
   extern __shared__ __attribute__((aligned(16))) char smem[];
   const int tid = threadIdx.x;
   const int lane = tid & 63;
@@ -629,28 +675,29 @@
 
   const int m_base = m0 + grp * 64, n_base = n0 + wc * 64;
   if constexpr (F8) fp8_scale_acc<4>(p, acc, m_base, n_base, lane);
-  if ((p.N & 7) == 0 && (p.ldo & 7) == 0)
+  if ((p.N & 7) == 0 && (p.ldo & 7) == 0 && ldo2_ok(p))
     gemm_epilogue_lds<EPI, 4>(p, acc, m_base, n_base, smem + wave * 8192, lane);
   else
     gemm_epilogue<EPI, 4>(p, acc, m_base + (lane & 15), n_base + (lane >> 4) * 4);
 }
 
-template <int EPI, bool F8>
-int launch_pp2(GemmP& p, hipStream_t s) {
+template <int EPI, bool F8, class P>
+int launch_pp2(P& p, hipStream_t s) {
   static bool attr = false;
   if (!attr) {
-    (void)hipFuncSetAttribute(reinterpret_cast<const void*>(&gemm_pp2_kernel<EPI, F8>), hipFuncAttributeMaxDynamicSharedMemorySize, PP2_LDS);
+    (void)hipFuncSetAttribute(reinterpret_cast<const void*>(&gemm_pp2_kernel<EPI, F8, P>), hipFuncAttributeMaxDynamicSharedMemorySize, PP2_LDS);
     attr = true;
   }
   p.tiles_m = (p.M + 127) / 128;
   p.tiles_n = (p.N + 255) / 256;
-  hipLaunchKernelGGL((gemm_pp2_kernel<EPI, F8>), dim3(p.tiles_m * p.tiles_n), dim3(PP_THREADS), PP2_LDS, s, p);
+  hipLaunchKernelGGL((gemm_pp2_kernel<EPI, F8, P>), dim3(p.tiles_m * p.tiles_n), dim3(PP_THREADS), PP2_LDS, s, p);
   return 0;
 }
 
-template <bool F8>
-int launch_pp2_epi(GemmP& p, int epilogue, hipStream_t s) {
-  switch (epilogue) {
+template <bool F8, class P>
+int launch_pp2_epi(P& p, int epilogue, hipStream_t s) {
+  if constexpr (is_split<P>) return epilogue == SF_EPI_BIAS ? launch_pp2<SF_EPI_BIAS, F8>(p, s) : -1;
+  else switch (epilogue) {
     case SF_EPI_BIAS: return launch_pp2<SF_EPI_BIAS, F8>(p, s);
     case SF_EPI_BIAS_GELU: return launch_pp2<SF_EPI_BIAS_GELU, F8>(p, s);
     case SF_EPI_BIAS_RESID: return launch_pp2<SF_EPI_BIAS_RESID, F8>(p, s);
@@ -659,23 +706,24 @@
   }
 }
 
-template <int EPI, int MT, bool F8>
-int launch_pp(GemmP& p, hipStream_t s) {
+template <int EPI, int MT, bool F8, class P>
+int launch_pp(P& p, hipStream_t s) {
   using Cfg = PPCfg<MT>;
   static bool attr = false;
   if (!attr) {
-    (void)hipFuncSetAttribute(reinterpret_cast<const void*>(&gemm_pp_kernel<EPI, MT, F8>), hipFuncAttributeMaxDynamicSharedMemorySize, Cfg::LDS);
+    (void)hipFuncSetAttribute(reinterpret_cast<const void*>(&gemm_pp_kernel<EPI, MT, F8, P>), hipFuncAttributeMaxDynamicSharedMemorySize, Cfg::LDS);
     attr = true;
   }
   p.tiles_m = (p.M + Cfg::BM - 1) / Cfg::BM;
   p.tiles_n = (p.N + 255) / 256;
-  hipLaunchKernelGGL((gemm_pp_kernel<EPI, MT, F8>), dim3(p.tiles_m * p.tiles_n), dim3(PP_THREADS), Cfg::LDS, s, p);
+  hipLaunchKernelGGL((gemm_pp_kernel<EPI, MT, F8, P>), dim3(p.tiles_m * p.tiles_n), dim3(PP_THREADS), Cfg::LDS, s, p);
   return 0;
 }
 
-template <int MT, bool F8>
-int launch_pp_epi(GemmP& p, int epilogue, hipStream_t s) {
-  switch (epilogue) {
+template <int MT, bool F8, class P>
+int launch_pp_epi(P& p, int epilogue, hipStream_t s) {
+  if constexpr (is_split<P>) return epilogue == SF_EPI_BIAS ? launch_pp<SF_EPI_BIAS, MT, F8>(p, s) : -1;
+  else switch (epilogue) {
     case SF_EPI_BIAS: return launch_pp<SF_EPI_BIAS, MT, F8>(p, s);
     case SF_EPI_BIAS_GELU: return launch_pp<SF_EPI_BIAS_GELU, MT, F8>(p, s);
     case SF_EPI_BIAS_RESID: return launch_pp<SF_EPI_BIAS_RESID, MT, F8>(p, s);
@@ -703,8 +751,28 @@
   return 0;
 }
 
-template <bool F8>
-int run_gemm(const sf_gemm_args* a, GemmP& p, const char* name, hipStream_t s) {
+int check_split(const sf_gemm_args* a, const sf_gemm_split* sp, const char* name) {
+  SF_CHECK(sp != nullptr && sp->out2 != nullptr && sp->seg_off != nullptr, "%s: null second region", name);
+  SF_CHECK(a->epilogue == SF_EPI_BIAS && a->batch <= 1, "%s: a second region needs SF_EPI_BIAS and no batch", name);
+  SF_CHECK(sp->n_split > 0 && sp->n_split < a->N && sp->n_split % 64 == 0, "%s: n_split=%d must be a multiple of 64 inside (0, N=%d)", name,
+           sp->n_split, a->N);
+  SF_CHECK(sp->ldo2 >= a->N - sp->n_split && sp->ldo2 % 4 == 0, "%s: ldo2=%d must be a multiple of 4 and >= N - n_split", name, sp->ldo2);
+  SF_CHECK(sp->seg_rows > 0 && sp->n_segs > 0 && sp->n_segs <= GEMM_MAX_SEGS && (int64_t)sp->n_segs * sp->seg_rows >= a->M,
+           "%s: %d segments of %d rows (at most %d segments) must cover M=%d", name, sp->n_segs, sp->seg_rows, GEMM_MAX_SEGS, a->M);
+  SF_CHECK((uintptr_t)sp->out2 % 16 == 0, "%s: misaligned second region", name);
+  for (int i = 0; i < sp->n_segs; ++i)
+    SF_CHECK(sp->seg_off[i] >= 0 && sp->seg_off[i] % 8 == 0, "%s: seg_off[%d]=%lld must be a non-negative multiple of 8", name, i, (long long)sp->seg_off[i]);
+  return 0;
+}
+
+void fill_split(const sf_gemm_split* sp, GemmSplitP& p) {
+  p.out2 = (bf16_t*)sp->out2;
+  p.n_split = sp->n_split; p.ldo2 = sp->ldo2; p.seg_rows = sp->seg_rows;
+  for (int i = 0; i < GEMM_MAX_SEGS; ++i) p.seg_off[i] = sp->seg_off[i < sp->n_segs ? i : sp->n_segs - 1];
+}
+
+template <bool F8, class P>
+int run_gemm(const sf_gemm_args* a, P& p, const char* name, hipStream_t s) {
   int st = a->structure;
   const int nk = p.K / BK;
   const bool pp_ok = a->batch <= 1 && a->epilogue != SF_EPI_F32 && nk >= 2;
@@ -737,7 +805,9 @@
   SF_CHECK(batch == 1 || (a->a_bstride % 8 == 0 && a->w_bstride % 8 == 0 && a->o_bstride % 4 == 0 && a->r_bstride % 4 == 0),
            "%s: batch strides must keep 16-byte (operands) / 8-byte (output) alignment", name);
   const dim3 grid(p.tiles_m * p.tiles_n, batch), block(GEMM_THREADS);
-  switch (a->epilogue) {
+  if constexpr (is_split<P>) {
+    hipLaunchKernelGGL((gemm_bf16_kernel<SF_EPI_BIAS, F8, P>), grid, block, GEMM_LDS, s, p);
+  } else switch (a->epilogue) {
     case SF_EPI_BIAS: hipLaunchKernelGGL((gemm_bf16_kernel<SF_EPI_BIAS, F8>), grid, block, GEMM_LDS, s, p); break;
     case SF_EPI_BIAS_GELU: hipLaunchKernelGGL((gemm_bf16_kernel<SF_EPI_BIAS_GELU, F8>), grid, block, GEMM_LDS, s, p); break;
     case SF_EPI_BIAS_RESID: hipLaunchKernelGGL((gemm_bf16_kernel<SF_EPI_BIAS_RESID, F8>), grid, block, GEMM_LDS, s, p); break;
@@ -776,13 +846,40 @@
   return run_gemm<false>(a, p, "sf_gemm_bf16", (hipStream_t)stream);
 }
 
+extern "C" int sf_gemm_bf16_split(const sf_gemm_args* a, const sf_gemm_split* split, void* stream) {
+  if (const int rc = check_args(a, "sf_gemm_bf16_split", BK)) return rc;
+  if (const int rc = check_split(a, split, "sf_gemm_bf16_split")) return rc;
+  GemmSplitP p;
+  fill_params(a, p, 1);
+  fill_split(split, p);
+  return run_gemm<false>(a, p, "sf_gemm_bf16_split", (hipStream_t)stream);
+}
+
+namespace {
+int check_fp8(const sf_gemm_args* a, const float* a_scale, int rows_per_segment, const float* w_scale, const char* name) {
+  if (const int rc = check_args(a, name, 2 * BK)) return rc;
+  SF_CHECK(a->batch <= 1, "%s: batched products are bf16-only", name);
+  SF_CHECK(a_scale && w_scale && rows_per_segment > 0, "%s: needs a_scale, w_scale and rows_per_segment > 0", name);
+  SF_CHECK((uintptr_t)w_scale % 16 == 0, "%s: w_scale must be 16-byte aligned", name);
+  return 0;
+}
+}
+
 extern "C" int sf_gemm_fp8(const sf_gemm_args* a, const float* a_scale, int rows_per_segment, const float* w_scale, void* stream) {
-  if (const int rc = check_args(a, "sf_gemm_fp8", 2 * BK)) return rc;
-  SF_CHECK(a->batch <= 1, "sf_gemm_fp8: batched products are bf16-only");
-  SF_CHECK(a_scale && w_scale && rows_per_segment > 0, "sf_gemm_fp8: needs a_scale, w_scale and rows_per_segment > 0");
-  SF_CHECK((uintptr_t)w_scale % 16 == 0, "sf_gemm_fp8: w_scale must be 16-byte aligned");
+  if (const int rc = check_fp8(a, a_scale, rows_per_segment, w_scale, "sf_gemm_fp8")) return rc;
   GemmP p;
   fill_params(a, p, 2);
   p.a_scale = a_scale; p.w_scale = w_scale; p.rows_per_seg = rows_per_segment;
   return run_gemm<true>(a, p, "sf_gemm_fp8", (hipStream_t)stream);
 }
+
+extern "C" int sf_gemm_fp8_split(const sf_gemm_args* a, const float* a_scale, int rows_per_segment, const float* w_scale,
+                                 const sf_gemm_split* split, void* stream) {
+  if (const int rc = check_fp8(a, a_scale, rows_per_segment, w_scale, "sf_gemm_fp8_split")) return rc;
+  if (const int rc = check_split(a, split, "sf_gemm_fp8_split")) return rc;
+  GemmSplitP p;
+  fill_params(a, p, 2);
+  fill_split(split, p);
+  p.a_scale = a_scale; p.w_scale = w_scale; p.rows_per_seg = rows_per_segment;
+  return run_gemm<true>(a, p, "sf_gemm_fp8_split", (hipStream_t)stream);
+}
diff --git a/self-forcing_amd/csrc/sf_host.h b/self-forcing_amd/csrc/sf_host.h
--- a/self-forcing_amd/csrc/sf_host.h
+++ b/self-forcing_amd/csrc/sf_host.h
@@ -30,8 +30,10 @@
   const void* wq = nullptr;
   const float* w_scale = nullptr;
   int rows_per_segment = 0;
+  sf_gemm_split sp;
   Gemm(const void* a, int lda, const void* w, int ldw, void* out, int ldo, int M, int N, int K) {
     memset(&g, 0, sizeof(g));
+    memset(&sp, 0, sizeof(sp));
     g.a = a; g.lda = lda; g.w = w; g.ldw = ldw; g.out = out; g.ldo = ldo; g.M = M; g.N = N; g.K = K;
     g.epilogue = SF_EPI_BIAS;
     g.rows_per_group = 1;
@@ -51,10 +53,15 @@
     wq = w_e4m3; w_scale = scale; rows_per_segment = rows_per_seg;
     return *this;
   }
-  int bf16(void* stream) const { return sf_gemm_bf16(&g, stream); }
+  Gemm& split(void* out2, int ldo2, int n_split, int seg_rows, const int64_t* seg_off, int n_segs) {
+    sp.out2 = out2; sp.ldo2 = ldo2; sp.n_split = n_split; sp.seg_rows = seg_rows; sp.seg_off = seg_off; sp.n_segs = n_segs;
+    return *this;
+  }
+  int bf16(void* stream) const { return sp.out2 ? sf_gemm_bf16_split(&g, &sp, stream) : sf_gemm_bf16(&g, stream); }
   int fp8(const void* aq, const float* a_scale, void* stream) const {
     sf_gemm_args q = g;
     q.a = aq; q.lda = g.K; q.w = wq;
+    if (sp.out2) return sf_gemm_fp8_split(&q, a_scale, rows_per_segment, w_scale, &sp, stream);
     return sf_gemm_fp8(&q, a_scale, rows_per_segment, w_scale, stream);
   }
 };
diff --git a/self-forcing_amd/model.py b/self-forcing_amd/model.py
--- a/self-forcing_amd/model.py
+++ b/self-forcing_amd/model.py
@@ -131,6 +131,8 @@
     def workspace(self, B: int, F: int, H: int, W: int, G: int) -> Tensor:
         return self._stream_bytes((B, F, H, W, G), lambda: _lib.lib().sf_dit_workspace_bytes(C.byref(self.cmodel), B, F, H, W, G))
 
+    v_route = "auto"
+
     def forward(self, noisy: Tensor, timestep: Tensor, prompt_embeds: Optional[Tensor], init_cross: bool,
                 k_cache: List[Tensor], v_cache: List[Tensor], ck_cache: List[Tensor], cv_cache: List[Tensor], plan: CachePlan,
                 start_frame: int, evict_scratch: Optional[Tensor] = None, cache_only: bool = False,
diff --git a/self-forcing_amd/ops.py b/self-forcing_amd/ops.py
--- a/self-forcing_amd/ops.py
+++ b/self-forcing_amd/ops.py
@@ -57,6 +57,39 @@
         return torch.ops.sf_hip.gemm(a, w, bias, epi, resid, gate_mod, gate_e0, rows_per_group, st)
     torch.ops.sf_hip.gemm_out(out, a, w, bias, epi, resid, gate_mod, gate_e0, rows_per_group, st)
     return out
+
+
+def gemm_split(a: Tensor, w: Tensor, bias: Optional[Tensor], out: Tensor, out2: Tensor, n_split: int, seg_rows: int, seg_off,
+               structure: str = "auto", a_scale: Optional[Tensor] = None, w_scale: Optional[Tensor] = None,
+               rows_per_segment: Optional[int] = None) -> None:
+    fp8 = a_scale is not None
+    dt = torch.float8_e4m3fn if fp8 else torch.bfloat16
+    a, w, out, out2 = _rows(a, "a", dt), _rows(w, "w", dt), _rows(out, "out"), _rows(out2, "out2")
+    M, K = a.shape
+    N = w.shape[0]
+    seg_off = [int(o) for o in seg_off]
+    if w.shape[1] != K or tuple(out.shape) != (M, N) or not 0 < n_split < N or out2.shape[1] < N - n_split or seg_rows <= 0:
+        raise ValueError(f"gemm_split: a {tuple(a.shape)}, w {tuple(w.shape)}, out {tuple(out.shape)}, out2 {tuple(out2.shape)}, n_split {n_split}")
+    if not 0 < len(seg_off) <= _lib.GEMM_MAX_SEGS or len(seg_off) * seg_rows < M:
+        raise ValueError(f"gemm_split: {len(seg_off)} segments of {seg_rows} rows do not cover M={M}")
+    ld2 = out2.stride(0)
+    for s, o in enumerate(seg_off):
+        rows = min(seg_rows, M - s * seg_rows)
+        if o < 0 or (rows > 0 and o + (rows - 1) * ld2 + (N - n_split) > (out2.shape[0] - 1) * ld2 + out2.shape[1]):
+            raise ValueError(f"gemm_split: segment {s} at offset {o} leaves out2 {tuple(out2.shape)}")
+    g = _lib.GemmArgs()
+    g.a, g.w, g.bias, g.out = a.data_ptr(), w.data_ptr(), _ptr(bias), out.data_ptr()
+    g.M, g.N, g.K = M, N, K
+    g.lda, g.ldw, g.ldo = a.stride(0), w.stride(0), out.stride(0)
+    g.epilogue, g.rows_per_group, g.structure = _EPI["bias"], 1, _lib.GEMM_STRUCTURES[structure]
+    sp = _lib.GemmSplit()
+    offs = (C.c_int64 * len(seg_off))(*seg_off)
+    sp.out2, sp.n_split, sp.ldo2, sp.seg_rows, sp.n_segs, sp.seg_off = out2.data_ptr(), n_split, ld2, seg_rows, len(seg_off), offs
+    if fp8:
+        a_scale, w_scale = a_scale.float().contiguous(), w_scale.float().contiguous()
+        check(lib().sf_gemm_fp8_split(g, a_scale.data_ptr(), rows_per_segment or M, w_scale.data_ptr(), sp, stream_handle()), "sf_gemm_fp8_split")
+    else:
+        check(lib().sf_gemm_bf16_split(g, sp, stream_handle()), "sf_gemm_bf16_split")
 
 
 def small_linear(x: Tensor, w: Tensor, bias: Optional[Tensor], act_in=None, act_out=None) -> Tensor:
@@ -135,18 +168,18 @@
     return out
 
 
-def qkv_norm_rope_cache(qkv: Tensor, norm_q_w: Tensor, norm_k_w: Tensor, k_cache: Tensor, v_cache: Tensor,
+def qkv_norm_rope_cache(qkv: Tensor, norm_q_w: Tensor, norm_k_w: Tensor, k_cache: Tensor, v_cache: Optional[Tensor],
                         rope_cos: Tensor, rope_sin: Tensor, grid, write_start: int, start_frame: int,
                         eps: float = 1e-6) -> Tensor:
     qkv = _rows(qkv, "qkv").contiguous()
     B, S, H, D = k_cache.shape
     f, h, w = grid
     Cc = H * D
-    if not (k_cache.is_contiguous() and v_cache.is_contiguous()):
+    if not (k_cache.is_contiguous() and (v_cache is None or v_cache.is_contiguous())):
         raise ValueError("qkv_norm_rope_cache: caches must be contiguous [B, S, H, D]")
     q = torch.empty(qkv.shape[0], Cc, dtype=torch.bfloat16, device=qkv.device)
     check(lib().sf_qkv_norm_rope_cache(qkv.data_ptr(), norm_q_w.data_ptr(), norm_k_w.data_ptr(), q.data_ptr(), k_cache.data_ptr(),
-                                       v_cache.data_ptr(), rope_cos.data_ptr(), rope_sin.data_ptr(), B, f, h, w, Cc, H, S,
+                                       _ptr(v_cache), rope_cos.data_ptr(), rope_sin.data_ptr(), B, f, h, w, Cc, H, S,
                                        write_start, start_frame, eps, stream_handle()), "sf_qkv_norm_rope_cache")
     return q
 
diff --git a/self-forcing_amd/torch_ops.py b/self-forcing_amd/torch_ops.py
--- a/self-forcing_amd/torch_ops.py
+++ b/self-forcing_amd/torch_ops.py
@@ -339,6 +339,10 @@
     return a, flow, x0
 
 
+def _v_route(m) -> int:
+    return _lib.V_ROUTES[getattr(m, "v_route", "auto")]
+
+
 def _timed_call(fn, *args) -> int:
     t0, c0 = time.perf_counter(), time.thread_time()
     rc = fn(*args)
@@ -361,7 +365,7 @@
     a, flow, x0 = _forward_args(m, model, noisy, timestep, prompt_embeds, add_condition, k_cache, v_cache, ck_cache, cv_cache, workspace,
                                 evict_scratch, init_cross, cache_only, sink, evict, keep, write_start, attn_start, attn_end, start_frame,
                                 kv_index, global_end)
-    _lib.check(_timed_call(_lib.lib().sf_dit_forward, C.byref(m.cmodel), C.byref(a), _stream(noisy)), "sf_dit_forward")
+    _lib.check(_timed_call(_lib.lib().sf_dit_forward_ex, C.byref(m.cmodel), C.byref(a), _v_route(m), _stream(noisy)), "sf_dit_forward")
     return flow, x0
 
 
@@ -378,7 +382,8 @@
                              False, True, *ctx_plan, None, 0)
     a1, flow, x0 = _forward_args(m, model, noisy, timestep, None, None, k_cache, v_cache, ck_cache, cv_cache, workspace, evict_scratch,
                                  False, False, *plan, kv_index, global_end)
-    _lib.check(_timed_call(_lib.lib().sf_dit_forward_pair, C.byref(m.cmodel), C.byref(a0), C.byref(a1), _stream(noisy)), "sf_dit_forward_pair")
+    _lib.check(_timed_call(_lib.lib().sf_dit_forward_pair_ex, C.byref(m.cmodel), C.byref(a0), C.byref(a1), _v_route(m), _stream(noisy)),
+               "sf_dit_forward_pair")
     return flow, x0
 
 
```

After: 90.83 (median of 6 runs). About the same (+0.3%).
